# AechPro/rlgym-ppo

Measured on AMD Instinct MI355X. Metric: ppo_update_samples_per_sec, higher is better.
Workload: dtype f32; 1 GPU; configs[1]: 4096 agents x 128 steps = 524,288-sample buffer, obs 107 f32, 90 discrete actions, 256x3 policy + critic; batch 524,288, minibatch 65,536

## Files before the change

### rlgym_ppo_amd/csrc/api.hip

```cpp
#include "build_id.h"
#include <math.h>
#include <stdarg.h>
#include <string.h>

#include "common.hpp"

namespace rlppo {

static thread_local char g_err[512] = "";

void set_error(const char *fmt, ...) {
    va_list ap;
    va_start(ap, fmt);
    vsnprintf(g_err, sizeof(g_err), fmt, ap);
    va_end(ap);
}

static int64_t padded_width(int64_t d) {
    const int64_t p16 = round_up(d, 16), p64 = round_up(d, 64);
    return (p64 - p16) * 10 >= p64 ? p16 : p64;
}
static int64_t padded_out(int64_t d) {
    if (d <= 32) return 32;
    if (d <= 64) return 64;
    if (d <= 96) return 96;
    return round_up(d, 128);
}

int make_layout(const int32_t *dims, int32_t n_layers, NetLayout *out) {
    RLPPO_CHECK_ARG(dims != nullptr && n_layers >= 1 && n_layers <= RLPPO_MAX_LAYERS, "network: n_layers=%d not in [1,%d]",
                    n_layers, RLPPO_MAX_LAYERS);
    for (int i = 0; i <= n_layers; ++i) RLPPO_CHECK_ARG(dims[i] >= 1, "network: dims[%d]=%d", i, dims[i]);
    out->n_layers = n_layers;
    int64_t off = 0, flat = 0;
    int pin = (int)padded_width(dims[0]);
    for (int l = 0; l < n_layers; ++l) {
        LayerLayout &L = out->L[l];
        L.in = dims[l];
        L.out = dims[l + 1];
        L.pin = pin;
        L.pout = (int)padded_out(dims[l + 1]);
        L.off_w = off;
        off += (int64_t)L.pout * L.pin;
        L.off_wt = off;
        off += (int64_t)L.pin * L.pout;
        L.off_b = off;
        off += L.pout;
        L.off_flat_w = flat;
        flat += (int64_t)L.out * L.in;
        L.off_flat_b = flat;
        flat += L.out;
        pin = L.pout;
    }
    out->packed_floats = off;
    out->flat_floats = flat;
    return 0;
}

static int max_pout(const NetLayout &net) {
    int m = 0;
    for (int l = 0; l < net.n_layers; ++l) m = net.L[l].pout > m ? net.L[l].pout : m;
    return m;
}

struct X3Layout {
    int64_t fwd[RLPPO_MAX_LAYERS], dx[RLPPO_MAX_LAYERS], total;
};
static void x3_layout(const NetLayout &net, X3Layout *o) {
    int64_t off = 0;
    const int last = net.n_layers - 1;
    for (int l = 0; l < net.n_layers; ++l) {
        const LayerLayout &L = net.L[l];
        o->fwd[l] = o->dx[l] = -1;
        if (l >= 1 && l < last && nt_split_ok(L.pout, L.pin)) {
            o->fwd[l] = off;
            off += (int64_t)3 * L.pout * L.pin;
        }
        if (l >= 1 && !(l == last && gemv_head_ok(L.out, L.pin)) && nt_split_ok(L.pin, L.pout)) {
            o->dx[l] = off;
            off += (int64_t)3 * L.pin * L.pout;
        }
    }
    o->total = off;
}

static int g_fold_vhead = 1;

struct RowSource {
    const float *x;
    int64_t ld;
    const unsigned *rowtab = nullptr;
    int64_t src_rows = 0;
};

static int forward(hipStream_t st, const NetLayout &net, const float *packed, const RowSource &in, int64_t n, int out_tanh,
                   float *const *acts, int bf16_operands = 0, unsigned long long *const *bits = nullptr, bool *have_bits = nullptr,
                   bool *head_folded = nullptr, const unsigned short *x3 = nullptr, bool head_prezeroed = false) {
    X3Layout xl;
    if (x3) x3_layout(net, &xl);
    if (have_bits)
        for (int l = 0; l < net.n_layers; ++l) have_bits[l] = false;
    const float *x = in.x;
    int64_t ldx = in.ld;
    const int hl = net.n_layers - 1;
    bool fold = head_folded && g_fold_vhead && hl >= 1 && !out_tanh && !bf16_operands && bits && bits[hl - 1] &&
                gemv_head_ok(net.L[hl].out, net.L[hl].pin) && net.L[hl - 1].pout / 128 <= 2;
    if (x3 && hl >= 1 && xl.fwd[hl - 1] >= 0) fold = false;
    if (head_folded) *head_folded = false;
    for (int l = 0; l < net.n_layers; ++l) {
        const LayerLayout &L = net.L[l];
        const bool last = l == net.n_layers - 1;
        const int epi = last ? (out_tanh ? EPI_BIAS_TANH : EPI_BIAS) : EPI_BIAS_RELU;
        int rc;
        if (last && head_folded && *head_folded) break;
        if (last && !out_tanh && gemv_head_ok(L.out, L.pin))
            rc = launch_gemv_fwd(st, x, ldx, packed + L.off_w, packed + L.off_b, acts[l], L.pout, n, L.pin, L.pout);
        else {
            rc = -1;
            if (!last && bits && bits[l] && x3 && xl.fwd[l] >= 0) {
                rc = launch_gemm_nt_split(st, x, ldx, x3 + xl.fwd[l], packed + L.off_b, acts[l], L.pout, n, L.pout, L.pin, 0, bits[l]);
                if (rc == 0) have_bits[l] = true;
            } else if (!last && bits && bits[l] && !bf16_operands) {
                NtDot dots[2];
                const bool fold_here = fold && l == hl - 1;
                if (fold_here) {
                    if (!head_prezeroed) RLPPO_HIP(hipMemsetAsync(acts[hl], 0, (size_t)n * sizeof(float), st));
                    dots[0].w = packed + net.L[hl].off_w;
                    dots[0].b = packed + net.L[hl].off_b;
                    dots[0].out = acts[hl];
                }
                rc = launch_gemm_nt_bits(st, x, ldx, packed + L.off_w, L.pin, packed + L.off_b, acts[l], L.pout, n, L.pout, L.pin,
                                         EPI_BIAS_RELU, bits[l], l == 0 ? in.rowtab : nullptr, in.src_rows, nullptr, fold_here ? dots : nullptr);
                if (rc == 0) have_bits[l] = true;
                if (fold_here) *head_folded = rc == 0;
            }
            if (l == 0 && in.rowtab && rc != 0) {
                if (rc == -1) set_error("forward: the gathered first layer needs the bitmask form");
                return rc == -1 ? RLPPO_ERR_ARG : rc;
            }
            if (rc == -1)
                rc = launch_gemm_nt(st, x, ldx, packed + L.off_w, L.pin, packed + L.off_b, nullptr, 0, acts[l], L.pout, n, L.pout,
                                    L.pin, epi, bf16_operands);
        }
        if (rc) return rc;
        x = acts[l];
        ldx = L.pout;
    }
    return 0;
}

static bool b16_next_wants_f32(const NetLayout &net, int l) {
    const int nx = l + 1, last = net.n_layers - 1;
    const LayerLayout &N = net.L[nx];
    if (nx == last) {
        const bool fwd_b16 = gemv_head_ok(N.out, N.pin) || nt_b16_ok(N.pout, N.pin, false);
        return !(fwd_b16 && thin_head_ok(N.out, N.pin));
    }
    return !(nt_b16_ok(N.pout, N.pin, true) && tn_b16_ok(N.pout, N.pin));
}
static int forward_b16(hipStream_t st, const NetLayout &net, const float *packed_r, const unsigned short *wb16, const float *x,
                       const unsigned short *xb, int64_t ldx, int64_t n, int out_tanh, float *const *acts,
                       unsigned short *const *actsb, unsigned long long *const *bits, bool *have_bits, bool *f32_valid) {
    for (int l = 0; l < net.n_layers; ++l) have_bits[l] = f32_valid[l] = false;
    int64_t off16 = 0;
    bool x_f32 = true;
    for (int l = 0; l < net.n_layers; ++l) {
        const LayerLayout &L = net.L[l];
        const bool last = l == net.n_layers - 1;
        int rc = 0;
        auto need_x_f32 = [&]() -> int {
            if (x_f32) return 0;
            x_f32 = f32_valid[l - 1] = true;
            return launch_expand_rows(st, actsb[l - 1], acts[l - 1], n * (int64_t)net.L[l - 1].pout);
        };
        if (last) {
            const int epi = out_tanh ? EPI_BIAS_TANH : EPI_BIAS;
            if (!out_tanh && gemv_head_ok(L.out, L.pin))
                rc = launch_gemv_fwd_b16(st, xb, ldx, packed_r + L.off_w, packed_r + L.off_b, acts[l], L.pout, n, L.pin, L.pout);
            else if (nt_b16_ok(L.pout, L.pin, false))
                rc = launch_gemm_nt_b16(st, xb, ldx, wb16 + off16, L.pin, packed_r + L.off_b, acts[l], L.pout, nullptr, 0, n, L.pout,
                                        L.pin, epi, 0, nullptr);
            else {
                rc = need_x_f32();
                if (rc == 0)
                    rc = launch_gemm_nt(st, x, ldx, packed_r + L.off_w, L.pin, packed_r + L.off_b, nullptr, 0, acts[l], L.pout, n,
                                        L.pout, L.pin, epi);
            }
            f32_valid[l] = true;
        } else if (nt_b16_ok(L.pout, L.pin, true) && bits[l]) {
            const bool want = b16_next_wants_f32(net, l);
            rc = launch_gemm_nt_b16(st, xb, ldx, wb16 + off16, L.pin, packed_r + L.off_b, want ? acts[l] : nullptr, L.pout, actsb[l],
                                    L.pout, n, L.pout, L.pin, EPI_BIAS_RELU, 1, bits[l]);
            have_bits[l] = rc == 0;
            f32_valid[l] = want;
        } else {
            rc = need_x_f32();
            if (rc) return rc;
            rc = -1;
            if (bits[l]) {
                rc = launch_gemm_nt_bits(st, x, ldx, packed_r + L.off_w, L.pin, packed_r + L.off_b, acts[l], L.pout, n, L.pout, L.pin,
                                         EPI_BIAS_RELU, bits[l]);
                have_bits[l] = rc == 0;
            }
            if (rc == -1)
                rc = launch_gemm_nt(st, x, ldx, packed_r + L.off_w, L.pin, packed_r + L.off_b, nullptr, 0, acts[l], L.pout, n, L.pout,
                                    L.pin, EPI_BIAS_RELU);
            if (rc == 0) rc = launch_round_rows(st, acts[l], actsb[l], n * (int64_t)L.pout);
            f32_valid[l] = true;
        }
        if (rc) return rc;
        off16 += (int64_t)L.pout * L.pin;
        x = acts[l];
        xb = actsb[l];
        x_f32 = f32_valid[l];
        ldx = L.pout;
    }
    return 0;
}

static size_t forward_ws_floats(const NetLayout &net, int64_t n) { return (size_t)2 * (size_t)n * (size_t)max_pout(net); }

static int forward_pingpong(hipStream_t st, const NetLayout &net, const float *packed, const float *obs, int64_t ld_obs,
                            int64_t n, int out_tanh, void *ws, size_t ws_bytes, float *final_out, const float **out,
                            int64_t *ld_out, int bf16_operands) {
    if (ws_bytes < forward_ws_floats(net, n) * sizeof(float)) {
        set_error("forward: workspace %zu < %zu bytes", ws_bytes, forward_ws_floats(net, n) * sizeof(float));
        return RLPPO_ERR_WORKSPACE;
    }
    RLPPO_CHECK_ARG(ld_obs >= net.L[0].pin && ld_obs % 4 == 0, "forward: ld_obs=%ld must be >= %d (zero padded rows)",
                    (long)ld_obs, net.L[0].pin);
    float *b0 = reinterpret_cast<float *>(ws);
    float *b1 = b0 + (size_t)n * max_pout(net);
    float *acts[RLPPO_MAX_LAYERS];
    for (int l = 0; l < net.n_layers; ++l) acts[l] = (l & 1) ? b1 : b0;
    if (final_out) acts[net.n_layers - 1] = final_out;
    int rc = forward(st, net, packed, RowSource{obs, ld_obs}, n, out_tanh, acts, bf16_operands);
    if (rc) return rc;
    *out = acts[net.n_layers - 1];
    *ld_out = net.L[net.n_layers - 1].pout;
    return 0;
}

}

using namespace rlppo;

static int g_fused_act = 1;
static std::atomic<long long> g_cnt_fused_act{0}, g_cnt_act_chain{0}, g_cnt_paired_pass{0}, g_cnt_gather_fused_pass{0}, g_cnt_pass{0}, g_cnt_group_dw{0}, g_cnt_md_nvec{0};
constexpr int64_t FUSED_ACT_MAX_ROWS = 8192;

struct ActCtx {
    int bf16 = 0;
    unsigned *done = nullptr;
    unsigned done_value = 0;
    unsigned *noise_ctl = nullptr;
    const unsigned *mask = nullptr;
    int mask_words = 0;
};
static int act_ctx(const rlppo_act_opts *o, ActCtx *c, bool late_noise = false, const char *mask_for = nullptr) {
    c->bf16 = get_infer_bf16();
    if (!o) return 0;
    RLPPO_CHECK_ARG(o->precision == RLPPO_PRECISION_DEFAULT || o->precision == RLPPO_PRECISION_FP32 || o->precision == RLPPO_PRECISION_BF16,
                    "act options: inference precision %d (0 = process default, 1 = fp32, 2 = bf16 operands)", o->precision);
    if (o->precision != RLPPO_PRECISION_DEFAULT) c->bf16 = o->precision == RLPPO_PRECISION_BF16;
    c->done = o->done_words;
    c->done_value = o->done_value;
    c->noise_ctl = o->noise_ctl;
    c->mask = o->action_mask;
    c->mask_words = o->mask_words;
    RLPPO_CHECK_ARG(!o->action_mask || !mask_for, "act options: action_mask is an option of the discrete head, not of %s", mask_for ? mask_for : "");
    RLPPO_CHECK_ARG(!o->noise_ctl || late_noise, "act options: noise_ctl is an option of rlppo_discrete_step");
    RLPPO_CHECK_ARG(!o->noise_ctl || (o->done_words && !(o->done_value & 0x80000000u)),
                    "act options: noise_ctl needs done_words (a kernel that gives up on the noise reports it there) and done_value < 2^31");
    return 0;
}
static int mask_words_check(const void *mask, int mask_words, int bits, const char *who, bool logits) {
    RLPPO_CHECK_ARG(!mask || mask_words == (bits + 31) / 32,
                    logits ? "%s: mask_words=%d, but %d logits need %d words per row" : "%s: mask_words=%d, but n_actions=%d needs %d words per row",
                    who, mask_words, bits, (bits + 31) / 32);
    return 0;
}
static int act_mask_check(const ActCtx &c, int n_actions) { return mask_words_check(c.mask, c.mask_words, n_actions, "act options", false); }
static int act_done(hipStream_t st, const ActCtx &c, int64_t n) {
    return c.done ? launch_signal_words(st, c.done, (int)rlppo_act_done_words(n), c.done_value) : 0;
}

extern "C" {
// ... 369 lines not shown
static int ensure_slot(SlotBank &b, int s) {
    if (!b.side[s]) {
        RLPPO_HIP(hipStreamCreateWithFlags(&b.side[s], hipStreamNonBlocking));
        RLPPO_HIP(hipStreamCreateWithFlags(&b.main[s], hipStreamNonBlocking));
        RLPPO_HIP(hipEventCreateWithFlags(&b.ev_fork[s], hipEventDisableTiming));
        RLPPO_HIP(hipEventCreateWithFlags(&b.ev_join[s], hipEventDisableTiming));
        RLPPO_HIP(hipEventCreateWithFlags(&b.ev_slot[s], hipEventDisableTiming));
        RLPPO_HIP(hipEventCreateWithFlags(&b.ev_mid[s], hipEventDisableTiming));
    }
    return 0;
}
static int order_after(hipStream_t to, hipStream_t from, hipEvent_t ev) {
    RLPPO_HIP(hipEventRecord(ev, from));
    RLPPO_HIP(hipStreamWaitEvent(to, ev, 0));
    return 0;
}

static size_t tn_layer_floats(const NetLayout &net, int l, int64_t mb, int prec) {
    size_t f = tn_partial_floats(net.L[l].out, net.L[l].in, mb);
    if (net.L[l].out == 1) {
        const size_t g = (size_t)cdiv(mb, 64) * (size_t)(net.L[l].pin + 4);
        if (g > f) f = g;
    }
    if (prec == 1 && l == net.n_layers - 1) {
        const size_t g = thin_dw_ws_floats(net.L[l].out, net.L[l].pin, mb);
        if (g > f) f = g;
    }
    return (f + 3) / 4 * 4;
}
static size_t tn_ws_floats(const NetLayout &net, int64_t mb, int prec) {
    size_t m = 0;
    for (int l = 0; l < net.n_layers; ++l) {
        const size_t f = tn_layer_floats(net, l, mb, prec);
        m = f > m ? f : m;
    }
    return m;
}
static int g_group_dw = 1;
struct DwList {
    TnProduct p[2 * RLPPO_MAX_LAYERS];
    int n = 0;
    void add(const LayerLayout &L, const float *dY, const RowSource &X, float *grad) {
        TnProduct &q = p[n++];
        q.dY = dY; q.ldy = L.pout; q.ny_valid = L.pout; q.X = X.x; q.ldx = X.ld; q.kx_valid = L.pin;
        q.dW = grad + L.off_flat_w; q.db = grad + L.off_flat_b; q.out = L.out; q.in = L.in;
        q.rowtab = X.rowtab; q.src_rows = X.src_rows;
    }
};
static bool dw_is_gemv(const NetLayout &net, int l) { return l == net.n_layers - 1 && l > 0 && gemv_head_ok(net.L[l].out, net.L[l].pin); }
static size_t tn_region_floats(const NetLayout &pol, const NetLayout &val, int64_t mb, int prec) {
    const size_t chains = tn_ws_floats(pol, mb, prec) + tn_ws_floats(val, mb, prec);
    int outs[2 * RLPPO_MAX_LAYERS], ins[2 * RLPPO_MAX_LAYERS], n = 0;
    for (const NetLayout *net : {&pol, &val})
        for (int l = 0; l < net->n_layers; ++l)
            if (!dw_is_gemv(*net, l)) {
                outs[n] = net->L[l].out;
                ins[n++] = net->L[l].in;
            }
    const size_t group = tn_group_floats(outs, ins, n, mb);
    return chains > group ? chains : group;
}

struct NetWs {
    float *act[RLPPO_MAX_LAYERS] = {};
    float *dx[RLPPO_MAX_LAYERS] = {};
    unsigned long long *bits[RLPPO_MAX_LAYERS] = {};
    unsigned short *actb[RLPPO_MAX_LAYERS] = {};
    unsigned short *dxb[RLPPO_MAX_LAYERS] = {};
    float *tn = nullptr;
};
struct WsPlan {
    NetWs pol, val;
    size_t tn_floats = 0;
    float *states = nullptr;
    float *g_old = nullptr, *g_adv = nullptr, *g_tgt = nullptr, *g_act = nullptr;
    unsigned *rowtab = nullptr;
    unsigned short *states_b = nullptr;
};
constexpr size_t BITS_PAD_RESERVE = 2, B16_PAD_RESERVE = 4;
static size_t plan_workspace(const NetLayout &pol, const NetLayout &val, int64_t mb, int prec, void *base, WsPlan *w) {
    const uintptr_t addr = reinterpret_cast<uintptr_t>(base);
    const size_t rows = (size_t)mb;
    size_t off = 0, slack = 0;
    auto take = [&](size_t floats) {
        off += floats;
        return reinterpret_cast<float *>(addr + (off - floats) * sizeof(float));
    };
    auto align = [&](size_t floats, size_t reserve) {
        const size_t pad = (floats - (addr / sizeof(float) + off) % floats) % floats;
        off += pad;
        slack += reserve - pad;
    };
    const NetLayout *nets[2] = {&pol, &val};
    NetWs *ws[2] = {&w->pol, &w->val};
    for (int i = 0; i < 2; ++i)
        for (int l = 0; l < nets[i]->n_layers; ++l) ws[i]->act[l] = take(rows * nets[i]->L[l].pout);
    const size_t m = max_pout(pol) > max_pout(val) ? max_pout(pol) : max_pout(val);
    for (int i = 0; i < 2; ++i)
        for (int l = 0; l + 1 < nets[i]->n_layers; ++l) ws[i]->dx[l] = take(rows * m);
    w->tn_floats = tn_region_floats(pol, val, mb, prec);
    w->pol.tn = take(w->tn_floats);
    w->val.tn = w->pol.tn + tn_ws_floats(pol, mb, prec);
    align(2, BITS_PAD_RESERVE);
    for (int i = 0; i < 2; ++i)
        for (int l = 0; l + 1 < nets[i]->n_layers; ++l) {
            const size_t f = nt_bits_floats(mb, nets[i]->L[l].pout);
            ws[i]->bits[l] = f ? reinterpret_cast<unsigned long long *>(take(f)) : nullptr;
        }
    w->states = take(rows * pol.L[0].pin);
    w->g_old = take(rows);
    w->g_adv = take(rows);
    w->g_tgt = take(rows);
    w->g_act = take(rows * pol.L[pol.n_layers - 1].pout);
    w->rowtab = reinterpret_cast<unsigned *>(take(rows));
    if (prec == 1) {
        align(4, B16_PAD_RESERVE);
        size_t el = pol.L[0].pin;
        for (int i = 0; i < 2; ++i)
            for (int l = 0; l + 1 < nets[i]->n_layers; ++l) el += 2 * (size_t)nets[i]->L[l].pout;
        unsigned short *hb = reinterpret_cast<unsigned short *>(take((el * rows + 1) / 2));
        auto take16 = [&](size_t n) {
            hb += n;
            return hb - n;
        };
        w->states_b = take16(rows * pol.L[0].pin);
        for (int i = 0; i < 2; ++i)
            for (int l = 0; l + 1 < nets[i]->n_layers; ++l) ws[i]->actb[l] = take16(rows * nets[i]->L[l].pout);
        for (int i = 0; i < 2; ++i)
            for (int l = 0; l + 1 < nets[i]->n_layers; ++l) ws[i]->dxb[l] = take16(rows * nets[i]->L[l].pout);
    }
    return off + slack;
}

static int resolve_precision(int32_t precision, int *mode) {
    RLPPO_CHECK_ARG(precision >= 0 && precision <= 3, "update precision %d (0 = process default, 1 = fp32, 2 = bf16 mixed precision, 3 = split-bf16 products)", precision);
    *mode = precision == RLPPO_PRECISION_DEFAULT ? g_update_bf16 : precision - 1;
    return 0;
}
size_t rlppo_minibatch_workspace_bytes_for(const int32_t *pol_dims, int32_t pol_layers, const int32_t *val_dims, int32_t val_layers,
                                           int64_t mb, int32_t precision) {
    NetLayout pol, val;
    int prec = 0;
    if (make_layout(pol_dims, pol_layers, &pol) || make_layout(val_dims, val_layers, &val) || resolve_precision(precision, &prec)) return 0;
    WsPlan unused;
    return plan_workspace(pol, val, mb > 0 ? mb : 0, prec, nullptr, &unused) * sizeof(float) + 256;
}
size_t rlppo_minibatch_workspace_bytes(const int32_t *pol_dims, int32_t pol_layers, const int32_t *val_dims,
                                       int32_t val_layers, int64_t mb) {
    return rlppo_minibatch_workspace_bytes_for(pol_dims, pol_layers, val_dims, val_layers, mb, RLPPO_PRECISION_DEFAULT);
}

static int backward(hipStream_t st, const NetLayout &net, const float *packed, const RowSource &in, int64_t mb, float *const *acts,
                    float *const *dx, float *grad, float *tn_ws, unsigned long long *const *bits, const bool *have_bits,
                    bool head_folded = false, const unsigned short *x3 = nullptr, DwList *defer = nullptr) {
    const int last = net.n_layers - 1;
    int rc = 0;
    X3Layout xl;
    if (x3) x3_layout(net, &xl);
    for (int l = last; l >= 0; --l) {
        const LayerLayout &L = net.L[l];
        const float *dY = l == last ? acts[last] : dx[l];
        const int64_t ld_hy = head_folded ? 1 : L.pout;
        const RowSource X = l > 0 ? RowSource{acts[l - 1], net.L[l - 1].pout} : in;
        const bool gemv = l == last && l > 0 && gemv_head_ok(L.out, L.pin);
        const size_t floats = tn_layer_floats(net, l, mb, 0);
        if (gemv)
            rc = launch_gemv_dw(st, dY, ld_hy, X.x, X.ld, grad + L.off_flat_w, grad + L.off_flat_b, L.in, L.pin, mb, tn_ws, floats);
        else if (defer)
            defer->add(L, dY, X, grad);
        else
            rc = launch_gemm_tn(st, dY, L.pout, L.pout, X.x, X.ld, L.pin, grad + L.off_flat_w, grad + L.off_flat_b, L.out, L.in, mb,
                                tn_ws, floats, X.rowtab, X.src_rows);
        if (rc) return rc;
        if (l == 0) break;
        rc = -1;
        if (gemv) {
            if (have_bits[l - 1]) rc = launch_gemv_dx_bits(st, dY, ld_hy, packed + L.off_w, bits[l - 1], dx[l - 1], L.pin, L.pin, mb);
            if (rc == -1) rc = launch_gemv_dx(st, dY, ld_hy, packed + L.off_w, acts[l - 1], L.pin, dx[l - 1], L.pin, L.pin, mb);
        } else {
            if (have_bits[l - 1] && x3 && xl.dx[l] >= 0)
                rc = launch_gemm_nt_split(st, dY, L.pout, x3 + xl.dx[l], nullptr, dx[l - 1], L.pin, mb, L.pin, L.pout, 1, bits[l - 1]);
            else if (have_bits[l - 1])
                rc = launch_gemm_nt_bits(st, dY, L.pout, packed + L.off_wt, L.pout, nullptr, dx[l - 1], L.pin, mb, L.pin, L.pout,
                                         EPI_MASK, bits[l - 1]);
            if (rc == -1)
                rc = launch_gemm_nt(st, dY, L.pout, packed + L.off_wt, L.pout, nullptr, acts[l - 1], L.pin, dx[l - 1], L.pin, mb,
                                    L.pin, L.pout, EPI_MASK);
        }
        if (rc) return rc;
    }
    return rc;
}

static int backward_b16(hipStream_t st, const NetLayout &net, const float *packed_r, const unsigned short *wb16, const float *states,
                        const unsigned short *states_b, int64_t ld_states, int64_t mb, float *const *acts,
                        unsigned short *const *actsb, float *const *dx, unsigned short *const *dxb, float *grad, float *tn_ws,
                        size_t tn_floats, unsigned long long *const *bits, const bool *have_bits, bool *f32_valid) {
    const int last = net.n_layers - 1;
    int64_t first[RLPPO_MAX_LAYERS], total = 0;
    for (int l = 0; l < net.n_layers; ++l) {
        first[l] = total;
        total += (int64_t)net.L[l].pout * net.L[l].pin;
    }
    bool dx_f32[RLPPO_MAX_LAYERS] = {};
    int rc = 0;
    auto act_f32 = [&](int l) -> int {
        if (l < 0 || f32_valid[l]) return 0;
        f32_valid[l] = true;
        return launch_expand_rows(st, actsb[l], acts[l], mb * (int64_t)net.L[l].pout);
    };
    auto grad_f32 = [&](int l) -> int {
        if (dx_f32[l]) return 0;
        dx_f32[l] = true;
        return launch_expand_rows(st, dxb[l], dx[l], mb * (int64_t)net.L[l].pout);
    };
    for (int l = last; l >= 0; --l) {
        const LayerLayout &L = net.L[l];
        const float *X = l > 0 ? acts[l - 1] : states;
        const unsigned short *Xb = l > 0 ? actsb[l - 1] : states_b;
        const int64_t ldx = l > 0 ? net.L[l - 1].pout : ld_states;
        const bool gemv = l == last && l > 0 && gemv_head_ok(L.out, L.pin);
        if (l == last) {
            rc = l > 0 ? launch_thin_dw_b16(st, acts[last], L.pout, Xb, ldx, grad + L.off_flat_w, grad + L.off_flat_b, L.out, L.in,
                                            L.pin, mb, tn_ws, tn_floats)
                       : -1;
            if (rc == -1) {
                rc = act_f32(l - 1);
                if (rc) return rc;
                if (gemv)
                    rc = launch_gemv_dw(st, acts[last], L.pout, X, ldx, grad + L.off_flat_w, grad + L.off_flat_b, L.in, L.pin, mb,
                                        tn_ws, tn_floats);
                else
                    rc = launch_gemm_tn(st, acts[last], L.pout, L.pout, X, ldx, L.pin, grad + L.off_flat_w, grad + L.off_flat_b,
                                        L.out, L.in, mb, tn_ws, tn_floats);
            }
        } else if (tn_b16_ok(L.pout, L.pin) && ldx % 8 == 0) {
            rc = launch_gemm_tn_b16(st, dxb[l], L.pout, Xb, ldx, grad + L.off_flat_w, grad + L.off_flat_b, L.pout, L.pin, L.out, L.in,
                                    mb, tn_ws, tn_floats);
        } else {
            rc = grad_f32(l);
            if (rc == 0) rc = act_f32(l - 1);
            if (rc) return rc;
            rc = launch_gemm_tn(st, dx[l], L.pout, L.pout, X, ldx, L.pin, grad + L.off_flat_w, grad + L.off_flat_b, L.out, L.in, mb,
                                tn_ws, tn_floats);
        }
        if (rc) return rc;
        if (l == 0) break;
        if (l < last && have_bits[l - 1] && nt_b16_ok(L.pin, L.pout, true)) {
            rc = launch_gemm_nt_b16(st, dxb[l], L.pout, wb16 + total + first[l], L.pout, nullptr, nullptr, 0, dxb[l - 1], L.pin, mb,
                                    L.pin, L.pout, EPI_MASK, 2, bits[l - 1]);
            if (rc) return rc;
            continue;
        }
        if (l == last && have_bits[l - 1]) {
            rc = launch_thin_dx_b16(st, acts[last], L.pout, L.out, packed_r + L.off_w, L.pin, bits[l - 1], dxb[l - 1], L.pin, L.pin, mb);
            if (rc == 0) continue;
            if (rc != -1) return rc;
        }
        const float *dY = acts[last];
        if (l < last) {
            rc = grad_f32(l);
            if (rc) return rc;
            dY = dx[l];
        }
        rc = -1;
        if (gemv) {
            if (have_bits[l - 1]) rc = launch_gemv_dx_bits(st, dY, L.pout, packed_r + L.off_w, bits[l - 1], dx[l - 1], L.pin, L.pin, mb);
            if (rc == -1) {
                rc = act_f32(l - 1);
                if (rc) return rc;
                rc = launch_gemv_dx(st, dY, L.pout, packed_r + L.off_w, acts[l - 1], L.pin, dx[l - 1], L.pin, L.pin, mb);
            }
        } else {
            if (have_bits[l - 1])
                rc = launch_gemm_nt_bits(st, dY, L.pout, packed_r + L.off_wt, L.pout, nullptr, dx[l - 1], L.pin, mb, L.pin, L.pout,
                                         EPI_MASK, bits[l - 1]);
            if (rc == -1) {
                rc = act_f32(l - 1);
                if (rc) return rc;
                rc = launch_gemm_nt(st, dY, L.pout, packed_r + L.off_wt, L.pout, nullptr, acts[l - 1], L.pin, dx[l - 1], L.pin, mb,
                                    L.pin, L.pout, EPI_MASK);
            }
        }
        if (rc) return rc;
        rc = launch_round_rows(st, dx[l - 1], dxb[l - 1], mb * (int64_t)L.pin);
        if (rc) return rc;
        dx_f32[l - 1] = true;
    }
    return rc;
}

static int g_head_order = 1;
static int g_paired = 1;
constexpr int64_t PAIRED_MIN_ROWS = 262144;
static bool twin_ok(const NetLayout &p, const NetLayout &v, int64_t mb) {
    if (p.n_layers != v.n_layers || p.n_layers < 2) return false;
    for (int l = 0; l + 1 < p.n_layers; ++l) {
        const LayerLayout &a = p.L[l], &b = v.L[l];
        if (a.in != b.in || a.out != b.out || a.pin != b.pin || a.pout != b.pout) return false;
        if (a.pout % 128 != 0 || a.pin % 16 != 0 || nt_bits_floats(mb, a.pout) == 0) return false;
    }
    return true;
}

static int head_forward(hipStream_t st, const NetLayout &net, const float *packed, const float *x, int64_t ldx, int64_t n, int out_tanh,
                        float *out) {
    const LayerLayout &L = net.L[net.n_layers - 1];
    if (!out_tanh && gemv_head_ok(L.out, L.pin)) return launch_gemv_fwd(st, x, ldx, packed + L.off_w, packed + L.off_b, out, L.pout, n, L.pin, L.pout);
    return launch_gemm_nt(st, x, ldx, packed + L.off_w, L.pin, packed + L.off_b, nullptr, 0, out, L.pout, n, L.pout, L.pin,
                          out_tanh ? EPI_BIAS_TANH : EPI_BIAS);
}
static int head_backward(hipStream_t st, const NetLayout &net, const float *packed, const float *dY, const float *X, int64_t mb,
                         float *dx_prev, float *grad, float *tn_ws, const unsigned long long *bits_prev, int64_t ld_dy = 0,
                         DwList *defer = nullptr) {
    const int last = net.n_layers - 1;
    const LayerLayout &L = net.L[last];
    const int64_t ldx = net.L[last - 1].pout;
    const bool gemv = gemv_head_ok(L.out, L.pin);
    const size_t floats = tn_layer_floats(net, last, mb, 0);
    if (!ld_dy) ld_dy = L.pout;
    int rc = 0;
    if (gemv) rc = launch_gemv_dw(st, dY, ld_dy, X, ldx, grad + L.off_flat_w, grad + L.off_flat_b, L.in, L.pin, mb, tn_ws, floats);
    else if (defer) defer->add(L, dY, RowSource{X, ldx}, grad);
    else rc = launch_gemm_tn(st, dY, L.pout, L.pout, X, ldx, L.pin, grad + L.off_flat_w, grad + L.off_flat_b, L.out, L.in, mb, tn_ws, floats);
    if (rc) return rc;
    if (gemv) return launch_gemv_dx_bits(st, dY, ld_dy, packed + L.off_w, bits_prev, dx_prev, L.pin, L.pin, mb);
    rc = launch_gemm_nt_bits(st, dY, L.pout, packed + L.off_wt, L.pout, nullptr, dx_prev, L.pin, mb, L.pin, L.pout, EPI_MASK,
                             const_cast<unsigned long long *>(bits_prev));
    if (rc == -1) {
        set_error("paired pass: the output layer's dX needs the bitmask form");
        return RLPPO_ERR_ARG;
    }
    return rc;
}

constexpr int64_t FUSED_GATHER_MIN_ROWS = 262144;
static RowSource first_layer_rows(const rlppo_minibatch_args &a, const NetLayout &pol, const NetLayout &val, int prec, const WsPlan &w) {
    const int64_t src_rows = a.ring_cap > 0 ? a.ring_cap : a.n_rows;
    auto gather_form = [&](const NetLayout &n) {
        return n.n_layers > 1 && nt_gather_ok(a.ld_states, src_rows, n.L[0].pout, n.L[0].pin) && tn_gather_ok(a.ld_states, src_rows) &&
               !(n.L[0].out > 64 && n.L[0].out <= 96 && !(n.L[0].in > 96 && n.L[0].in <= 112));
    };
    if (prec != 1 && (g_fused_gather == 2 || (g_fused_gather == 1 && a.mb >= FUSED_GATHER_MIN_ROWS)) && src_rows > 0 &&
        gather_form(pol) && gather_form(val))
        return RowSource{a.states, a.ld_states, w.rowtab, src_rows};
    return RowSource{w.states, pol.L[0].pin};
}

struct Pass {
    const rlppo_minibatch_args *a;
    NetLayout pol, val;
    int64_t mb;
    int prec;
    int64_t ring_base, ring_cap;
    WsPlan w;
    RowSource rows;
    LossCfg cfg;
    MdSpec md;
    bool md_general = false;
    const float *pol_w, *val_w;
    hipStream_t st, side;
    DwList *defer;
};

static LossCfg loss_cfg(const rlppo_minibatch_args &a) {
    LossCfg c;
    c.clip = a.clip_range;
    c.clip_lo = (float)(1.0 - (double)a.clip_range);
    c.clip_hi = (float)(1.0 + (double)a.clip_range);
    c.ent_coef = a.ent_coef;
    c.mb_ratio = a.mb_ratio;
    c.inv_mb = 1.0f / (float)a.mb;
    c.var_m = a.var_m;
    c.var_b = a.var_b;
    c.adv_norm = a.adv_norm;
    c.vclip = a.value_clip;
    c.kl_slots = a.kl_slots;
    c.stop_word = a.stop_word;
    return c;
}

static int policy_loss(hipStream_t st, const Pass &p) {
    const rlppo_minibatch_args &a = *p.a;
    const int last = p.pol.n_layers - 1;
    const LayerLayout &L = p.pol.L[last];
    const WsPlan &w = p.w;
    MaskRows mr;
    mr.mask = a.action_mask;
    mr.W = a.mask_words;
    mr.idx = a.idx;
    mr.ring_base = p.ring_base;
    mr.ring_cap = p.ring_cap;
    if (a.head == RLPPO_HEAD_DISCRETE) {
        return launch_discrete_loss(st, w.pol.act[last], L.pout, L.out, w.g_act, w.g_old, w.g_adv, p.mb, p.cfg, a.stats, a.action_mask ? &mr : nullptr);
    }
    if (a.head == RLPPO_HEAD_GAUSSIAN)
        return launch_gaussian_loss(st, w.pol.act[last], L.pout, L.out / 2, w.g_act, w.g_old, w.g_adv, p.mb, p.cfg, a.stats);
    if (p.md_general) {
        ++g_cnt_md_nvec;
        return launch_multidiscrete_nvec_loss(st, w.pol.act[last], L.pout, w.g_act, w.g_old, w.g_adv, p.mb, p.cfg, a.stats, p.md,
                                              a.action_mask ? &mr : nullptr);
    }
    return launch_multidiscrete_loss(st, w.pol.act[last], L.pout, w.g_act, w.g_old, w.g_adv, p.mb, p.cfg, a.stats);
}

static int gather(const Pass &p) {
    const rlppo_minibatch_args &a = *p.a;
    const WsPlan &w = p.w;
    const int width = p.pol.L[0].pin;
    float *const vout = w.val.act[p.val.n_layers - 1];
    if (p.prec == 1) {
        auto lean0 = [](const NetLayout &n) {
            return n.n_layers > 1 && nt_b16_ok(n.L[0].pout, n.L[0].pin, true) && tn_b16_ok(n.L[0].pout, n.L[0].pin);
        };
        const int rc = launch_gather_rows_round(p.st, a.states, a.ld_states, a.idx, lean0(p.pol) && lean0(p.val) ? nullptr : w.states,
                                                w.states_b, width, p.mb, p.ring_base, p.ring_cap);
        if (rc) return rc;
    } else if (!p.rows.rowtab) {
        GatherMeta gm;
        gm.actions = a.actions; gm.old_logp = a.old_logp; gm.adv = a.advantages; gm.targets = a.targets;
        gm.g_old = w.g_old; gm.g_adv = w.g_adv; gm.g_tgt = w.g_tgt; gm.g_act = w.g_act;
        gm.zero_n = vout;
        gm.act_dim = a.act_dim;
        return launch_gather_rows(p.st, a.states, a.ld_states, a.idx, w.states, width, p.mb, p.ring_base, p.ring_cap, &gm);
    }
    return launch_gather_meta(p.st, a.idx, a.actions, a.act_dim, a.old_logp, a.advantages, a.targets, w.g_act, w.g_old, w.g_adv, w.g_tgt,
                              p.mb, p.ring_base, p.ring_cap, p.rows.rowtab ? w.rowtab : nullptr, vout);
}

static int paired_pass(const Pass &p, SlotBank &bk, int slot) {
    const rlppo_minibatch_args &a = *p.a;
    const NetLayout &pol = p.pol, &val = p.val;
    const WsPlan &w = p.w;
    const int64_t mb = p.mb;
    const hipStream_t st = p.st, hs = p.side;
    const int H = pol.n_layers - 1;
    int rc;
    const LayerLayout &Lvh = val.L[H];
    const bool fold_v = g_fold_vhead && gemv_head_ok(Lvh.out, Lvh.pin) && val.L[H - 1].pout / 128 <= 2;
    float *vout = w.val.act[H], *pout = w.pol.act[H];
    const int64_t ldv = fold_v ? 1 : Lvh.pout;
    const float *xp = p.rows.x, *xv = xp;
    int64_t ldx = p.rows.ld;
    for (int l = 0; l < H; ++l) {
        const LayerLayout &Lp = pol.L[l], &Lv = val.L[l];
        NtAlt alt;
        alt.A = xv;
        alt.B = p.val_w + Lv.off_w;
        alt.bias = p.val_w + Lv.off_b;
        alt.C = w.val.act[l];
        alt.bits = w.val.bits[l];
        NtDot dots[2];
        const bool fold_here = fold_v && l == H - 1;
        if (fold_here) {
            dots[1].w = p.val_w + Lvh.off_w;
            dots[1].out = vout;
            dots[1].b = p.val_w + Lvh.off_b;
        }
        rc = launch_gemm_nt_bits(st, xp, ldx, p.pol_w + Lp.off_w, Lp.pin, p.pol_w + Lp.off_b, w.pol.act[l], Lp.pout, mb, Lp.pout, Lp.pin,
                                 EPI_BIAS_RELU, w.pol.bits[l], l == 0 ? p.rows.rowtab : nullptr, p.rows.src_rows, &alt,
                                 fold_here ? dots : nullptr);
        if (rc) {
            if (rc == -1) set_error("paired pass: a hidden layer does not have the bitmask form");
            return rc == -1 ? RLPPO_ERR_ARG : rc;
        }
        xp = w.pol.act[l];
        xv = w.val.act[l];
        ldx = Lp.pout;
    }
    if (hs != st) {
        rc = order_after(hs, st, bk.ev_fork[slot]);
        if (rc) return rc;
    }
    if (!fold_v) {
        rc = head_forward(hs, val, p.val_w, xv, ldx, mb, 0, vout);
        if (rc) return rc;
    }
    rc = launch_value_loss(hs, vout, ldv, w.g_tgt, w.g_adv, mb, p.cfg, a.stats);
    if (rc) return rc;
    const bool ordered = g_head_order && hs != st;
    if (!ordered) {
        rc = head_backward(hs, val, p.val_w, vout, xv, mb, w.val.dx[H - 1], a.val_grad, w.val.tn, w.val.bits[H - 1], ldv, p.defer);
        if (rc) return rc;
    }
    rc = head_forward(st, pol, p.pol_w, xp, ldx, mb, a.head == RLPPO_HEAD_GAUSSIAN, pout);
    if (rc) return rc;
    rc = policy_loss(st, p);
    if (rc) return rc;
    if (ordered) {
        rc = order_after(hs, st, bk.ev_mid[slot]);
        if (rc) return rc;
        rc = head_backward(hs, val, p.val_w, vout, xv, mb, w.val.dx[H - 1], a.val_grad, w.val.tn, w.val.bits[H - 1], ldv, p.defer);
        if (rc) return rc;
    }
    rc = head_backward(st, pol, p.pol_w, pout, xp, mb, w.pol.dx[H - 1], a.pol_grad, w.pol.tn, w.pol.bits[H - 1], 0, p.defer);
    if (rc) return rc;
    if (hs != st) {
        rc = order_after(st, hs, bk.ev_join[slot]);
        if (rc) return rc;
    }
    for (int l = H - 1; l >= 0; --l) {
        const LayerLayout &Lp = pol.L[l], &Lv = val.L[l];
        const RowSource Xp = l > 0 ? RowSource{w.pol.act[l - 1], pol.L[l - 1].pout} : p.rows;
        const RowSource Xv = l > 0 ? RowSource{w.val.act[l - 1], val.L[l - 1].pout} : p.rows;
        if (p.defer) {
            p.defer->add(Lp, w.pol.dx[l], Xp, a.pol_grad);
            p.defer->add(Lv, w.val.dx[l], Xv, a.val_grad);
        } else {
            TnPair pr;
            pr.dY = w.val.dx[l];
            pr.X = Xv.x;
            pr.dW = a.val_grad + Lv.off_flat_w;
            pr.db = a.val_grad + Lv.off_flat_b;
            pr.ws = w.val.tn;
            rc = launch_gemm_tn(st, w.pol.dx[l], Lp.pout, Lp.pout, Xp.x, Xp.ld, Lp.pin, a.pol_grad + Lp.off_flat_w, a.pol_grad + Lp.off_flat_b,
                                Lp.out, Lp.in, mb, w.pol.tn, tn_layer_floats(pol, l, mb, 0), Xp.rowtab, Xp.src_rows, &pr);
            if (rc) return rc;
        }
        if (l == 0) break;
        NtAlt alt;
        alt.A = w.val.dx[l];
        alt.B = p.val_w + Lv.off_wt;
        alt.C = w.val.dx[l - 1];
        alt.bits = w.val.bits[l - 1];
        rc = launch_gemm_nt_bits(st, w.pol.dx[l], Lp.pout, p.pol_w + Lp.off_wt, Lp.pout, nullptr, w.pol.dx[l - 1], Lp.pin, mb, Lp.pin,
                                 Lp.pout, EPI_MASK, w.pol.bits[l - 1], nullptr, 0, &alt);
        if (rc) return rc == -1 ? RLPPO_ERR_ARG : rc;
    }
    return 0;
}

static int two_chain_pass(const Pass &p) {
    const rlppo_minibatch_args &a = *p.a;
    const NetLayout &pol = p.pol, &val = p.val;
    const WsPlan &w = p.w;
    const int64_t mb = p.mb;
    const bool b16 = p.prec == 1;
    const unsigned short *pol_wb16 = reinterpret_cast<const unsigned short *>(a.pol_wb16);
    const unsigned short *val_wb16 = reinterpret_cast<const unsigned short *>(a.val_wb16);
    const unsigned short *pol_x3 = p.prec == 2 ? pol_wb16 : nullptr, *val_x3 = p.prec == 2 ? val_wb16 : nullptr;
    bool phave[RLPPO_MAX_LAYERS] = {}, vhave[RLPPO_MAX_LAYERS] = {};
    bool pf32[RLPPO_MAX_LAYERS] = {}, vf32[RLPPO_MAX_LAYERS] = {};
    bool v_folded = false;
    int rc;
    if (b16) {
        rc = forward_b16(p.side, val, p.val_w, val_wb16, p.rows.x, w.states_b, p.rows.ld, mb, 0, w.val.act, w.val.actb, w.val.bits, vhave,
                         vf32);
        if (rc) return rc;
        rc = forward_b16(p.st, pol, p.pol_w, pol_wb16, p.rows.x, w.states_b, p.rows.ld, mb, a.head == RLPPO_HEAD_GAUSSIAN, w.pol.act,
                         w.pol.actb, w.pol.bits, phave, pf32);
    } else {
        rc = forward(p.side, val, p.val_w, p.rows, mb, 0, w.val.act, 0, w.val.bits, vhave, &v_folded, val_x3, true);
        if (rc) return rc;
        rc = forward(p.st, pol, p.pol_w, p.rows, mb, a.head == RLPPO_HEAD_GAUSSIAN, w.pol.act, 0, w.pol.bits, phave, nullptr, pol_x3);
    }
    if (rc) return rc;
    const int64_t ldv = v_folded ? 1 : val.L[val.n_layers - 1].pout;
    rc = launch_value_loss(p.side, w.val.act[val.n_layers - 1], ldv, w.g_tgt, w.g_adv, mb, p.cfg, a.stats);
    if (rc) return rc;
    rc = policy_loss(p.st, p);
    if (rc) return rc;
    if (b16) {
        rc = backward_b16(p.side, val, p.val_w, val_wb16, p.rows.x, w.states_b, p.rows.ld, mb, w.val.act, w.val.actb, w.val.dx, w.val.dxb,
                          a.val_grad, w.val.tn, tn_ws_floats(val, mb, p.prec), w.val.bits, vhave, vf32);
        if (rc) return rc;
        return backward_b16(p.st, pol, p.pol_w, pol_wb16, p.rows.x, w.states_b, p.rows.ld, mb, w.pol.act, w.pol.actb, w.pol.dx, w.pol.dxb,
                            a.pol_grad, w.pol.tn, tn_ws_floats(pol, mb, p.prec), w.pol.bits, phave, pf32);
    }
    rc = backward(p.side, val, p.val_w, p.rows, mb, w.val.act, w.val.dx, a.val_grad, w.val.tn, w.val.bits, vhave, v_folded, val_x3, p.defer);
    if (rc) return rc;
    return backward(p.st, pol, p.pol_w, p.rows, mb, w.pol.act, w.pol.dx, a.pol_grad, w.pol.tn, w.pol.bits, phave, false, pol_x3, p.defer);
}

static int ppo_minibatch(void *stream, const rlppo_minibatch_args *a, const int32_t *md_nvec, int32_t md_heads) {
    RLPPO_CHECK_ARG(a != nullptr, "ppo_minibatch: null args");
    Pass p;
    p.a = a;
    int rc = make_layout(a->pol_dims, a->pol_layers, &p.pol);
    if (rc) return rc;
    rc = make_layout(a->val_dims, a->val_layers, &p.val);
    if (rc) return rc;
    const NetLayout &pol = p.pol, &val = p.val;
    const int64_t mb = p.mb = a->mb;
    if (mb == 0) return 0;
    rc = resolve_precision(a->precision, &p.prec);
    if (rc) return rc;
    RLPPO_CHECK_ARG(mb > 0 && a->pol_packed && a->val_packed && a->pol_grad && a->val_grad && a->states && a->actions &&
                        a->old_logp && a->targets && a->advantages && a->idx && a->stats && a->workspace,
                    "ppo_minibatch: null pointer");
    RLPPO_CHECK_ARG(val.L[val.n_layers - 1].out == 1, "ppo_minibatch: critic must have one output");
    RLPPO_CHECK_ARG(a->value_clip >= 0.f && a->value_clip < INFINITY, "ppo_minibatch: value_clip=%g", (double)a->value_clip);
    RLPPO_CHECK_ARG(pol.L[0].in == val.L[0].in, "ppo_minibatch: policy and critic observe different sizes");
    RLPPO_CHECK_ARG(a->ld_states >= pol.L[0].pin && a->ld_states % 4 == 0, "ppo_minibatch: ld_states=%ld < %d",
                    (long)a->ld_states, pol.L[0].pin);
    const size_t ws_bytes = plan_workspace(pol, val, mb, p.prec, a->workspace, &p.w) * sizeof(float);
    if (a->ws_bytes < ws_bytes) {
        set_error("ppo_minibatch: workspace %zu < %zu bytes", a->ws_bytes, ws_bytes);
        return RLPPO_ERR_WORKSPACE;
    }
    const int n_out = pol.L[pol.n_layers - 1].out;
    RLPPO_CHECK_ARG(a->head == RLPPO_HEAD_DISCRETE || a->head == RLPPO_HEAD_GAUSSIAN || a->head == RLPPO_HEAD_MULTIDISCRETE,
                    "ppo_minibatch: unknown head %d", a->head);
    RLPPO_CHECK_ARG(!a->action_mask || a->head == RLPPO_HEAD_DISCRETE || (a->head == RLPPO_HEAD_MULTIDISCRETE && md_nvec),
                    "ppo_minibatch: action_mask is an option of the discrete head, not of the %s head",
                    a->head == RLPPO_HEAD_GAUSSIAN ? "Gaussian" : "multi-discrete (without md_nvec: the fixed-bin kernels take no mask)");
    if (int rc_mask = mask_words_check(a->action_mask, a->mask_words, n_out, "ppo_minibatch", false)) return rc_mask;
    if (a->head == RLPPO_HEAD_DISCRETE) {
        RLPPO_CHECK_ARG(a->act_dim == 1, "discrete head: act_dim must be 1");
        RLPPO_CHECK_ARG(pol.L[pol.n_layers - 1].pout <= DISCRETE_LOSS_MAX_LD, "discrete head: padded width %ld too large",
                        (long)pol.L[pol.n_layers - 1].pout);
    }
    if (a->head == RLPPO_HEAD_GAUSSIAN)
        RLPPO_CHECK_ARG(n_out % 2 == 0 && a->act_dim == n_out / 2, "gaussian head: act_dim=%d, outputs=%d", a->act_dim, n_out);
    RLPPO_CHECK_ARG(!md_nvec || a->head == RLPPO_HEAD_MULTIDISCRETE, "ppo_minibatch: md_nvec is an option of the multi-discrete head, not of the %s head",
                    a->head == RLPPO_HEAD_GAUSSIAN ? "Gaussian" : "discrete");
    if (a->head == RLPPO_HEAD_MULTIDISCRETE && md_nvec) {
        rc = md_spec_make(md_nvec, md_heads, "multi-discrete head: md_nvec / md_heads", &p.md);
        if (rc) return rc;
        p.md_general = true;
        RLPPO_CHECK_ARG(p.md.S == n_out, "multi-discrete head: md_nvec sums to %d, but the policy has %d outputs", p.md.S, n_out);
        RLPPO_CHECK_ARG(a->act_dim == p.md.H, "multi-discrete head: act_dim=%d, but md_heads=%d", a->act_dim, p.md.H);
    } else if (a->head == RLPPO_HEAD_MULTIDISCRETE)
        RLPPO_CHECK_ARG(n_out == 21 && a->act_dim == 8, "multi-discrete head: needs 21 outputs and act_dim 8");
    RLPPO_CHECK_ARG(p.prec != 1 || (a->pol_packed_r && a->val_packed_r && a->pol_wb16 && a->val_wb16),
                    "ppo_minibatch: the bf16 update precision needs the rlppo_net_pack_bf16 images of both networks (pol_packed_r / val_packed_r / pol_wb16 / val_wb16)");
    RLPPO_CHECK_ARG(p.prec != 2 || (a->pol_wb16 && a->val_wb16),
                    "ppo_minibatch: the split-bf16 update precision needs the rlppo_net_pack_x3 images of both networks (pol_wb16 / val_wb16)");
    p.ring_cap = a->ring_cap > 0 ? a->ring_cap : INT64_MAX;
    p.ring_base = a->ring_cap > 0 ? a->ring_base : 0;
    RLPPO_CHECK_ARG(p.ring_base >= 0 && p.ring_base < p.ring_cap, "ppo_minibatch: ring_base=%ld not in [0, ring_cap=%ld)",
                    (long)a->ring_base, (long)a->ring_cap);
    const int slot = a->slot;
    RLPPO_CHECK_ARG(slot >= 0 && slot < RLPPO_MAX_SLOTS, "ppo_minibatch: slot %d not in [0, %d)", slot, RLPPO_MAX_SLOTS);

    p.rows = first_layer_rows(*a, pol, val, p.prec, p.w);
    const bool twin = p.prec == 0 && (g_paired == 2 || (g_paired == 1 && mb >= PAIRED_MIN_ROWS)) && twin_ok(pol, val, mb);
    p.cfg = loss_cfg(*a);
    p.pol_w = p.prec == 1 ? a->pol_packed_r : a->pol_packed;
    p.val_w = p.prec == 1 ? a->val_packed_r : a->val_packed;
    DwList dws;
    p.defer = (g_group_dw && p.prec != 1) ? &dws : nullptr;

    SlotBank *bank = nullptr;
    rc = slot_bank(&bank);
    if (rc) return rc;
    SlotBank &bk = *bank;
    rc = ensure_slot(bk, slot);
    if (rc) return rc;
    const hipStream_t caller = (hipStream_t)stream;
    p.st = caller;
    if (slot > 0) {
        p.st = bk.main[slot];
        rc = order_after(p.st, caller, bk.ev_slot[slot]);
        if (rc) return rc;
        bk.pending[slot] = true;
    }
    rc = gather(p);
    if (rc) return rc;
    p.side = p.st;
    if (g_two_streams) {
        p.side = bk.side[slot];
        rc = order_after(p.side, p.st, bk.ev_fork[slot]);
        if (rc) return rc;
    }
    ++g_cnt_pass;
    if (twin) ++g_cnt_paired_pass;
    if (p.rows.rowtab) ++g_cnt_gather_fused_pass;
    rc = twin ? paired_pass(p, bk, slot) : two_chain_pass(p);
    if (rc) return rc;
    if (!twin && p.side != p.st) {
        rc = order_after(p.st, p.side, bk.ev_join[slot]);
        if (rc) return rc;
    }
    if (p.defer && dws.n) {
        ++g_cnt_group_dw;
        rc = launch_gemm_tn_group(p.st, dws.p, dws.n, mb, p.w.pol.tn, p.w.tn_floats);
    }
    return rc;
}

int rlppo_ppo_minibatch(void *stream, const rlppo_minibatch_args *a) { return ppo_minibatch(stream, a, nullptr, 0); }
int rlppo_ppo_minibatch_nvec(void *stream, const rlppo_minibatch_args *a, const int32_t *md_nvec, int32_t md_heads) {
    return ppo_minibatch(stream, a, md_nvec, md_heads);
}

int rlppo_ppo_join(void *stream) {
    SlotBank *bank = nullptr;
    int rc = slot_bank(&bank);
    if (rc) return rc;
    SlotBank &bk = *bank;
    for (int s = 1; s < RLPPO_MAX_SLOTS; ++s)
        if (bk.pending[s]) {
            rc = order_after((hipStream_t)stream, bk.main[s], bk.ev_slot[s]);
            if (rc) return rc;
            bk.pending[s] = false;
        }
    return 0;
}

int rlppo_clip_adam(void *stream, float *params, float *grads, float *exp_avg, float *exp_avg_sq, int64_t n,
                    double max_norm, double lr, double beta1, double beta2, double eps, int64_t step, double *gnorm2) {
    if (n == 0) return 0;
    RLPPO_CHECK_ARG(n > 0 && params && grads && exp_avg && exp_avg_sq && gnorm2 && step >= 1, "clip_adam: bad argument");
    const double bc1 = 1.0 - pow(beta1, (double)step);
    const double bc2 = 1.0 - pow(beta2, (double)step);
    const float step_size = (float)(lr / bc1);
    const float bc2_sqrt = (float)sqrt(bc2);
    return launch_clip_adam((hipStream_t)stream, params, grads, exp_avg, exp_avg_sq, n, (float)max_norm, step_size, bc2_sqrt,
                            (float)(1.0 - beta1), (float)beta2, (float)(1.0 - beta2), (float)eps, gnorm2);
}

int rlppo_clip_adam_pack2(void *stream, const rlppo_opt_net *a, const rlppo_opt_net *b, void *sync_ws) {
    RLPPO_CHECK_ARG(a && b, "clip_adam_pack2: null descriptor");
    const rlppo_opt_net *d[2] = {a, b};
    NetLayout nets[2];
    float *p[2], *g[2], *m[2], *v[2], *packed[2];
    double *gn[2];
    int64_t n[2];
    float max_norm[2], step_size[2], bc2_sqrt[2], omb1[2], beta2[2], omb2[2], eps[2];
    const unsigned *skip[2];
    for (int k = 0; k < 2; ++k) {
        skip[k] = d[k]->skip_word;
        int rc = make_layout(d[k]->dims, d[k]->n_layers, &nets[k]);
        if (rc) return rc;
        RLPPO_CHECK_ARG(d[k]->params && d[k]->grads && d[k]->exp_avg && d[k]->exp_avg_sq && d[k]->packed && d[k]->gnorm2 &&
                            d[k]->step >= 1, "clip_adam_pack2: bad argument (net %d)", k);
        const double bc1 = 1.0 - pow(d[k]->beta1, (double)d[k]->step);
        const double bc2 = 1.0 - pow(d[k]->beta2, (double)d[k]->step);
        p[k] = d[k]->params; g[k] = d[k]->grads; m[k] = d[k]->exp_avg; v[k] = d[k]->exp_avg_sq; packed[k] = d[k]->packed;
        gn[k] = d[k]->gnorm2;
        const LayerLayout &last = nets[k].L[nets[k].n_layers - 1];
        n[k] = last.off_flat_b + last.out;
        max_norm[k] = (float)d[k]->max_norm; step_size[k] = (float)(d[k]->lr / bc1); bc2_sqrt[k] = (float)sqrt(bc2);
        omb1[k] = (float)(1.0 - d[k]->beta1); beta2[k] = (float)d[k]->beta2; omb2[k] = (float)(1.0 - d[k]->beta2);
        eps[k] = (float)d[k]->eps;
    }
    return launch_clip_adam_pack2((hipStream_t)stream, nets, p, g, m, v, packed, gn, n, max_norm, step_size, bc2_sqrt, omb1, beta2,
                                  omb2, eps, sync_ws, skip);
}

int64_t rlppo_kl_slots_doubles(int64_t mb) { return kl_slots_doubles(mb); }

int rlppo_adv_stats(void *stream, const int64_t *idx, int64_t n, const float *advantages, int64_t ring_base, int64_t ring_cap,
                    float *out, void *ws) {
    RLPPO_CHECK_ARG(n >= 1 && idx && advantages && out && ws, "adv_stats: bad argument");
    const int64_t cap = ring_cap > 0 ? ring_cap : INT64_MAX, base = ring_cap > 0 ? ring_base : 0;
    RLPPO_CHECK_ARG(base >= 0 && base < cap, "adv_stats: ring_base=%ld not in [0, ring_cap=%ld)", (long)ring_base, (long)ring_cap);
    return launch_adv_stats((hipStream_t)stream, idx, n, advantages, base, cap, out, ws);
}

int rlppo_kl_gate(void *stream, const rlppo_kl_gate_args *a) {
    RLPPO_CHECK_ARG(a && a->kl_slots && a->n_passes >= 0 && a->slot_stride >= 3 && a->phase >= 0 && a->phase <= 2 && a->stop_word,
                    "kl_gate: bad argument");
    RLPPO_CHECK_ARG(a->phase == 0 || a->exchange, "kl_gate: phases 1 and 2 need the exchange words");
    RLPPO_CHECK_ARG(a->phase == 1 || a->host_words, "kl_gate: host_words missing");
    return launch_kl_gate((hipStream_t)stream, *a);
}

int rlppo_learn_report(void *stream, const rlppo_report_args *a) {
    RLPPO_CHECK_ARG(a != nullptr, "learn_report: null args");
    RLPPO_CHECK_ARG(a->n_pol >= 0 && a->n_val >= 0 && (a->n_pol == 0 || (a->pol_before && a->pol_now)) && (a->n_val == 0 || (a->val_before && a->val_now)),
                    "learn_report: parameter vectors missing");
    RLPPO_CHECK_ARG(a->stats && a->out && a->done_word && a->ws, "learn_report: null pointer (stats / out / done_word / ws)");
    RLPPO_CHECK_ARG((reinterpret_cast<uintptr_t>(a->ws) & 15) == 0, "learn_report: ws must be 16-byte aligned");
    return launch_learn_report((hipStream_t)stream, *a);
}

}

extern "C" {
int rlppo_gather_rows(void *stream, const float *src, int64_t ld_src, const int64_t *idx, float *dst, int32_t width, int64_t n) {
    if (n == 0) return 0;
    RLPPO_CHECK_ARG(n > 0 && src && idx && dst, "gather_rows: null pointer");
    return launch_gather_rows((hipStream_t)stream, src, ld_src, idx, dst, width, n);
}
int rlppo_welford_increment(void *stream, const float *samples, int64_t ld, int64_t n, int32_t d, void *mean, void *m2,
                            int64_t count, int32_t state_is_f64) {
    if (n == 0) return 0;
    RLPPO_CHECK_ARG(n > 0 && d > 0 && ld >= d && count >= 0 && samples && mean && m2, "welford_increment: bad argument");
    return launch_welford((hipStream_t)stream, samples, ld, n, d, mean, m2, (long long)count, state_is_f64 != 0);
}
int rlppo_welford_merge(void *stream, int32_t d, void *mean, void *m2, int64_t count, const float *other_mean,
                        const float *other_m2, int64_t other_count, int32_t state_is_f64) {
    if (other_count == 0) return 0;
    RLPPO_CHECK_ARG(d > 0 && count >= 0 && other_count > 0 && mean && m2 && other_mean && other_m2, "welford_merge: bad argument");
    return launch_welford_merge((hipStream_t)stream, d, mean, m2, (long long)count, other_mean, other_m2, (long long)other_count,
                                state_is_f64 != 0);
}
int64_t rlppo_wb16_elems(const int32_t *dims, int32_t n_layers) {
    NetLayout net;
    if (make_layout(dims, n_layers, &net)) return -1;
    int64_t n = 0;
    for (int l = 0; l < net.n_layers; ++l) n += (int64_t)net.L[l].pout * net.L[l].pin;
    return 2 * n;
}
int rlppo_net_pack_bf16(void *stream, const int32_t *dims, int32_t n_layers, const float *flat, float *packed_r, void *wb16) {
    NetLayout net;
    int rc = make_layout(dims, n_layers, &net);
    if (rc) return rc;
    RLPPO_CHECK_ARG(flat && packed_r && wb16, "net_pack_bf16: null pointer");
    return launch_pack_bf16((hipStream_t)stream, net, flat, packed_r, reinterpret_cast<unsigned short *>(wb16));
}
int64_t rlppo_x3_elems(const int32_t *dims, int32_t n_layers) {
    NetLayout net;
    if (make_layout(dims, n_layers, &net)) return -1;
    X3Layout xl;
    x3_layout(net, &xl);
    return xl.total;
}
int rlppo_net_pack_x3(void *stream, const int32_t *dims, int32_t n_layers, const float *packed, void *planes) {
    NetLayout net;
    int rc = make_layout(dims, n_layers, &net);
    if (rc) return rc;
    X3Layout xl;
    x3_layout(net, &xl);
    if (xl.total == 0) return 0;
    RLPPO_CHECK_ARG(packed && planes, "net_pack_x3: null pointer");
    unsigned short *pl = reinterpret_cast<unsigned short *>(planes);
    for (int l = 0; l < net.n_layers; ++l) {
        const LayerLayout &L = net.L[l];
        if (xl.fwd[l] >= 0) {
            rc = launch_pack_split((hipStream_t)stream, packed + L.off_w, L.pin, L.pout, L.pin, pl + xl.fwd[l]);
            if (rc) return rc;
        }
        if (xl.dx[l] >= 0) {
            rc = launch_pack_split((hipStream_t)stream, packed + L.off_wt, L.pout, L.pin, L.pout, pl + xl.dx[l]);
            if (rc) return rc;
        }
    }
    return 0;
}
int rlppo_dbg_pack_x3(void *stream, const float *S, int64_t ld, int32_t R, int32_t C, void *planes) {
    return launch_pack_split((hipStream_t)stream, S, ld, R, C, reinterpret_cast<unsigned short *>(planes));
}
int rlppo_dbg_gemm_nt_x3(void *stream, const float *A, int64_t lda, const void *planes, const float *bias, float *C, int64_t ldc, int64_t M,
                         int32_t N, int32_t K, int32_t mode, void *bits) {
    return launch_gemm_nt_split((hipStream_t)stream, A, lda, reinterpret_cast<const unsigned short *>(planes), bias, C, ldc, M, N, K, mode,
                                reinterpret_cast<unsigned long long *>(bits));
}
static int64_t g_selection_epoch = 0;
int rlppo_set_update_precision(int32_t mode) {
    RLPPO_CHECK_ARG(mode >= 0 && mode <= 2, "set_update_precision: mode %d (0 = fp32, 1 = bf16 mixed precision, 2 = split-bf16 products)", mode);
    g_update_bf16 = mode;
    ++g_selection_epoch;
    return 0;
}
int rlppo_get_update_precision(void) { return g_update_bf16; }
int rlppo_set_inference_precision(int32_t mode) {
    RLPPO_CHECK_ARG(mode == 0 || mode == 1, "set_inference_precision: mode %d (0 = fp32, 1 = bf16 operands)", mode);
    set_infer_bf16(mode);
    ++g_selection_epoch;
    return 0;
}
int rlppo_dbg_set(int32_t key, int32_t value) {
    ++g_selection_epoch;
    switch (key) {
        case 1: set_gae_algo(value); return 0;
        case 4: g_two_streams = value; return 0;
        case 21: set_gae_spin_limit(value); return 0;
        case 22: set_gae_oversubscribe(value); return 0;
        case 34: set_fused_spin_limit(value); return 0;
        case 35: set_fused_test_hold(value); return 0;
        case 36: set_split_persistent(value); return 0;
        case 23: set_b16_wide_tiles(value); return 0;
        case 24: set_exp_fast_transform(value); return 0;
        case 26: g_fused_gather = value; return 0;
        case 27: g_fused_act = value; return 0;
        case 29: g_paired = value; return 0;
        case 31: g_head_order = value; return 0;
        case 32: g_fold_vhead = value; return 0;
        case 33: set_pair_interleave(value); return 0;
        case 37: g_group_dw = value; return 0;
        case 38: set_tn_group_budget(value); return 0;
        case 40: set_nt_skinny(value); return 0;
        case 41: g_window_mode = value; return 0;
        default: break;
    }
    set_error("dbg_set: unknown key %d", key);
    return RLPPO_ERR_ARG;
}
int64_t rlppo_selection_epoch(void) { return g_selection_epoch; }
const int64_t *rlppo_selection_epoch_ptr(void) { return &g_selection_epoch; }
int rlppo_dbg_count(int32_t key, int64_t delta) {
    RLPPO_CHECK_ARG(key == 6, "dbg_count: key %d (only counter 6 is kept by hosts that replay)", key);
    g_cnt_md_nvec += delta;
    return 0;
}
int64_t rlppo_dbg_counter(int32_t key) {
    switch (key) {
        case 0: return g_cnt_fused_act;
        case 1: return g_cnt_act_chain;
        case 2: return g_cnt_pass;
        case 3: return g_cnt_paired_pass;
        case 4: return g_cnt_gather_fused_pass;
        case 5: return g_cnt_group_dw;
        case 6: return g_cnt_md_nvec;
        default: return -1;
    }
}
size_t rlppo_dbg_gemm_nt_bits_bytes(int64_t M, int32_t N) { return nt_bits_floats(M, N) * sizeof(float); }
int rlppo_dbg_gemm_nt_bits(void *stream, const float *A, int64_t lda, const float *B, int64_t ldb, const float *bias, float *C,
                           int64_t ldc, int64_t M, int32_t N, int32_t K, int32_t epilogue, void *bits) {
    const int rc = launch_gemm_nt_bits((hipStream_t)stream, A, lda, B, ldb, bias, C, ldc, M, N, K, epilogue,
                                       reinterpret_cast<unsigned long long *>(bits));
    if (rc == -1) {
        set_error("dbg_gemm_nt_bits: the bitmask form does not apply to this call");
        return RLPPO_ERR_ARG;
    }
    return rc;
}
int rlppo_dbg_gemm_nt(void *stream, const float *A, int64_t lda, const float *B, int64_t ldb, const float *bias,
                      const float *mask_src, int64_t ld_mask, float *C, int64_t ldc, int64_t M, int32_t N, int32_t K,
                      int32_t epilogue) {
    return launch_gemm_nt((hipStream_t)stream, A, lda, B, ldb, bias, mask_src, ld_mask, C, ldc, M, N, K, epilogue);
}
int rlppo_dbg_gemm_nt_b16(void *stream, const void *A, int64_t lda, const void *W, int64_t ldw, const float *bias, float *C,
                          int64_t ldc, void *Cb, int64_t ldcb, int64_t M, int32_t N, int32_t K, int32_t epilogue, int32_t hidden,
                          void *bits) {
    return launch_gemm_nt_b16((hipStream_t)stream, reinterpret_cast<const unsigned short *>(A), lda,
                              reinterpret_cast<const unsigned short *>(W), ldw, bias, C, ldc, reinterpret_cast<unsigned short *>(Cb),
                              ldcb, M, N, K, epilogue, hidden, reinterpret_cast<unsigned long long *>(bits));
}
int rlppo_dbg_gemm_tn_b16(void *stream, const void *dY, int64_t ldy, const void *X, int64_t ldx, float *dW, float *db, int32_t pout,
                          int32_t pin, int32_t out, int32_t in, int64_t M, void *ws, size_t ws_bytes) {
    return launch_gemm_tn_b16((hipStream_t)stream, reinterpret_cast<const unsigned short *>(dY), ldy,
                              reinterpret_cast<const unsigned short *>(X), ldx, dW, db, pout, pin, out, in, M, (float *)ws,
                              ws_bytes / sizeof(float));
}
size_t rlppo_dbg_thin_head_workspace_bytes(int32_t out, int32_t kp, int64_t M) { return thin_dw_ws_floats(out, kp, M) * sizeof(float); }
int rlppo_dbg_thin_head_b16(void *stream, const float *dY, int64_t ldy, int32_t out, const float *W, int64_t ldw, const void *bits,
                            const void *hb, int64_t ldh, void *dxb, float *dW, float *db, int32_t in, int32_t kp, int64_t M, void *ws,
                            size_t ws_bytes) {
    int rc = launch_thin_dx_b16((hipStream_t)stream, dY, ldy, out, W, ldw, reinterpret_cast<const unsigned long long *>(bits),
                                reinterpret_cast<unsigned short *>(dxb), kp, kp, M);
    if (rc) return rc == -1 ? RLPPO_ERR_ARG : rc;
    rc = launch_thin_dw_b16((hipStream_t)stream, dY, ldy, reinterpret_cast<const unsigned short *>(hb), ldh, dW, db, out, in, kp, M,
                            (float *)ws, ws_bytes / sizeof(float));
    return rc == -1 ? RLPPO_ERR_ARG : rc;
}
static int tn_products(const rlppo_tn_product *p, int32_t n, TnProduct *q) {
    RLPPO_CHECK_ARG(p && n > 0 && n <= 2 * RLPPO_MAX_LAYERS, "gemm_tn_group: %d products (1..%d)", n, 2 * RLPPO_MAX_LAYERS);
    for (int i = 0; i < n; ++i) {
        q[i].dY = p[i].dY; q[i].ldy = p[i].ldy; q[i].ny_valid = p[i].ny_valid; q[i].X = p[i].X; q[i].ldx = p[i].ldx;
        q[i].kx_valid = p[i].kx_valid; q[i].dW = p[i].dW; q[i].db = p[i].db; q[i].out = p[i].out; q[i].in = p[i].in;
        q[i].rowtab = p[i].rowtab; q[i].src_rows = p[i].src_rows;
    }
    return 0;
}
size_t rlppo_dbg_gemm_tn_group_workspace_bytes(const rlppo_tn_product *p, int32_t n, int64_t M) {
    if (!p || n <= 0 || n > 2 * RLPPO_MAX_LAYERS) return 0;
    int outs[2 * RLPPO_MAX_LAYERS], ins[2 * RLPPO_MAX_LAYERS];
    for (int i = 0; i < n; ++i) {
        outs[i] = p[i].out;
        ins[i] = p[i].in;
    }
    return tn_group_floats(outs, ins, n, M) * sizeof(float);
}
int rlppo_dbg_gemm_tn_group(void *stream, const rlppo_tn_product *p, int32_t n, int64_t M, void *ws, size_t ws_bytes) {
    TnProduct q[2 * RLPPO_MAX_LAYERS];
    const int rc = tn_products(p, n, q);
    if (rc) return rc;
    return launch_gemm_tn_group((hipStream_t)stream, q, n, M, (float *)ws, ws_bytes / sizeof(float));
}
size_t rlppo_dbg_gemm_tn_workspace_bytes(int32_t out, int32_t in, int64_t M) { return tn_partial_floats(out, in, M) * sizeof(float); }
int rlppo_dbg_gemm_tn(void *stream, const float *dY, int64_t ldy, int32_t ny_valid, const float *X, int64_t ldx,
                      int32_t kx_valid, float *dW, float *db, int32_t out, int32_t in, int64_t M, void *ws, size_t ws_bytes) {
    return launch_gemm_tn((hipStream_t)stream, dY, ldy, ny_valid, X, ldx, kx_valid, dW, db, out, in, M, (float *)ws,
                          ws_bytes / sizeof(float));
}
}
```

### rlgym_ppo_amd/csrc/common.hpp

```cpp
#pragma once
#include <hip/hip_runtime.h>
#include <stdint.h>
#include <stdio.h>

#include <atomic>

#include "../../include/rlppo.h"

namespace rlppo {

void set_error(const char *fmt, ...);

#define RLPPO_CHECK_ARG(cond, ...)                \
    do {                                          \
        if (!(cond)) {                            \
            rlppo::set_error(__VA_ARGS__);        \
            return RLPPO_ERR_ARG;                 \
        }                                         \
    } while (0)

#define RLPPO_HIP(expr)                                                                         \
    do {                                                                                        \
        hipError_t e_ = (expr);                                                                 \
        if (e_ != hipSuccess) {                                                                 \
            rlppo::set_error("%s failed: %s (%s:%d)", #expr, hipGetErrorString(e_), __FILE__, __LINE__); \
            return (int)e_;                                                                     \
        }                                                                                       \
    } while (0)

#define RLPPO_LAUNCH_CHECK() RLPPO_HIP(hipGetLastError())

struct PerDeviceOnce {
    std::atomic<unsigned long long> done{0};
};
inline int set_dynamic_lds_once(const void *fn, int bytes, PerDeviceOnce &once) {
    int dev = 0;
    RLPPO_HIP(hipGetDevice(&dev));
    const unsigned long long bit = 1ull << (dev & 63);
    if (!(once.done.load(std::memory_order_acquire) & bit)) {
        RLPPO_HIP(hipFuncSetAttribute(fn, hipFuncAttributeMaxDynamicSharedMemorySize, bytes));
        once.done.fetch_or(bit, std::memory_order_release);
    }
    return 0;
}
inline int device_cu_count(int *cus) {
    static std::atomic<int> by_dev[64];
    int dev = 0;
    RLPPO_HIP(hipGetDevice(&dev));
    int n = by_dev[dev & 63].load(std::memory_order_relaxed);
    if (n == 0) {
        RLPPO_HIP(hipDeviceGetAttribute(&n, hipDeviceAttributeMultiprocessorCount, dev));
        by_dev[dev & 63].store(n, std::memory_order_relaxed);
    }
    *cus = n;
    return 0;
}
#undef hipLaunchKernelGGL
#define hipLaunchKernelGGL(kernel, grid, block, shmem, stream, ...)        \
    do {                                                                   \
        (void)hipGetLastError();                                           \
        kernel<<<(grid), (block), (shmem), (stream)>>>(__VA_ARGS__);       \
    } while (0)

static inline int64_t round_up(int64_t x, int64_t m) { return (x + m - 1) / m * m; }
static inline int64_t cdiv(int64_t a, int64_t b) { return (a + b - 1) / b; }

struct LayerLayout {
    int in, out;
    int pin, pout;
    int64_t off_w, off_wt, off_b;
    int64_t off_flat_w, off_flat_b;
};

struct NetLayout {
    int n_layers;
    LayerLayout L[RLPPO_MAX_LAYERS];
    int64_t packed_floats;
    int64_t flat_floats;
};

int make_layout(const int32_t *dims, int32_t n_layers, NetLayout *out);

enum Epilogue { EPI_BIAS = 0, EPI_BIAS_RELU = 1, EPI_BIAS_TANH = 2, EPI_MASK = 3 };

int launch_gemm_nt(hipStream_t st, const float *A, int64_t lda, const float *B, int64_t ldb, const float *bias,
                   const float *mask_src, int64_t ld_mask, float *C, int64_t ldc, int64_t M, int N, int K, int epi,
                   int bf16_operands = 0);
size_t nt_bits_floats(int64_t M, int N);
struct NtAlt {
    const float *A = nullptr, *B = nullptr, *bias = nullptr;
    float *C = nullptr;
    unsigned long long *bits = nullptr;
    int interleave = 0;
};
struct NtDot {
    const float *w = nullptr, *b = nullptr;
    float *out = nullptr;
};
struct TnPair {
    const float *dY = nullptr, *X = nullptr;
    float *dW = nullptr, *db = nullptr, *ws = nullptr;
};
int launch_gemm_nt_bits(hipStream_t st, const float *A, int64_t lda, const float *B, int64_t ldb, const float *bias, float *C,
                        int64_t ldc, int64_t M, int N, int K, int epi, unsigned long long *bits, const unsigned *rowtab = nullptr,
                        int64_t src_rows = 0, const NtAlt *alt = nullptr, const NtDot *dot = nullptr );
bool nt_gather_ok(int64_t lda, int64_t src_rows, int N, int K);
int launch_gemm_nt_bf16(hipStream_t st, const float *A, int64_t lda, const float *B, int64_t ldb, const float *bias, float *C,
                        int64_t ldc, int64_t M, int N, int nb, int K, int epi);
void set_infer_bf16(int v);
void set_pair_interleave(int v);
void set_nt_skinny(int on);
int get_infer_bf16();
size_t tn_partial_floats(int out, int in, int64_t M);
int launch_gemm_tn(hipStream_t st, const float *dY, int64_t ldy, int ny_valid, const float *X, int64_t ldx, int kx_valid,
                   float *dW, float *db, int out, int in, int64_t M, float *ws, size_t ws_floats, const unsigned *rowtab = nullptr,
                   int64_t src_rows = 0, const TnPair *pair = nullptr);
bool tn_gather_ok(int64_t ldx, int64_t src_rows);
struct TnProduct {
    const float *dY = nullptr;
    int64_t ldy = 0;
    int ny_valid = 0;
    const float *X = nullptr;
    int64_t ldx = 0;
    int kx_valid = 0;
    float *dW = nullptr, *db = nullptr;
    int out = 0, in = 0;
    const unsigned *rowtab = nullptr;
    int64_t src_rows = 0;
};
constexpr int TN_GROUP_MAX = 2 * RLPPO_MAX_LAYERS;
size_t tn_group_floats(const int *outs, const int *ins, int n, int64_t M);
int launch_gemm_tn_group(hipStream_t st, const TnProduct *prods, int n, int64_t M, float *ws, size_t ws_floats);
void set_tn_group_budget(int workgroups);

bool nt_b16_ok(int N, int K, bool hidden);
bool nt_split_ok(int N, int K);
void set_split_persistent(int v);
int launch_pack_split(hipStream_t st, const float *S, int64_t ld, int R, int Cc, unsigned short *planes);
int launch_gemm_nt_split(hipStream_t st, const float *A, int64_t lda, const unsigned short *planes, const float *bias, float *C, int64_t ldc,
                         int64_t M, int N, int K, int mode, unsigned long long *bits);
int launch_gemm_nt_b16(hipStream_t st, const unsigned short *A, int64_t lda, const unsigned short *B, int64_t ldb, const float *bias,
                       float *C, int64_t ldc, unsigned short *Cb, int64_t ldcb, int64_t M, int N, int K, int epi, int mode,
                       unsigned long long *bits);
void set_b16_wide_tiles(int on);
bool tn_b16_ok(int pout, int pin);
int launch_gemm_tn_b16(hipStream_t st, const unsigned short *dY, int64_t ldy, const unsigned short *X, int64_t ldx, float *dW,
                       float *db, int pout, int pin, int out, int in, int64_t M, float *ws, size_t ws_floats);

void set_exp_fast_transform(int on);

bool gemv_head_ok(int out, int kp);
int launch_gemv_fwd(hipStream_t st, const float *x, int64_t ldx, const float *w, const float *b, float *y, int64_t ldy, int64_t n, int kp, int pout);
int launch_gemv_fwd_b16(hipStream_t st, const unsigned short *x, int64_t ldx, const float *w, const float *b, float *y, int64_t ldy,
                        int64_t n, int kp, int pout);
bool thin_head_ok(int out, int kp);
size_t thin_dw_ws_floats(int out, int kp, int64_t n);
int launch_thin_dx_b16(hipStream_t st, const float *dy, int64_t ldy, int out, const float *w, int64_t ldw,
                       const unsigned long long *bits, unsigned short *dxb, int64_t ldc, int kp, int64_t n);
int launch_thin_dw_b16(hipStream_t st, const float *dy, int64_t ldy, const unsigned short *xb, int64_t ldx, float *dw, float *db,
                       int out, int in, int kp, int64_t n, float *ws, size_t ws_floats);
int launch_gemv_dx(hipStream_t st, const float *dy, int64_t ldy, const float *w, const float *mask, int64_t ldm, float *dx, int64_t ldc, int kp, int64_t n);
int launch_gemv_dx_bits(hipStream_t st, const float *dy, int64_t ldy, const float *w, const unsigned long long *bits, float *dx,
                        int64_t ldc, int kp, int64_t n);
int launch_gemv_dw(hipStream_t st, const float *dy, int64_t ldy, const float *x, int64_t ldx, float *dw, float *db, int in, int kp, int64_t n,
                   float *ws = nullptr, size_t ws_floats = 0);

struct LossCfg {
    float clip, clip_lo, clip_hi, ent_coef, mb_ratio, inv_mb;
    float var_m, var_b;
    const float *adv_norm = nullptr;
    float vclip = 0.f;
    double *kl_slots = nullptr;
    const unsigned *stop_word = nullptr;
};
__host__ __device__ __forceinline__ int64_t ring_row(int64_t i, int64_t base, int64_t cap) {
    const int64_t r = i + base;
    return r >= cap ? r - cap : r;
}
int launch_discrete_sample_logits(hipStream_t, const float *, int64_t, int64_t, int, const float *, int64_t *, float *, float *,
                                  const unsigned *mask = nullptr, int mask_words = 0);
int launch_discrete_probs(hipStream_t st, const float *logits, int64_t ld, int64_t n, int A, int clamp, float *probs,
                          int64_t ld_p, int64_t *flat_argmax, const unsigned *mask = nullptr, int mask_words = 0);
struct MaskRows {
    const unsigned *mask = nullptr;
    int W = 0;
    const int64_t *idx = nullptr;
    int64_t ring_base = 0, ring_cap = INT64_MAX;
};
int launch_categorical_select(hipStream_t, const float *, int64_t, int64_t, int, const float *, int64_t *, float *);
int launch_gaussian_sample(hipStream_t, const float *, int64_t, int64_t, int, const float *, float, float, float *, float *,
                           unsigned *done_words = nullptr, unsigned done_value = 0);
int launch_multidiscrete_sample(hipStream_t, const float *, int64_t, int64_t, const float *, int64_t *, float *,
                                unsigned *done_words = nullptr, unsigned done_value = 0);
int launch_value_loss(hipStream_t st, float *vout, int64_t ldv, const float *targets, const float *adv, int64_t mb, const LossCfg &cfg,
                      double *stats);
int64_t kl_slots_doubles(int64_t mb);
constexpr int64_t DISCRETE_LOSS_MAX_LD = 64 * 32;
int launch_discrete_loss(hipStream_t, float *, int64_t, int, const float *, const float *, const float *, int64_t, const LossCfg &, double *,
                         const MaskRows *mask_rows = nullptr);
int launch_gaussian_loss(hipStream_t, float *, int64_t, int, const float *, const float *, const float *, int64_t, const LossCfg &, double *);
int launch_multidiscrete_loss(hipStream_t, float *, int64_t, const float *, const float *, const float *, int64_t, const LossCfg &, double *);
struct MdSpec {
    int H, B, S;
    unsigned char b[RLPPO_MD_MAX_HEADS];
};
int md_spec_make(const int32_t *nvec, int n_heads, const char *who, MdSpec *spec);
int launch_multidiscrete_nvec_sample(hipStream_t, const float *, int64_t, int64_t, const float *, int64_t *, float *, const MdSpec &,
                                     unsigned *done_words = nullptr, unsigned done_value = 0, const unsigned *mask = nullptr,
                                     int mask_words = 0);
int launch_multidiscrete_nvec_loss(hipStream_t, float *, int64_t, const float *, const float *, const float *, int64_t, const LossCfg &, double *,
                                   const MdSpec &, const MaskRows *mask_rows = nullptr);

struct FusedActIO {
    const float *rows = nullptr;
    int64_t ld_rows = 0;
    const void *raw = nullptr;
    int raw_is_f64 = 0, standardize = 0;
    int64_t ld_raw = 0;
    float mean0 = 0.f, std0 = 1.f;
    const float *mean_v = nullptr, *std_v = nullptr;
    float *rows_out = nullptr;
    int64_t ld_rows_out = 0;
    const float *noise = nullptr;
    int64_t *actions = nullptr;
    float *actions_f32 = nullptr;
    float *logp = nullptr, *probs_out = nullptr;
    unsigned *done_words = nullptr;
    unsigned done_value = 0;
    unsigned *noise_ctl = nullptr;
    const unsigned *mask = nullptr;
    int mask_words = 0;
};
bool fused_act_ok(const NetLayout &net);
}
void host_window_register(void *base, size_t bytes, unsigned *hdp_flush);
void host_window_unregister(void *base);
namespace rlppo {
int launch_discrete_act_fused(hipStream_t st, const NetLayout &net, const float *packed, const FusedActIO &io, int64_t n);

size_t gae_workspace_bytes(int64_t n);
void set_gae_algo(int algo);
void set_gae_spin_limit(int v);
void set_gae_oversubscribe(int v);
void set_fused_spin_limit(int v);
void set_fused_test_hold(int v);
int launch_gae(hipStream_t, const float *, const float *, const float *, const float *, const float *, int64_t, double, double, float,
               float *, float *, float *, void *, size_t);

int launch_pack(hipStream_t, const NetLayout &, const float *, float *);
int launch_pack_bf16(hipStream_t st, const NetLayout &net, const float *flat, float *packed_r, unsigned short *wb16);
int launch_round_rows(hipStream_t st, float *x, unsigned short *xb, int64_t n_elems);
int launch_expand_rows(hipStream_t st, const unsigned short *xb, float *x, int64_t n_elems);
int launch_gather_rows_round(hipStream_t st, const float *src, int64_t ld_src, const int64_t *idx, float *dst, unsigned short *dstb,
                             int width, int64_t n, int64_t ring_base, int64_t ring_cap);
int launch_clip_adam(hipStream_t, float *p, float *g, float *m, float *v, int64_t n, float max_norm, float step_size,
                     float bc2_sqrt, float one_minus_beta1, float beta2, float one_minus_beta2, float eps, double *gnorm2);
int launch_clip_adam_pack2(hipStream_t st, const NetLayout *nets, float *const *p, float *const *g, float *const *m, float *const *v,
                           float *const *packed, double *const *gnorm2, const int64_t *n, const float *max_norm,
                           const float *step_size, const float *bc2_sqrt, const float *omb1, const float *beta2, const float *omb2,
                           const float *eps, void *sync_ws = nullptr, const unsigned *const *skip = nullptr);
int launch_adv_stats(hipStream_t st, const int64_t *idx, int64_t n, const float *adv, int64_t ring_base, int64_t ring_cap, float *out,
                     void *ws);
int launch_kl_gate(hipStream_t st, const rlppo_kl_gate_args &a);
int launch_welford(hipStream_t st, const float *x, int64_t ld, int64_t n, int d, void *mean, void *m2, long long count0, int state_f64);
int launch_welford_merge(hipStream_t st, int d, void *mean, void *m2, long long count, const float *omean, const float *om2,
                         long long ocount, int state_f64);
struct GatherMeta {
    const float *actions = nullptr, *old_logp = nullptr, *adv = nullptr, *targets = nullptr;
    float *g_act = nullptr, *g_old = nullptr, *g_adv = nullptr, *g_tgt = nullptr, *zero_n = nullptr;
    int act_dim = 0;
};
int launch_gather_rows(hipStream_t st, const float *src, int64_t ld_src, const int64_t *idx, float *dst, int width, int64_t n,
                       int64_t ring_base = 0, int64_t ring_cap = INT64_MAX, const GatherMeta *meta = nullptr);
int launch_gather_meta(hipStream_t st, const int64_t *idx, const float *actions, int act_dim, const float *old_logp,
                       const float *adv, const float *targets, float *g_act, float *g_old, float *g_adv, float *g_tgt, int64_t n,
                       int64_t ring_base, int64_t ring_cap, unsigned *rowtab = nullptr, float *zero_n = nullptr);
int launch_i64_to_f32(hipStream_t st, const int64_t *src, float *dst, int64_t n);
int launch_learn_report(hipStream_t st, const rlppo_report_args &r);
int launch_signal_words(hipStream_t st, unsigned *words, int count, unsigned value);
int launch_pad_rows(hipStream_t, const void *, int, int64_t, int64_t, int64_t, float *, int64_t, int, float, float);
int launch_pad_rows_vec(hipStream_t, const void *, int, int64_t, int64_t, int64_t, float *, int64_t, const float *, const float *);

}
```

### rlgym_ppo_amd/csrc/gemm.hip

```cpp
#include "gemm_detail.hpp"

namespace rlppo {

template <int NB, int EPI, int BKT, bool BITS = false, bool GATHER = false>
__global__ __launch_bounds__(256, BKT == 16 ? 4 : 2) void gemm_nt_dma_kernel(const float *__restrict__ A, unsigned lda_b,
                                                                              const float *__restrict__ B, unsigned ldb_b,
                                                                              const float *__restrict__ bias,
                                                                              const float *__restrict__ mask_src,
                                                                              unsigned ldm_b, float *__restrict__ C,
                                                                              unsigned ldc_b, int64_t M, int K,
                                                                              unsigned long long *__restrict__ bits = nullptr,
                                                                              const unsigned *__restrict__ rowtab = nullptr,
                                                                              unsigned src_rows = 0, NtAlt alt = NtAlt{},
                                                                              NtDot dot = NtDot{}, NtDot dot_alt = NtDot{}) {
    constexpr int BN = NB * 16;
    constexpr int CPR = BKT / 4;
    constexpr int RPW = 64 / CPR;
    constexpr int RPP = 4 * RPW;
    constexpr int A_IT = SBM / RPP, B_IT = BN / RPP;
    constexpr int B_REM = BN % RPP;
    static_assert(B_REM % RPW == 0, "the ragged staging pass must be whole wave instructions");
    __shared__ __attribute__((aligned(16))) float lds[2 * SBM * BKT + 2 * BN * BKT];
    float *As = lds;
    float *Bs = lds + 2 * SBM * BKT;

    const int tid = threadIdx.x;
    const int lane = tid & 63, wave = tid >> 6;
    const int wave_u = __builtin_amdgcn_readfirstlane(wave);
    const int r16 = lane & 15, q = lane >> 4;
    int row_tile, col_tile;
    xcd_tile(row_tile, col_tile);
    int nct = gridDim.y;
    bool second = blockIdx.z != 0;
    if (alt.interleave) {
        nct >>= 1;
        second = col_tile >= nct;
        if (second) col_tile -= nct;
    }
    if (second) {
        A = alt.A;
        B = alt.B;
        bias = alt.bias;
        C = alt.C;
        bits = alt.bits;
        dot = dot_alt;
    }
    const int64_t m0 = (int64_t)row_tile * SBM;
    const int n0 = col_tile * BN;
    const int rows_here = (int)((M - m0) < SBM ? (M - m0) : SBM);
    unsigned long long *const bit_word = BITS ? bits + ((size_t)row_tile * nct + col_tile) * 256 + tid : nullptr;
    unsigned long long mask_word = 0;
    if (BITS && EPI == EPI_MASK) mask_word = *bit_word;

    const __amdgpu_buffer_rsrc_t a_rs = GATHER ? __builtin_amdgcn_make_buffer_rsrc(const_cast<float *>(A), (short)lda_b, src_rows, 0x00020000)
                                               : make_rsrc(reinterpret_cast<const char *>(A) + m0 * lda_b,
                                                           (unsigned)(rows_here - 1) * lda_b + (unsigned)K * 4);
    const __amdgpu_buffer_rsrc_t b_rs = make_rsrc(reinterpret_cast<const char *>(B) + (int64_t)n0 * ldb_b,
                                                  (unsigned)(BN - 1) * ldb_b + (unsigned)K * 4);
    const int row_p = wave * RPW + lane / CPR, pch = lane % CPR;
    const int lch = BKT == 32 ? (pch ^ (row_p & 7)) : (pch ^ ((0 - (row_p >> 2)) & 3));
    const unsigned a_off = GATHER ? (unsigned)lch * 16 : (unsigned)row_p * lda_b + lch * 16;
    const unsigned b_off = (unsigned)row_p * ldb_b + lch * 16;
    const unsigned a_step = (unsigned)RPP * lda_b, b_step = (unsigned)RPP * ldb_b;
    unsigned a_row[4];
    static_assert(A_IT <= 4, "a_row");
    if (GATHER) {
        const __amdgpu_buffer_rsrc_t t_rs = make_rsrc(rowtab + m0, (unsigned)rows_here * 4);
#pragma unroll
        for (int i = 0; i < A_IT; ++i) a_row[i] = __builtin_amdgcn_raw_buffer_load_b32(t_rs, (unsigned)(row_p + i * RPP) * 4, 0, 0);
    }

    f32x4 acc[2][NB];
    if (EPI == EPI_MASK) {
#pragma unroll
        for (int i = 0; i < 2; ++i)
#pragma unroll
            for (int j = 0; j < NB; ++j) acc[i][j] = f32x4{0.f, 0.f, 0.f, 0.f};
    } else {
        const __amdgpu_buffer_rsrc_t bias_rs = make_rsrc(bias + n0, BN * 4);
#pragma unroll
        for (int j = 0; j < NB; ++j) {
            acc[0][j] = ldb(bias_rs, (unsigned)(q * 16), j * 64);
            acc[1][j] = acc[0][j];
        }
    }

    auto issue_tile = [&](int buf, unsigned kb) {
        float *Ad = As + buf * SBM * BKT + wave_u * RPW * BKT;
        float *Bd = Bs + buf * BN * BKT + wave_u * RPW * BKT;
#pragma unroll
        for (int i = 0; i < A_IT; ++i) {
            if (GATHER)
                __builtin_amdgcn_struct_ptr_buffer_load_lds(a_rs, Ad + i * RPP * BKT, 16, a_row[i], a_off, kb, 0, 0);
            else
                __builtin_amdgcn_raw_ptr_buffer_load_lds(a_rs, Ad + i * RPP * BKT, 16, a_off, kb + i * a_step, 0, 0);
        }
#pragma unroll
        for (int i = 0; i < B_IT; ++i)
            __builtin_amdgcn_raw_ptr_buffer_load_lds(b_rs, Bd + i * RPP * BKT, 16, b_off, kb + i * b_step, 0, 0);
        if (B_REM != 0 && wave_u * RPW < B_REM)
            __builtin_amdgcn_raw_ptr_buffer_load_lds(b_rs, Bd + B_IT * RPP * BKT, 16, b_off, kb + B_IT * b_step, 0, 0);
    };

    const int nk = K / BKT;
    if (GATHER) asm volatile("s_waitcnt vmcnt(0)" ::: "memory");
    issue_tile(0, 0);
    asm volatile("s_waitcnt vmcnt(0)" ::: "memory");
    __syncthreads();
    for (int kt = 0; kt < nk; ++kt) {
        const int cur = kt & 1;
        if ((kt + 1) < nk) issue_tile(cur ^ 1, (unsigned)(kt + 1) * (BKT * 4));
        const float *Ac = As + cur * SBM * BKT + (wave * 32) * BKT;
        const float *Bc = Bs + cur * BN * BKT;
#pragma unroll
        for (int kc = 0; kc < BKT / 16; ++kc) {
            f32x4 fa[2], fb[NB];
#pragma unroll
            for (int i = 0; i < 2; ++i) fa[i] = *reinterpret_cast<const f32x4 *>(&Ac[dswz<BKT>(i * 16 + r16, kc * 4 + q)]);
#pragma unroll
            for (int j = 0; j < NB; ++j) fb[j] = *reinterpret_cast<const f32x4 *>(&Bc[dswz<BKT>(j * 16 + r16, kc * 4 + q)]);
#pragma unroll
            for (int s = 0; s < 4; ++s)
#pragma unroll
                for (int i = 0; i < 2; ++i)
#pragma unroll
                    for (int j = 0; j < NB; ++j) acc[i][j] = MFMA16(fb[j][s], fa[i][s], acc[i][j]);
        }
        __builtin_amdgcn_sched_barrier(0);
        asm volatile("s_waitcnt vmcnt(0)" ::: "memory");
        __syncthreads();
    }
    char *const park = reinterpret_cast<char *>(lds) + wave_u * 8192;
    if (BITS && EPI == EPI_MASK) {
        apply_bits<NB>(acc, mask_word);
        nt_epilogue<NB, EPI_NONE>(acc, nullptr, 0, C, ldc_b, m0, n0, rows_here, wave, r16, q, park);
    } else if (BITS && EPI == EPI_BIAS_RELU) {
#pragma unroll
        for (int i = 0; i < 2; ++i)
#pragma unroll
            for (int j = 0; j < NB; ++j)
#pragma unroll
                for (int e = 0; e < 4; ++e) acc[i][j][e] = relu1(acc[i][j][e]);
        *bit_word = relu_bits<NB>(acc);
        if (dot.w) {
            const __amdgpu_buffer_rsrc_t w_rs = make_rsrc(dot.w + n0, BN * 4);
            float s0 = 0.f, s1 = 0.f;
#pragma unroll
            for (int j = 0; j < NB; ++j) {
                const f32x4 wv = ldb(w_rs, (unsigned)(q * 16), j * 64);
#pragma unroll
                for (int e = 0; e < 4; ++e) {
                    s0 += acc[0][j][e] * wv[e];
                    s1 += acc[1][j][e] * wv[e];
                }
            }
            s0 += __shfl_xor(s0, 16);
            s1 += __shfl_xor(s1, 16);
            s0 += __shfl_xor(s0, 32);
            s1 += __shfl_xor(s1, 32);
            if (q == 0) {
                const float b0 = col_tile == 0 ? dot.b[0] : 0.f;
                const int r0 = wave * 32 + r16;
                if (r0 < rows_here) atomicAdd(dot.out + m0 + r0, s0 + b0);
                if (r0 + 16 < rows_here) atomicAdd(dot.out + m0 + r0 + 16, s1 + b0);
            }
        }
        nt_epilogue<NB, EPI_NONE>(acc, nullptr, 0, C, ldc_b, m0, n0, rows_here, wave, r16, q, park);
    } else {
        nt_epilogue<NB, EPI>(acc, mask_src, ldm_b, C, ldc_b, m0, n0, rows_here, wave, r16, q, park);
    }
}

__device__ __forceinline__ bf16x8 to_bf16x8(const float *lo, const float *hi) {
    const f32x4 a = *reinterpret_cast<const f32x4 *>(lo), b = *reinterpret_cast<const f32x4 *>(hi);
    bf16x8 r;
#pragma unroll
    for (int e = 0; e < 4; ++e) {
        r[e] = (__bf16)a[e];
        r[4 + e] = (__bf16)b[e];
    }
    return r;
}

template <int NB, int EPI>
__global__ __launch_bounds__(256, 2) void gemm_nt_bf16_kernel(const float *__restrict__ A, unsigned lda_b,
                                                                              const float *__restrict__ B, unsigned ldb_b,
                                                                              const float *__restrict__ bias,
                                                                              const float *__restrict__ mask_src,
                                                                              unsigned ldm_b, float *__restrict__ C,
                                                                              unsigned ldc_b, int64_t M, int K) {
    constexpr int BN = NB * 16;
    constexpr int BKT = 32;
    constexpr int CPR = BKT / 4;
    constexpr int RPW = 64 / CPR;
    constexpr int RPP = 4 * RPW;
    constexpr int A_IT = SBM / RPP, B_IT = BN / RPP;
    static_assert(BN % RPP == 0, "column tile must be a whole number of staging passes");
    __shared__ __attribute__((aligned(16))) float lds[2 * SBM * BKT + 2 * BN * BKT];
    float *As = lds;
    float *Bs = lds + 2 * SBM * BKT;

    const int tid = threadIdx.x;
    const int lane = tid & 63, wave = tid >> 6;
    const int wave_u = __builtin_amdgcn_readfirstlane(wave);
    const int r16 = lane & 15, q = lane >> 4;
    int row_tile, col_tile;
    xcd_tile(row_tile, col_tile);
    const int64_t m0 = (int64_t)row_tile * SBM;
    const int n0 = col_tile * BN;
    const int rows_here = (int)((M - m0) < SBM ? (M - m0) : SBM);

    const __amdgpu_buffer_rsrc_t a_rs = make_rsrc(reinterpret_cast<const char *>(A) + m0 * lda_b,
                                                  (unsigned)(rows_here - 1) * lda_b + (unsigned)K * 4);
    const __amdgpu_buffer_rsrc_t b_rs = make_rsrc(reinterpret_cast<const char *>(B) + (int64_t)n0 * ldb_b,
                                                  (unsigned)(BN - 1) * ldb_b + (unsigned)K * 4);
    const int row_p = wave * RPW + lane / CPR, pch = lane % CPR;
    const int lch = BKT == 32 ? (pch ^ (row_p & 7)) : (pch ^ ((0 - (row_p >> 2)) & 3));
    const unsigned a_off = (unsigned)row_p * lda_b + lch * 16;
    const unsigned b_off = (unsigned)row_p * ldb_b + lch * 16;
    const unsigned a_step = (unsigned)RPP * lda_b, b_step = (unsigned)RPP * ldb_b;

    f32x4 acc[2][NB];
    if (EPI == EPI_MASK) {
#pragma unroll
        for (int i = 0; i < 2; ++i)
#pragma unroll
            for (int j = 0; j < NB; ++j) acc[i][j] = f32x4{0.f, 0.f, 0.f, 0.f};
    } else {
        const __amdgpu_buffer_rsrc_t bias_rs = make_rsrc(bias + n0, BN * 4);
#pragma unroll
        for (int j = 0; j < NB; ++j) {
            acc[0][j] = ldb(bias_rs, (unsigned)(q * 16), j * 64);
            acc[1][j] = acc[0][j];
        }
    }

    auto issue_tile = [&](int buf, unsigned kb) {
        float *Ad = As + buf * SBM * BKT + wave_u * RPW * BKT;
        float *Bd = Bs + buf * BN * BKT + wave_u * RPW * BKT;
#pragma unroll
        for (int i = 0; i < A_IT; ++i)
            __builtin_amdgcn_raw_ptr_buffer_load_lds(a_rs, Ad + i * RPP * BKT, 16, a_off, kb + i * a_step, 0, 0);
#pragma unroll
        for (int i = 0; i < B_IT; ++i)
            __builtin_amdgcn_raw_ptr_buffer_load_lds(b_rs, Bd + i * RPP * BKT, 16, b_off, kb + i * b_step, 0, 0);
    };

    const int nk = K / BKT;
    issue_tile(0, 0);
    asm volatile("s_waitcnt vmcnt(0)" ::: "memory");
    __syncthreads();
    for (int kt = 0; kt < nk; ++kt) {
        const int cur = kt & 1;
        if ((kt + 1) < nk) issue_tile(cur ^ 1, (unsigned)(kt + 1) * (BKT * 4));
        const float *Ac = As + cur * SBM * BKT + (wave * 32) * BKT;
        const float *Bc = Bs + cur * BN * BKT;
        bf16x8 fa[2], fb[NB];
#pragma unroll
        for (int i = 0; i < 2; ++i) fa[i] = to_bf16x8(&Ac[dswz<32>(i * 16 + r16, 2 * q)], &Ac[dswz<32>(i * 16 + r16, 2 * q + 1)]);
#pragma unroll
        for (int j = 0; j < NB; ++j) fb[j] = to_bf16x8(&Bc[dswz<32>(j * 16 + r16, 2 * q)], &Bc[dswz<32>(j * 16 + r16, 2 * q + 1)]);
#pragma unroll
        for (int i = 0; i < 2; ++i)
#pragma unroll
            for (int j = 0; j < NB; ++j) acc[i][j] = __builtin_amdgcn_mfma_f32_16x16x32_bf16(fb[j], fa[i], acc[i][j], 0, 0, 0);
        __builtin_amdgcn_sched_barrier(0);
        asm volatile("s_waitcnt vmcnt(0)" ::: "memory");
        __syncthreads();
    }
    nt_epilogue<NB, EPI>(acc, mask_src, ldm_b, C, ldc_b, m0, n0, rows_here, wave, r16, q);
}

template <int NB>
static int launch_nt_1(hipStream_t st, dim3 grid, int epi, const float *A, unsigned lda_b, const float *B, unsigned ldb_b,
                       const float *bias, const float *mask_src, unsigned ldm_b, float *C, unsigned ldc_b, int64_t M,
                       int K) {
    constexpr int BKT = (NB * 16) % 32 == 0 && NB * 16 >= 64 ? 16 : 32;
    if (BKT == 32 && K % 32 != 0) {
        if (epi == EPI_BIAS_RELU || epi == EPI_BIAS || epi == EPI_BIAS_TANH || epi == EPI_MASK) {
#define NT16(E)                                                                                                         \
    case E:                                                                                                            \
        hipLaunchKernelGGL((gemm_nt_dma_kernel<NB, E, 16>), grid, dim3(256), 0, st, A, lda_b, B, ldb_b, bias, mask_src,  \
                           ldm_b, C, ldc_b, M, K);                                                                     \
        break;
            switch (epi) { NT16(EPI_BIAS) NT16(EPI_BIAS_RELU) NT16(EPI_BIAS_TANH) NT16(EPI_MASK) }
#undef NT16
            RLPPO_LAUNCH_CHECK();
            return 0;
        }
    }
#define NT(E)                                                                                                          \
    case E:                                                                                                            \
        hipLaunchKernelGGL((gemm_nt_dma_kernel<NB, E, BKT>), grid, dim3(256), 0, st, A, lda_b, B, ldb_b, bias, mask_src, \
                           ldm_b, C, ldc_b, M, K);                                                                     \
        break;
    switch (epi) {
        NT(EPI_BIAS) NT(EPI_BIAS_RELU) NT(EPI_BIAS_TANH) NT(EPI_MASK)
        default:
            set_error("gemm_nt: bad epilogue %d", epi);
            return RLPPO_ERR_ARG;
    }
#undef NT
    RLPPO_LAUNCH_CHECK();
    return 0;
}

namespace {
constexpr int SK_AHEAD = 8;
constexpr int64_t SK_MAX_ROWS = 1024;
int g_nt_skinny = 1;
}
void set_nt_skinny(int on) { g_nt_skinny = on; }

template <int EPI>
__global__ __launch_bounds__(256) void gemm_nt_skinny_kernel(const float *__restrict__ A, int64_t lda, const float *__restrict__ B, int64_t ldb,
                                                             const float *__restrict__ bias, float *__restrict__ C, int64_t ldc, int64_t M, int N,
                                                             int K) {
    const int lane = threadIdx.x & 63, wave = threadIdx.x >> 6;
    const int r16 = lane & 15, q = lane >> 4;
    const int n0 = ((int)blockIdx.x * 4 + wave) * 16;
    if (n0 >= N) return;
    const int64_t m0 = (int64_t)blockIdx.y * 16;
    const int64_t arow = m0 + r16 < M ? m0 + r16 : M - 1;
    const float *ap = A + arow * lda + q * 4;
    const float *bp = B + (int64_t)(n0 + r16) * ldb + q * 4;
    f32x4 acc = *reinterpret_cast<const f32x4 *>(bias + n0 + q * 4);
    const int nk = K / 16;
    f32x4 fa[2][SK_AHEAD], fb[2][SK_AHEAD];
    auto fetch = [&](int buf, int kt0) {
#pragma unroll
        for (int i = 0; i < SK_AHEAD; ++i) {
            const int kt = kt0 + i < nk ? kt0 + i : nk - 1;
            fa[buf][i] = *reinterpret_cast<const f32x4 *>(ap + kt * 16);
            fb[buf][i] = *reinterpret_cast<const f32x4 *>(bp + kt * 16);
        }
    };
    fetch(0, 0);
    for (int kt0 = 0; kt0 < nk; kt0 += 2 * SK_AHEAD) {
        fetch(1, kt0 + SK_AHEAD);
#pragma unroll
        for (int i = 0; i < SK_AHEAD; ++i)
            if (kt0 + i < nk) {
#pragma unroll
                for (int s = 0; s < 4; ++s) acc = MFMA16(fb[0][i][s], fa[0][i][s], acc);
            }
        fetch(0, kt0 + 2 * SK_AHEAD);
#pragma unroll
        for (int i = 0; i < SK_AHEAD; ++i)
            if (kt0 + SK_AHEAD + i < nk) {
#pragma unroll
                for (int s = 0; s < 4; ++s) acc = MFMA16(fb[1][i][s], fa[1][i][s], acc);
            }
    }
#pragma unroll
    for (int e = 0; e < 4; ++e) {
        if (EPI == EPI_BIAS_RELU) acc[e] = relu1(acc[e]);
        if (EPI == EPI_BIAS_TANH) acc[e] = tanhf(acc[e]);
    }
    if (m0 + r16 < M) *reinterpret_cast<f32x4 *>(C + (m0 + r16) * ldc + n0 + q * 4) = acc;
}

static int launch_gemm_nt_skinny(hipStream_t st, const float *A, int64_t lda, const float *B, int64_t ldb, const float *bias, float *C,
                                 int64_t ldc, int64_t M, int N, int K, int epi) {
    dim3 grid((unsigned)cdiv(N, 64), (unsigned)cdiv(M, 16));
#define SK(E)                                                                                                              \
    case E:                                                                                                                \
        hipLaunchKernelGGL((gemm_nt_skinny_kernel<E>), grid, dim3(256), 0, st, A, lda, B, ldb, bias, C, ldc, M, N, K);      \
        break;
    switch (epi) {
        SK(EPI_BIAS) SK(EPI_BIAS_RELU) SK(EPI_BIAS_TANH)
        default:
            set_error("gemm_nt (few rows): bad epilogue %d", epi);
            return RLPPO_ERR_ARG;
    }
#undef SK
    RLPPO_LAUNCH_CHECK();
    return 0;
}

static int g_infer_bf16 = 0;
void set_infer_bf16(int v) { g_infer_bf16 = v; }
int get_infer_bf16() { return g_infer_bf16; }

template <int NB>
static int launch_bf16_1(hipStream_t st, dim3 grid, int epi, const float *A, unsigned lda_b, const float *B, unsigned ldb_b,
                         const float *bias, float *C, unsigned ldc_b, int64_t M, int K) {
#define BF(E)                                                                                                          \
    case E:                                                                                                            \
        hipLaunchKernelGGL((gemm_nt_bf16_kernel<NB, E>), grid, dim3(256), 0, st, A, lda_b, B, ldb_b, bias, nullptr, 0u, C, \
                           ldc_b, M, K);                                                                               \
        break;
    switch (epi) {
        BF(EPI_BIAS) BF(EPI_BIAS_RELU) BF(EPI_BIAS_TANH)
        default:
            set_error("gemm_nt (bf16 operands): epilogue %d is not a forward epilogue", epi);
            return RLPPO_ERR_ARG;
    }
#undef BF
    RLPPO_LAUNCH_CHECK();
    return 0;
}

int launch_gemm_nt_bf16(hipStream_t st, const float *A, int64_t lda, const float *B, int64_t ldb, const float *bias, float *C,
                        int64_t ldc, int64_t M, int N, int nb, int K, int epi) {
    dim3 grid((unsigned)cdiv(M, SBM), (unsigned)(N / (nb * 16)));
    const unsigned la = (unsigned)(lda * 4), lb = (unsigned)(ldb * 4), lc = (unsigned)(ldc * 4);
    switch (nb) {
        case 8: return launch_bf16_1<8>(st, grid, epi, A, la, B, lb, bias, C, lc, M, K);
        case 6: return launch_bf16_1<6>(st, grid, epi, A, la, B, lb, bias, C, lc, M, K);
        case 4: return launch_bf16_1<4>(st, grid, epi, A, la, B, lb, bias, C, lc, M, K);
        default: return launch_bf16_1<2>(st, grid, epi, A, la, B, lb, bias, C, lc, M, K);
    }
}

size_t nt_bits_floats(int64_t M, int N) {
    if (N % 128 != 0 || M <= 0) return 0;
    return (size_t)cdiv(M, SBM) * (size_t)(N / 128) * 256 * 2;
}
static int g_pair_interleave = 1;
void set_pair_interleave(int v) { g_pair_interleave = v; }
bool nt_gather_ok(int64_t lda, int64_t src_rows, int N, int K) {
    return N % 128 == 0 && K % 16 == 0 && lda * 4 < 16384 && lda % 4 == 0 && src_rows > 0 && src_rows < ((int64_t)1 << 32);
}
int launch_gemm_nt_bits(hipStream_t st, const float *A, int64_t lda, const float *B, int64_t ldb, const float *bias, float *C,
                        int64_t ldc, int64_t M, int N, int K, int epi, unsigned long long *bits, const unsigned *rowtab,
                        int64_t src_rows, const NtAlt *alt, const NtDot *dot) {
    if (!bits || N % 128 != 0 || K % 16 != 0 || M <= 0) return -1;
    if (epi != EPI_BIAS_RELU && epi != EPI_MASK) return -1;
    const int64_t lim = (int64_t)1 << 31;
    if ((!rowtab && 129 * lda * 4 >= lim) || 129 * ldb * 4 >= lim || 129 * ldc * 4 >= lim) return -1;
    RLPPO_CHECK_ARG(!alt || (alt->A && alt->B && alt->C && alt->bits), "gemm_nt: incomplete second operand set");
    dim3 grid((unsigned)cdiv(M, SBM), (unsigned)(N / 128), alt ? 2u : 1u);
    NtAlt second = alt ? *alt : NtAlt{};
    if (alt && g_pair_interleave) {
        grid.y *= 2;
        grid.z = 1;
        second.interleave = 1;
    }
    const NtDot d0 = dot ? dot[0] : NtDot{}, d1 = dot && alt ? dot[1] : NtDot{};
    RLPPO_CHECK_ARG(!dot || (epi == EPI_BIAS_RELU && N / 128 <= 2 && (!d0.w || (d0.out && d0.b)) && (!d1.w || (d1.out && d1.b))),
                    "gemm_nt: the folded one-output head needs the ReLU forward form and at most two column tiles");
    const unsigned la = (unsigned)(lda * 4), lb = (unsigned)(ldb * 4), lc = (unsigned)(ldc * 4);
    if (rowtab) {
        RLPPO_CHECK_ARG(epi == EPI_BIAS_RELU && nt_gather_ok(lda, src_rows, N, K), "gemm_nt (gathered rows): unsupported shape");
        hipLaunchKernelGGL((gemm_nt_dma_kernel<8, EPI_BIAS_RELU, 16, true, true>), grid, dim3(256), 0, st, A, la, B, lb, bias, nullptr,
                           0u, C, lc, M, K, bits, rowtab, (unsigned)src_rows, second, d0, d1);
    } else if (epi == EPI_BIAS_RELU)
        hipLaunchKernelGGL((gemm_nt_dma_kernel<8, EPI_BIAS_RELU, 16, true>), grid, dim3(256), 0, st, A, la, B, lb, bias, nullptr,
                           0u, C, lc, M, K, bits, nullptr, 0u, second, d0, d1);
    else
        hipLaunchKernelGGL((gemm_nt_dma_kernel<8, EPI_MASK, 16, true>), grid, dim3(256), 0, st, A, la, B, lb, nullptr, nullptr, 0u,
                           C, lc, M, K, bits, nullptr, 0u, second);
    RLPPO_LAUNCH_CHECK();
    return 0;
}

int launch_gemm_nt(hipStream_t st, const float *A, int64_t lda, const float *B, int64_t ldb, const float *bias,
                   const float *mask_src, int64_t ld_mask, float *C, int64_t ldc, int64_t M, int N, int K, int epi,
                   int bf16_operands) {
    if (M <= 0) return 0;
    RLPPO_CHECK_ARG(K > 0 && K % 16 == 0, "gemm_nt: K=%d must be a positive multiple of 16", K);
    RLPPO_CHECK_ARG(lda % 4 == 0 && ldb % 4 == 0 && ldc % 4 == 0 && lda >= K && ldb >= K && ldc >= N,
                    "gemm_nt: leading dimensions lda=%ld ldb=%ld ldc=%ld incompatible with K=%d N=%d", (long)lda,
                    (long)ldb, (long)ldc, K, N);
    RLPPO_CHECK_ARG(epi != EPI_MASK || (mask_src && ld_mask >= N && ld_mask % 4 == 0), "gemm_nt: mask operand missing");
    RLPPO_CHECK_ARG(epi == EPI_MASK || bias, "gemm_nt: bias operand missing");
    int nb;
    if (N % 128 == 0) nb = 8;
    else if (N == 96) nb = 6;
    else if (N == 64) nb = 4;
    else if (N == 32) nb = 2;
    else {
        set_error("gemm_nt: N=%d is not a padded output width", N);
        return RLPPO_ERR_ARG;
    }
    const int64_t lim = (int64_t)1 << 31;
    RLPPO_CHECK_ARG(129 * lda * 4 < lim && 129 * ldb * 4 < lim && 129 * ldc * 4 < lim && 129 * ld_mask * 4 < lim,
                    "gemm_nt: a leading dimension is too wide for 32-bit tile offsets");
    if (bf16_operands && epi != EPI_MASK && K % 32 == 0) return launch_gemm_nt_bf16(st, A, lda, B, ldb, bias, C, ldc, M, N, nb, K, epi);
    if (g_nt_skinny && M <= SK_MAX_ROWS && epi != EPI_MASK && !bf16_operands) return launch_gemm_nt_skinny(st, A, lda, B, ldb, bias, C, ldc, M, N, K, epi);
    dim3 grid((unsigned)cdiv(M, SBM), (unsigned)(N / (nb * 16)));
    const unsigned la = (unsigned)(lda * 4), lb = (unsigned)(ldb * 4), lc = (unsigned)(ldc * 4), lm = (unsigned)(ld_mask * 4);
    switch (nb) {
        case 8: return launch_nt_1<8>(st, grid, epi, A, la, B, lb, bias, mask_src, lm, C, lc, M, K);
        case 6: return launch_nt_1<6>(st, grid, epi, A, la, B, lb, bias, mask_src, lm, C, lc, M, K);
        case 4: return launch_nt_1<4>(st, grid, epi, A, la, B, lb, bias, mask_src, lm, C, lc, M, K);
        default: return launch_nt_1<2>(st, grid, epi, A, la, B, lb, bias, mask_src, lm, C, lc, M, K);
    }
}

namespace {
constexpr int TM = 32;
constexpr unsigned OOR = 0x80000000u;
}

struct TnGeom {
    int ni, nj, wn;
    __host__ __device__ int bnt() const { return wn * ni * 16; }
    __host__ __device__ int bkx() const { return (4 / wn) * nj * 16; }
    __host__ __device__ int tile_floats() const { return ni * nj * 1024; }
};
static TnGeom tn_geometry(int out, int in) {
    if (in > 96 && in <= 112) return TnGeom{2, 7, 4};
    if (out > 64 && out <= 96) return TnGeom{3, 4, 2};
    return TnGeom{4, 4, 2};
}

constexpr int TN_LDS_FLOATS = 2 * 2 * 32 * 128;
template <int TMT, int NI, int NJ, int WN, bool GATHER>
__device__ __forceinline__ void tn_tile(float *lds, const float *__restrict__ dY, unsigned ldy_b, int ny_valid,
                                        const float *__restrict__ X, unsigned ldx_b, int kx_valid, bool with_db, int out, int64_t M,
                                        int rows_per_wg, float *__restrict__ partial, const unsigned *__restrict__ rowtab,
                                        unsigned src_rows, int bx, int by, int bz, int tiles_x, int tiles_y, int splits_z) {
    constexpr int WK = 4 / WN;
    constexpr int BNT = WN * NI * 16, BKX = WK * NJ * 16, TILE_F = NI * NJ * 1024;
    constexpr int PPW = TMT / 8;
    static_assert(2 * 2 * TMT * 128 <= TN_LDS_FLOATS && 8 * 128 <= TN_LDS_FLOATS, "stage buffers");
    float *Ys = lds;
    float *Xs = lds + 2 * TMT * 128;

    const int tid = threadIdx.x;
    const int lane = tid & 63, wave = tid >> 6;
    const int wave_u = __builtin_amdgcn_readfirstlane(wave);
    const int r16 = lane & 15, q = lane >> 4;
    const int wn = wave / WK, wk = wave % WK;
    const int n0 = bx * BNT, k0 = by * BKX;
    const int64_t mbeg = (int64_t)bz * rows_per_wg;
    const int rows = (int)((M - mbeg) < rows_per_wg ? (M - mbeg) : rows_per_wg);
    const int steps = (rows + TMT - 1) / TMT;
    const int rem = rows - (steps - 1) * TMT;
    const int ny_here = (ny_valid - n0) < BNT ? (ny_valid - n0) : BNT;
    const int kx_here = (kx_valid - k0) < BKX ? (kx_valid - k0) : BKX;

    const __amdgpu_buffer_rsrc_t y_rs = make_rsrc(reinterpret_cast<const char *>(dY) + mbeg * ldy_b + (int64_t)n0 * 4,
                                                  (unsigned)(rows - 1) * ldy_b + (unsigned)ny_here * 4);
    const __amdgpu_buffer_rsrc_t x_rs =
        GATHER ? __builtin_amdgcn_make_buffer_rsrc(const_cast<float *>(X), (short)ldx_b, src_rows, 0x00020000)
               : make_rsrc(reinterpret_cast<const char *>(X) + mbeg * ldx_b + (int64_t)k0 * 4,
                           (unsigned)(rows - 1) * ldx_b + (unsigned)kx_here * 4);
    const int row_l = 2 * wave + (lane >> 5);
    const int lch = (lane & 31) ^ ((row_l & 3) << 2);
    const bool x_col = lch * 4 < kx_here;
    const unsigned y_off = (lch * 4 < ny_here) ? (unsigned)row_l * ldy_b + lch * 16 : OOR;
    const unsigned x_off = GATHER ? (unsigned)(k0 * 4 + lch * 16) : (x_col ? (unsigned)row_l * ldx_b + lch * 16 : OOR);
    const unsigned y_row8 = 8u * ldy_b, x_row8 = 8u * ldx_b, y_stage = TMT * ldy_b, x_stage = TMT * ldx_b;
    unsigned x_row[4];
    static_assert(PPW <= 4, "x_row");
    const __amdgpu_buffer_rsrc_t t_rs = make_rsrc(GATHER ? rowtab + mbeg : nullptr, GATHER ? (unsigned)rows * 4 : 0u);
    auto load_rows = [&](int stage) {
        if (GATHER) {
#pragma unroll
            for (int i = 0; i < PPW; ++i)
                x_row[i] = __builtin_amdgcn_raw_buffer_load_b32(t_rs, (unsigned)row_l * 4, (unsigned)(stage * TMT + 8 * i) * 4, 0);
        }
    };

    auto issue_stage = [&](int buf, int stage) {
        float *Yd = Ys + (buf * TMT + 2 * wave_u) * 128, *Xd = Xs + (buf * TMT + 2 * wave_u) * 128;
#pragma unroll
        for (int i = 0; i < PPW; ++i) {
            __builtin_amdgcn_raw_ptr_buffer_load_lds(y_rs, Yd + 8 * i * 128, 16, y_off, (unsigned)stage * y_stage + i * y_row8, 0, 0);
            if (GATHER) {
                if (x_col) __builtin_amdgcn_struct_ptr_buffer_load_lds(x_rs, Xd + 8 * i * 128, 16, x_row[i], x_off, 0, 0, 0);
            } else {
                __builtin_amdgcn_raw_ptr_buffer_load_lds(x_rs, Xd + 8 * i * 128, 16, x_off, (unsigned)stage * x_stage + i * x_row8, 0, 0);
            }
        }
    };
    const int zr = tid >> 5, zc = (tid & 31) * 4;
    auto clear_tail = [&](int buf) {
        const f32x4 z = f32x4{0.f, 0.f, 0.f, 0.f};
        for (int r = rem + zr; r < TMT; r += 8) {
            *reinterpret_cast<f32x4 *>(&Ys[(buf * TMT + r) * 128 + zc]) = z;
            *reinterpret_cast<f32x4 *>(&Xs[(buf * TMT + r) * 128 + zc]) = z;
        }
    };

    f32x4 acc[NI][NJ], acc2[NI][NJ];
#pragma unroll
    for (int i = 0; i < NI; ++i)
#pragma unroll
        for (int j = 0; j < NJ; ++j) acc[i][j] = acc2[i][j] = f32x4{0.f, 0.f, 0.f, 0.f};
    f32x4 bs4 = f32x4{0.f, 0.f, 0.f, 0.f};
    const bool want_db = with_db && by == 0;

    load_rows(0);
    if (GATHER) asm volatile("s_waitcnt vmcnt(0)" ::: "memory");
    issue_stage(0, 0);
    if (steps > 1) load_rows(1);
    asm volatile("s_waitcnt vmcnt(0)" ::: "memory");
    if (steps == 1 && rem < TMT) clear_tail(0);
    __syncthreads();
    int fy[NI], fx[NJ];
#pragma unroll
    for (int i = 0; i < NI; ++i) {
        const int g = wn * NI + i;
        fy[i] = q * 128 + (((g & ~3) | ((g & 3) ^ q)) << 4) + r16;
    }
#pragma unroll
    for (int j = 0; j < NJ; ++j) {
        const int g = wk * NJ + j;
        fx[j] = q * 128 + (((g & ~3) | ((g & 3) ^ q)) << 4) + r16;
// ... 490 lines not shown
```

### rlgym_ppo_amd/csrc/heads.hip

```cpp
#include <type_traits>

#include "common.hpp"

namespace rlppo {

constexpr float PROB_MIN = 1e-11f;

__device__ __forceinline__ float wave_max(float v) {
#pragma unroll
    for (int o = 32; o > 0; o >>= 1) v = fmaxf(v, __shfl_xor(v, o));
    return v;
}
__device__ __forceinline__ float wave_sum(float v) {
#pragma unroll
    for (int o = 32; o > 0; o >>= 1) v += __shfl_xor(v, o);
    return v;
}

template <int CTRL>
__device__ __forceinline__ float dpp_mov(float v) {
    return __builtin_bit_cast(float, __builtin_amdgcn_update_dpp(0, __builtin_bit_cast(int, v), CTRL, 0xF, 0xF, true));
}
__device__ __forceinline__ float row16_sum(float v) {
    v += dpp_mov<0xB1>(v);
// ... 184 lines not shown
static int launch_discrete_sample(hipStream_t st, const float *src, int64_t ld, int64_t n, int A, const float *noise,
                                  int64_t *actions, float *logp, float *probs_out, const unsigned *mask = nullptr, int W = 0) {
    if (n <= 0) return 0;
    if (FROM_PROBS) mask = nullptr;
    RLPPO_CHECK_ARG(!mask || W == (A + 31) / 32, "discrete head: mask_words=%d, n_actions=%d needs %d", W, A, (A + 31) / 32);
    return dispatch_discrete(A, mask != nullptr, [&](auto epl, auto masked) {
        hipLaunchKernelGGL((discrete_sample_kernel<decltype(epl)::value, FROM_PROBS, !FROM_PROBS && decltype(masked)::value>), dim3((unsigned)cdiv(n, 4)), dim3(256), 0, st, src,
                           ld, n, A, noise, actions, logp, probs_out, mask, W);
    });
}

int launch_discrete_sample_logits(hipStream_t st, const float *logits, int64_t ld, int64_t n, int A, const float *noise,
                                  int64_t *actions, float *logp, float *probs_out, const unsigned *mask, int mask_words) {
    return launch_discrete_sample<false>(st, logits, ld, n, A, noise, actions, logp, probs_out, mask, mask_words);
}
int launch_categorical_select(hipStream_t st, const float *probs, int64_t ld, int64_t n, int A, const float *noise,
                              int64_t *actions, float *logp) {
    return launch_discrete_sample<true>(st, probs, ld, n, A, noise, actions, logp, nullptr);
}

template <int EPL, bool MASKED>
__global__ __launch_bounds__(256) void discrete_probs_kernel(const float *__restrict__ logits, int64_t ld, int64_t n, int A,
                                                              int clamp, float *__restrict__ probs, int64_t ld_p,
                                                              unsigned long long *__restrict__ key,
                                                              const unsigned *__restrict__ mask, int W) {
    typedef WaveRow<EPL> L;
    const L lay;
    const int64_t row = (int64_t)blockIdx.x * L::ROWS + lay.group;
    if (row >= n) return;
    float p[EPL], pc[EPL];
    unsigned valid = 0;
    if (MASKED) valid = lay.valid_bits(mask + row * W, A);
    const auto in = [&](int e) { return MASKED ? ((valid >> e) & 1u) != 0 : lay.col(e) < A; };
    lay.load(logits + row * ld, ld, p, in);
    softmax_clamp<L>(p, pc, in);
    float best = -1.f;
    int besti = 0x7fffffff;
#pragma unroll
    for (int e = 0; e < EPL; ++e) {
        const int c = lay.col(e);
        if (probs && c < A) probs[row * ld_p + c] = in(e) ? (clamp ? pc[e] : p[e]) : 0.f;
        if (in(e) && pc[e] > best) {
            best = pc[e];
            besti = c;
        }
    }
    if (!key) return;
#pragma unroll
    for (int o = 32; o > 0; o >>= 1) {
        const float ov = __shfl_xor(best, o);
        const int oi = __shfl_xor(besti, o);
        if (ov > best || (ov == best && oi < besti)) {
            best = ov;
            besti = oi;
        }
    }
    if (lay.writer()) {
        const unsigned long long flat = (unsigned long long)(row * A + besti);
        atomicMax(key, ((unsigned long long)__float_as_uint(best) << 32) | (0xffffffffull - flat));
    }
}
__global__ void decode_flat_argmax_kernel(unsigned long long *key) {
    *(long long *)key = (long long)(0xffffffffull - (*key & 0xffffffffull));
}

int launch_discrete_probs(hipStream_t st, const float *logits, int64_t ld, int64_t n, int A, int clamp, float *probs,
                          int64_t ld_p, int64_t *flat_argmax, const unsigned *mask, int W) {
    if (n <= 0) return 0;
    RLPPO_CHECK_ARG(!mask || W == (A + 31) / 32, "discrete head: mask_words=%d, n_actions=%d needs %d", W, A, (A + 31) / 32);
    if (flat_argmax && (unsigned long long)n * (unsigned long long)A > 0xffffffffull) {
        set_error("discrete_probs: n * n_actions exceeds the 32-bit flat index of the arg-max key");
        return RLPPO_ERR_ARG;
    }
    unsigned long long *key = (unsigned long long *)flat_argmax;
    if (key) RLPPO_HIP(hipMemsetAsync(key, 0, sizeof(*key), st));
    const int rc = dispatch_discrete(A, mask != nullptr, [&](auto epl, auto masked) {
        hipLaunchKernelGGL((discrete_probs_kernel<decltype(epl)::value, decltype(masked)::value>), dim3((unsigned)cdiv(n, 4)), dim3(256), 0, st, logits, ld, n, A, clamp, probs,
                           ld_p, key, mask, W);
    });
    if (rc) return rc;
    if (key) {
        hipLaunchKernelGGL(decode_flat_argmax_kernel, dim3(1), dim3(1), 0, st, key);
        RLPPO_LAUNCH_CHECK();
    }
    return 0;
}

__device__ __forceinline__ float surrogate_weight(float ratio, float adv, const LossCfg &c, float &s_min) {
    const float s1 = ratio * adv;
    const float cl = fminf(fmaxf(ratio, c.clip_lo), c.clip_hi);
    const float s2 = cl * adv;
    const float inr = (ratio >= c.clip_lo && ratio <= c.clip_hi) ? 1.f : 0.f;
    s_min = fminf(s1, s2);
    return s1 < s2 ? 1.f : (s1 > s2 ? inr : 0.5f + 0.5f * inr);
}

__device__ __forceinline__ float surrogate_adv(float adv, const LossCfg &c) { return c.adv_norm ? (adv - c.adv_norm[0]) * c.adv_norm[1] : adv; }

struct Surrogate {
    float lr, ratio, smin, g_logp;
};
__device__ __forceinline__ Surrogate surrogate_row(float lp, float old_logp, float stored_adv, const LossCfg &c) {
    const float adv = surrogate_adv(stored_adv, c);
    Surrogate t;
    t.lr = lp - old_logp;
    t.ratio = expf(t.lr);
    const float w = surrogate_weight(t.ratio, adv, c, t.smin);
    t.g_logp = c.mb_ratio * (-(adv * w * t.ratio) * c.inv_mb);
    return t;
}
__device__ __forceinline__ void surrogate_stats_add(float (&st)[5], float entropy, const Surrogate &t, const LossCfg &c) {
    st[RLPPO_STAT_ENTROPY] += entropy;
    st[RLPPO_STAT_KL] += ((t.ratio - 1.f) - t.lr) * c.inv_mb;
    st[RLPPO_STAT_CLIPFRAC] += (fabsf(t.ratio - 1.f) > c.clip ? 1.f : 0.f) * c.inv_mb;
    st[RLPPO_STAT_PLOSS] += -t.smin * c.inv_mb;
}

__device__ __forceinline__ void block_stats_add(double *stats, const float (&v)[5], bool active, const LossCfg &c,
                                                double *kl_slots = nullptr) {
    __shared__ float red[5][4];
    const int lane = threadIdx.x & 63, wave = threadIdx.x >> 6;
#pragma unroll
    for (int k = 0; k < 5; ++k) {
        float x = wave_sum(active ? v[k] : 0.f);
        if (lane == 0) red[k][wave] = x;
    }
    __syncthreads();
    if (threadIdx.x < 5) {
        const int k = threadIdx.x;
        const double s = (double)red[k][0] + (double)red[k][1] + (double)red[k][2] + (double)red[k][3];
        if (k == RLPPO_STAT_KL && kl_slots) {
            kl_slots[2 + blockIdx.x] = s;
            if (blockIdx.x == 0) {
                kl_slots[0] = (double)gridDim.x;
                kl_slots[1] = (double)c.mb_ratio;
            }
        }
        if (!(c.stop_word && *c.stop_word)) atomicAdd(stats + k, s);
    }
}

constexpr int64_t DISCRETE_LOSS_MAX_BLOCKS = 2048;
static unsigned discrete_loss_grid(int64_t mb, int rows_per_block) {
    const int64_t g = cdiv(mb, rows_per_block);
    return (unsigned)(g < DISCRETE_LOSS_MAX_BLOCKS ? g : DISCRETE_LOSS_MAX_BLOCKS);
}
static unsigned thread_per_row_grid(int64_t mb) { return (unsigned)cdiv(mb, 256); }
int64_t kl_slots_doubles(int64_t mb) {
    const int64_t g = thread_per_row_grid(mb > 0 ? mb : 1);
    return 2 + (g > DISCRETE_LOSS_MAX_BLOCKS ? g : DISCRETE_LOSS_MAX_BLOCKS);
}

__device__ __forceinline__ float value_row(float *vout_row, float target, float adv, const LossCfg &c) {
    const float v = vout_row[0];
    if (c.vclip > 0.f) {
        const float v_old = target - adv;
        const float dv = v - v_old;
        const float d = (v_old + fminf(fmaxf(dv, -c.vclip), c.vclip)) - target;
        vout_row[0] = fabsf(dv) <= c.vclip ? c.mb_ratio * (2.f * d * c.inv_mb) : 0.f;
        return d * d;
    }
    const float d = v - target;
    vout_row[0] = c.mb_ratio * (2.f * d * c.inv_mb);
    return d * d;
}

template <class L, bool MASKED>
__global__ __launch_bounds__(256) void discrete_loss_kernel(float *__restrict__ logits, int64_t ld, int A,
                                                             const float *__restrict__ actions,
                                                             const float *__restrict__ old_logp,
                                                             const float *__restrict__ advantages, int64_t mb,
                                                             LossCfg cfg, double *__restrict__ stats, MaskRows mr) {
    constexpr int EPL = L::EPL;
    const L lay;
    float st[5] = {0.f, 0.f, 0.f, 0.f, 0.f};
    for (int64_t base = (int64_t)blockIdx.x * L::ROWS; base < mb; base += (int64_t)gridDim.x * L::ROWS) {
        const bool live = base + lay.group < mb;
        if (!L::SHADOW && !live) break;
        const int64_t row = live ? base + lay.group : mb - 1;
        float *z = logits + row * ld;
        unsigned valid = 0;
        if (MASKED) valid = lay.valid_bits(mr.mask + ring_row(mr.idx[row], mr.ring_base, mr.ring_cap) * mr.W, A);
        const auto in = [&](int e) { return MASKED ? ((valid >> e) & 1u) != 0 : lay.col(e) < A; };
        float p[EPL], pc[EPL], lp[EPL];
        lay.load(z, ld, p, in);
        softmax_clamp<L>(p, pc, in);
        const int a = (int)actions[row];
        float ent = 0.f, lpa = 0.f, pca = 0.f;
#pragma unroll
        for (int e = 0; e < EPL; ++e) {
            lp[e] = in(e) ? logf(pc[e]) : 0.f;
            if (in(e)) ent -= lp[e] * pc[e];
            if (lay.col(e) == a) {
                lpa = MASKED && !in(e) ? logf(pc[e]) : lp[e];
                pca = pc[e];
            }
        }
        ent = L::sum(ent);
        lpa = L::sum(lpa);
        pca = L::sum(pca);
        const Surrogate t = surrogate_row(lpa, old_logp[row], advantages[row], cfg);
        const float g_ent = cfg.mb_ratio * (cfg.ent_coef * cfg.inv_mb);
        float g[EPL];
        float dot = 0.f;
#pragma unroll
        for (int e = 0; e < EPL; ++e) {
            g[e] = 0.f;
            if (in(e)) {
                g[e] = g_ent * (lp[e] + 1.f);
                if (lay.col(e) == a) g[e] += t.g_logp / pca;
                if (!(p[e] >= PROB_MIN)) g[e] = 0.f;
            }
            dot += g[e] * p[e];
        }
        dot = L::sum(dot);
#pragma unroll
        for (int e = 0; e < EPL; ++e) g[e] = in(e) ? p[e] * (g[e] - dot) : 0.f;
        if (live) lay.store(z, ld, g);
        if (live && lay.writer()) surrogate_stats_add(st, ent * cfg.inv_mb, t, cfg);
    }
    block_stats_add(stats, st, true, cfg, cfg.kl_slots);
}

__global__ __launch_bounds__(256) void value_loss_kernel(float *__restrict__ vout, int64_t ldv, const float *__restrict__ targets,
                                                         const float *__restrict__ advantages, int64_t mb, LossCfg cfg,
                                                         double *__restrict__ stats) {
    float st[5] = {0.f, 0.f, 0.f, 0.f, 0.f};
    for (int64_t row = (int64_t)blockIdx.x * 256 + threadIdx.x; row < mb; row += (int64_t)gridDim.x * 256)
        st[RLPPO_STAT_VLOSS] += value_row(vout + row * ldv, targets[row], cfg.vclip > 0.f ? advantages[row] : 0.f, cfg) * cfg.inv_mb;
    block_stats_add(stats, st, true, cfg);
}

int launch_value_loss(hipStream_t st, float *vout, int64_t ldv, const float *targets, const float *adv, int64_t mb, const LossCfg &cfg,
                      double *stats) {
    if (mb <= 0) return 0;
    RLPPO_CHECK_ARG(!(cfg.vclip > 0.f) || adv, "value loss: clipping needs the advantages");
    dim3 grid((unsigned)(cdiv(mb, 256) < 1024 ? cdiv(mb, 256) : 1024));
    hipLaunchKernelGGL(value_loss_kernel, grid, dim3(256), 0, st, vout, ldv, targets, adv, mb, cfg, stats);
    RLPPO_LAUNCH_CHECK();
    return 0;
}

int launch_discrete_loss(hipStream_t st, float *logits, int64_t ld, int A, const float *actions, const float *old_logp, const float *adv,
                         int64_t mb, const LossCfg &cfg, double *stats, const MaskRows *mr) {
    if (mb <= 0) return 0;
    RLPPO_CHECK_ARG(ld <= DISCRETE_LOSS_MAX_LD, "discrete head: padded width %ld too large", (long)ld);
    const bool masked = mr && mr->mask;
    RLPPO_CHECK_ARG(!masked || (mr->W == (A + 31) / 32 && mr->idx), "discrete head: mask_words=%d, n_actions=%d needs %d", mr->W, A, (A + 31) / 32);
    return dispatch_discrete((int)ld, masked, [&](auto epl, auto is_masked) {
        typedef std::conditional_t<decltype(epl)::value == 2, Lanes16, WaveRow<decltype(epl)::value>> L;
        hipLaunchKernelGGL((discrete_loss_kernel<L, decltype(is_masked)::value>), dim3(discrete_loss_grid(mb, L::ROWS)), dim3(256), 0, st, logits, ld, A, actions,
                           old_logp, adv, mb, cfg, stats, masked ? *mr : MaskRows{});
    });
}

constexpr int FLOAT_SUM_K = 32;

__device__ __forceinline__ float gauss_logpdf(float x, float mean, float sd) {
    const float msq = mean * mean, ssq = sd * sd, xsq = x * x;
    const float t1 = -(msq / (2.f * ssq));
    const float t2 = (mean * x) / ssq;
    const float t3 = -(xsq / (2.f * ssq));
    const float t4 = logf(1.f / sqrtf((float)(2.0 * 3.14159265358979323846) * ssq));
    return t1 + t2 + t3 + t4;
}

__device__ __forceinline__ void block_done_words(unsigned *done_words, unsigned done_value, int64_t n) {
    if (!done_words) return;
    __builtin_amdgcn_fence(__ATOMIC_RELEASE, "");
    __syncthreads();
    const int64_t w = (int64_t)blockIdx.x * 16 + threadIdx.x;
    if (threadIdx.x < 16 && w < (n + 15) / 16) __hip_atomic_store(done_words + w, done_value, __ATOMIC_RELEASE, __HIP_MEMORY_SCOPE_SYSTEM);
}

__global__ __launch_bounds__(256) void gaussian_sample_kernel(const float *__restrict__ y, int64_t ld, int64_t n, int k,
                                                               const float *__restrict__ eps, float var_m, float var_b,
                                                               float *__restrict__ actions, float *__restrict__ logp,
                                                               unsigned *done_words, unsigned done_value) {
    const int64_t row = (int64_t)blockIdx.x * blockDim.x + threadIdx.x;
    if (row < n) {
        const float *yr = y + row * ld;
        float lp = 0.f;
        double lpd = 0.0;
        for (int j = 0; j < k; ++j) {
            const float mean = yr[j];
            const float sd = yr[k + j] * var_m + var_b;
            float a = eps[row * k + j] * sd + mean;
            a = fminf(fmaxf(a, -1.f), 1.f);
            actions[row * k + j] = a;
            if (k <= FLOAT_SUM_K)
                lp += gauss_logpdf(a, mean, sd);
            else
                lpd += (double)gauss_logpdf(a, mean, sd);
        }
        logp[row] = k <= FLOAT_SUM_K ? lp : (float)lpd;
    }
    block_done_words(done_words, done_value, n);
}

int launch_gaussian_sample(hipStream_t st, const float *y, int64_t ld, int64_t n, int k, const float *eps, float var_m,
                           float var_b, float *actions, float *logp, unsigned *done_words, unsigned done_value) {
    if (n <= 0) return 0;
    hipLaunchKernelGGL(gaussian_sample_kernel, dim3((unsigned)cdiv(n, 256)), dim3(256), 0, st, y, ld, n, k, eps, var_m,
                       var_b, actions, logp, done_words, done_value);
    RLPPO_LAUNCH_CHECK();
    return 0;
}

__global__ __launch_bounds__(256) void gaussian_loss_kernel(float *__restrict__ y, int64_t ld, int k,
                                                             const float *__restrict__ actions,
                                                             const float *__restrict__ old_logp,
                                                             const float *__restrict__ advantages, int64_t mb,
                                                             LossCfg cfg, double *__restrict__ stats) {
    const int64_t row = (int64_t)blockIdx.x * blockDim.x + threadIdx.x;
    const bool active = row < mb;
    float st[5] = {0.f, 0.f, 0.f, 0.f, 0.f};
    if (active) {
// ... 347 lines not shown
```

### rlgym_ppo_amd/csrc/optim.hip

```cpp
#include <atomic>

#include "common.hpp"

namespace rlppo {

struct PackJob {
    int in, out, pin, pout;
    int64_t off_w, off_wt, off_b, off_flat_w, off_flat_b;
    int64_t first;
};
struct PackJobs {
    int n;
    PackJob j[RLPPO_MAX_LAYERS];
    int64_t total;
};

__global__ __launch_bounds__(256) void pack_kernel(const float *__restrict__ flat, float *__restrict__ packed, PackJobs jobs) {
    for (int64_t g = (int64_t)blockIdx.x * blockDim.x + threadIdx.x; g < jobs.total; g += (int64_t)gridDim.x * blockDim.x) {
        int l = 0;
        while (l + 1 < jobs.n && g >= jobs.j[l + 1].first) ++l;
        const PackJob &J = jobs.j[l];
        const int64_t e = g - J.first;
        const int o = (int)(e / J.pin), i = (int)(e % J.pin);
        const float w = (o < J.out && i < J.in) ? flat[J.off_flat_w + (int64_t)o * J.in + i] : 0.f;
// ... 20 lines not shown
}

__device__ __forceinline__ unsigned short bf16_bits(float x) { return __builtin_bit_cast(unsigned short, (__bf16)x); }
__global__ __launch_bounds__(256) void pack_bf16_kernel(const float *__restrict__ flat, float *__restrict__ packed_r,
                                                        unsigned short *__restrict__ wb16, PackJobs jobs) {
    for (int64_t g = (int64_t)blockIdx.x * blockDim.x + threadIdx.x; g < jobs.total; g += (int64_t)gridDim.x * blockDim.x) {
        int l = 0;
        while (l + 1 < jobs.n && g >= jobs.j[l + 1].first) ++l;
        const PackJob &J = jobs.j[l];
        const int64_t e = g - J.first;
        const int o = (int)(e / J.pin), i = (int)(e % J.pin);
        const float w = (o < J.out && i < J.in) ? flat[J.off_flat_w + (int64_t)o * J.in + i] : 0.f;
        const unsigned short h = bf16_bits(w);
        const float wr = __uint_as_float((unsigned)h << 16);
        packed_r[J.off_w + (int64_t)o * J.pin + i] = wr;
        packed_r[J.off_wt + (int64_t)i * J.pout + o] = wr;
        wb16[J.first + e] = h;
        wb16[jobs.total + J.first + (int64_t)i * J.pout + o] = h;
        if (i == 0) packed_r[J.off_b + o] = o < J.out ? flat[J.off_flat_b + o] : 0.f;
    }
}

int launch_pack_bf16(hipStream_t st, const NetLayout &net, const float *flat, float *packed_r, unsigned short *wb16) {
    PackJobs jobs;
    jobs.n = net.n_layers;
    int64_t tot = 0;
    for (int l = 0; l < net.n_layers; ++l) {
        const LayerLayout &L = net.L[l];
        jobs.j[l] = PackJob{L.in, L.out, L.pin, L.pout, L.off_w, L.off_wt, L.off_b, L.off_flat_w, L.off_flat_b, tot};
        tot += (int64_t)L.pin * L.pout;
    }
    jobs.total = tot;
    const int blocks = (int)(cdiv(tot, 256) < 2048 ? cdiv(tot, 256) : 2048);
    hipLaunchKernelGGL(pack_bf16_kernel, dim3(blocks), dim3(256), 0, st, flat, packed_r, wb16, jobs);
    RLPPO_LAUNCH_CHECK();
    return 0;
}

__global__ __launch_bounds__(256) void round_rows_kernel(float *__restrict__ x, unsigned short *__restrict__ xb, int64_t n4) {
    typedef float f32x4 __attribute__((ext_vector_type(4)));
    typedef unsigned short u16x4 __attribute__((ext_vector_type(4)));
    for (int64_t g = (int64_t)blockIdx.x * blockDim.x + threadIdx.x; g < n4; g += (int64_t)gridDim.x * blockDim.x) {
        f32x4 v = reinterpret_cast<f32x4 *>(x)[g];
        u16x4 h;
#pragma unroll
        for (int e = 0; e < 4; ++e) {
            const float f = v[e];
            h[e] = bf16_bits(f);
            v[e] = __uint_as_float((unsigned)h[e] << 16);
        }
        reinterpret_cast<f32x4 *>(x)[g] = v;
        reinterpret_cast<u16x4 *>(xb)[g] = h;
    }
}

int launch_round_rows(hipStream_t st, float *x, unsigned short *xb, int64_t n_elems) {
    if (n_elems <= 0) return 0;
    RLPPO_CHECK_ARG(n_elems % 4 == 0, "round_rows: element count %ld is not a multiple of 4", (long)n_elems);
    const int64_t n4 = n_elems / 4;
    const int blocks = (int)(cdiv(n4, 256) < 8192 ? cdiv(n4, 256) : 8192);
    hipLaunchKernelGGL(round_rows_kernel, dim3(blocks), dim3(256), 0, st, x, xb, n4);
    RLPPO_LAUNCH_CHECK();
    return 0;
}

__global__ __launch_bounds__(256) void expand_rows_kernel(const unsigned short *__restrict__ xb, float *__restrict__ x, int64_t n4) {
    typedef float f32x4 __attribute__((ext_vector_type(4)));
    typedef unsigned short u16x4 __attribute__((ext_vector_type(4)));
    for (int64_t g = (int64_t)blockIdx.x * blockDim.x + threadIdx.x; g < n4; g += (int64_t)gridDim.x * blockDim.x) {
        const u16x4 h = reinterpret_cast<const u16x4 *>(xb)[g];
        f32x4 v;
#pragma unroll
        for (int e = 0; e < 4; ++e) v[e] = __uint_as_float((unsigned)h[e] << 16);
        reinterpret_cast<f32x4 *>(x)[g] = v;
    }
}

int launch_expand_rows(hipStream_t st, const unsigned short *xb, float *x, int64_t n_elems) {
    if (n_elems <= 0) return 0;
    RLPPO_CHECK_ARG(n_elems % 4 == 0, "expand_rows: element count %ld is not a multiple of 4", (long)n_elems);
    const int64_t n4 = n_elems / 4;
    const int blocks = (int)(cdiv(n4, 256) < 8192 ? cdiv(n4, 256) : 8192);
    hipLaunchKernelGGL(expand_rows_kernel, dim3(blocks), dim3(256), 0, st, xb, x, n4);
    RLPPO_LAUNCH_CHECK();
    return 0;
}

__global__ __launch_bounds__(256) void i64_to_f32_kernel(const int64_t *__restrict__ src, float *__restrict__ dst, int64_t n) {
    const int64_t i = (int64_t)blockIdx.x * 256 + threadIdx.x;
    if (i < n) dst[i] = (float)src[i];
}
__global__ void signal_words_kernel(unsigned *__restrict__ words, int count, unsigned value) {
    __builtin_amdgcn_fence(__ATOMIC_RELEASE, "");
    for (int i = threadIdx.x; i < count; i += blockDim.x) __hip_atomic_store(words + i, value, __ATOMIC_RELEASE, __HIP_MEMORY_SCOPE_SYSTEM);
}
int launch_signal_words(hipStream_t st, unsigned *words, int count, unsigned value) {
    if (count <= 0) return 0;
    hipLaunchKernelGGL(signal_words_kernel, dim3(1), dim3(64), 0, st, words, count, value);
    RLPPO_LAUNCH_CHECK();
    return 0;
}
int launch_i64_to_f32(hipStream_t st, const int64_t *src, float *dst, int64_t n) {
    if (n <= 0) return 0;
    hipLaunchKernelGGL(i64_to_f32_kernel, dim3((unsigned)cdiv(n, 256)), dim3(256), 0, st, src, dst, n);
    RLPPO_LAUNCH_CHECK();
    return 0;
}

template <typename T>
__global__ __launch_bounds__(256) void pad_rows_kernel(const T *__restrict__ src, int64_t n, int64_t d, int64_t ld_src,
                                                        float *__restrict__ dst, int64_t ld_dst, int standardize,
                                                        float mean0, float std0) {
    const int64_t total = n * ld_dst;
    for (int64_t g = (int64_t)blockIdx.x * blockDim.x + threadIdx.x; g < total; g += (int64_t)gridDim.x * blockDim.x) {
        const int64_t r = g / ld_dst, c = g % ld_dst;
        float v = 0.f;
        if (c < d) {
            v = (float)src[r * ld_src + c];
            if (standardize) v = fminf(fmaxf((v - mean0) / std0, -5.f), 5.f);
        }
        dst[g] = v;
    }
}

template <typename T>
__global__ __launch_bounds__(256) void pad_rows_vec_kernel(const T *__restrict__ src, int64_t n, int64_t d, int64_t ld_src,
                                                            float *__restrict__ dst, int64_t ld_dst,
                                                            const float *__restrict__ mean, const float *__restrict__ stdv) {
    const int64_t total = n * ld_dst;
    for (int64_t g = (int64_t)blockIdx.x * blockDim.x + threadIdx.x; g < total; g += (int64_t)gridDim.x * blockDim.x) {
        const int64_t r = g / ld_dst, c = g % ld_dst;
        float v = 0.f;
        if (c < d) v = fminf(fmaxf(((float)src[r * ld_src + c] - mean[c]) / stdv[c], -5.f), 5.f);
        dst[g] = v;
    }
}

__global__ __launch_bounds__(256) void gather_rows_kernel(const float *__restrict__ src, int64_t ld_src,
                                                          const int64_t *__restrict__ idx, float *__restrict__ dst,
                                                          int chunks_per_row, int64_t n, int64_t ring_base, int64_t ring_cap, GatherMeta meta) {
    typedef float f32x4 __attribute__((ext_vector_type(4)));
    const int64_t t = (int64_t)blockIdx.x * 256 + threadIdx.x;
    const int64_t row = t / chunks_per_row;
    const int c = (int)(t - row * chunks_per_row);
    if (row >= n) return;
    const int64_t srow = ring_row(idx[row], ring_base, ring_cap);
    const f32x4 v = __builtin_nontemporal_load(reinterpret_cast<const f32x4 *>(src + srow * ld_src) + c);
    reinterpret_cast<f32x4 *>(dst)[t] = v;
    if (c == 0 && meta.g_old) {
        meta.g_old[row] = meta.old_logp[srow];
        meta.g_adv[row] = meta.adv[srow];
        meta.g_tgt[row] = meta.targets[srow];
        for (int k = 0; k < meta.act_dim; ++k) meta.g_act[row * meta.act_dim + k] = meta.actions[srow * meta.act_dim + k];
        if (meta.zero_n) meta.zero_n[row] = 0.f;
    }
}

__global__ __launch_bounds__(256) void gather_rows_round_kernel(const float *__restrict__ src, int64_t ld_src,
                                                                const int64_t *__restrict__ idx, float *__restrict__ dst,
                                                                unsigned short *__restrict__ dstb, int chunks_per_row, int64_t n,
                                                                int64_t ring_base, int64_t ring_cap) {
    typedef float f32x4 __attribute__((ext_vector_type(4)));
    typedef unsigned short u16x4 __attribute__((ext_vector_type(4)));
    const int64_t t = (int64_t)blockIdx.x * 256 + threadIdx.x;
    const int64_t row = t / chunks_per_row;
    const int c = (int)(t - row * chunks_per_row);
    if (row >= n) return;
    f32x4 v = __builtin_nontemporal_load(reinterpret_cast<const f32x4 *>(src + ring_row(idx[row], ring_base, ring_cap) * ld_src) + c);
    u16x4 h;
#pragma unroll
    for (int e = 0; e < 4; ++e) {
        const float f = v[e];
        h[e] = bf16_bits(f);
        v[e] = __uint_as_float((unsigned)h[e] << 16);
    }
    if (dst) reinterpret_cast<f32x4 *>(dst)[t] = v;
    reinterpret_cast<u16x4 *>(dstb)[t] = h;
}

int launch_gather_rows_round(hipStream_t st, const float *src, int64_t ld_src, const int64_t *idx, float *dst, unsigned short *dstb,
                             int width, int64_t n, int64_t ring_base, int64_t ring_cap) {
    if (n <= 0) return 0;
    RLPPO_CHECK_ARG(width > 0 && width % 4 == 0 && ld_src >= width && ld_src % 4 == 0, "gather_rows: width=%d ld=%ld", width,
                    (long)ld_src);
    const int cpr = width / 4;
    hipLaunchKernelGGL(gather_rows_round_kernel, dim3((unsigned)cdiv(n * cpr, 256)), dim3(256), 0, st, src, ld_src, idx, dst, dstb,
                       cpr, n, ring_base, ring_cap);
    RLPPO_LAUNCH_CHECK();
    return 0;
}

__global__ __launch_bounds__(256) void gather_meta_kernel(const int64_t *__restrict__ idx, const float *__restrict__ actions,
                                                          int act_dim, const float *__restrict__ old_logp,
                                                          const float *__restrict__ adv, const float *__restrict__ targets,
                                                          float *__restrict__ g_act, float *__restrict__ g_old,
                                                          float *__restrict__ g_adv, float *__restrict__ g_tgt, int64_t n,
                                                          int64_t ring_base, int64_t ring_cap, unsigned *__restrict__ rowtab,
                                                          float *__restrict__ zero_n) {
    const int64_t r = (int64_t)blockIdx.x * 256 + threadIdx.x;
    if (r >= n) return;
    const int64_t src = ring_row(idx[r], ring_base, ring_cap);
    if (rowtab) rowtab[r] = (unsigned)src;
    if (zero_n) zero_n[r] = 0.f;
    g_old[r] = old_logp[src];
    g_adv[r] = adv[src];
    g_tgt[r] = targets[src];
    for (int k = 0; k < act_dim; ++k) g_act[r * act_dim + k] = actions[src * act_dim + k];
}

int launch_gather_meta(hipStream_t st, const int64_t *idx, const float *actions, int act_dim, const float *old_logp,
                       const float *adv, const float *targets, float *g_act, float *g_old, float *g_adv, float *g_tgt, int64_t n,
                       int64_t ring_base, int64_t ring_cap, unsigned *rowtab, float *zero_n) {
    if (n <= 0) return 0;
    hipLaunchKernelGGL(gather_meta_kernel, dim3((unsigned)cdiv(n, 256)), dim3(256), 0, st, idx, actions, act_dim, old_logp, adv,
                       targets, g_act, g_old, g_adv, g_tgt, n, ring_base, ring_cap, rowtab, zero_n);
    RLPPO_LAUNCH_CHECK();
    return 0;
}

int launch_gather_rows(hipStream_t st, const float *src, int64_t ld_src, const int64_t *idx, float *dst, int width,
                       int64_t n, int64_t ring_base, int64_t ring_cap, const GatherMeta *meta) {
    if (n <= 0) return 0;
    RLPPO_CHECK_ARG(width > 0 && width % 4 == 0 && ld_src >= width && ld_src % 4 == 0, "gather_rows: width=%d ld=%ld", width,
                    (long)ld_src);
    const int cpr = width / 4;
    hipLaunchKernelGGL(gather_rows_kernel, dim3((unsigned)cdiv(n * cpr, 256)), dim3(256), 0, st, src, ld_src, idx, dst, cpr, n, ring_base,
                       ring_cap, meta ? *meta : GatherMeta{});
    RLPPO_LAUNCH_CHECK();
    return 0;
}

template <typename T>
__global__ __launch_bounds__(128) void welford_kernel(const float *__restrict__ x, int64_t ld, int64_t n, int d,
                                                      T *__restrict__ mean, T *__restrict__ m2, long long count0) {
    const int f = blockIdx.x * 128 + threadIdx.x;
    if (f >= d) return;
    T mu = mean[f], v = m2[f];
    constexpr int PF = 16;
    int64_t i = 0;
    for (; i + PF <= n; i += PF) {
        float xs[PF];
#pragma unroll
        for (int u = 0; u < PF; ++u) xs[u] = x[(i + u) * ld + f];
#pragma unroll
        for (int u = 0; u < PF; ++u) {
            const long long prev = count0 + i + u;
            const T cnt = (T)(prev + 1);
            const T delta = (T)xs[u] - mu;
            const T dn = delta / cnt;
            mu += dn;
            v += (delta * dn) * (T)prev;
        }
    }
    for (; i < n; ++i) {
        const long long prev = count0 + i;
        const T cnt = (T)(prev + 1);
        const T delta = (T)x[i * ld + f] - mu;
        const T dn = delta / cnt;
        mu += dn;
        v += (delta * dn) * (T)prev;
    }
    mean[f] = mu;
    m2[f] = v;
}

int launch_welford(hipStream_t st, const float *x, int64_t ld, int64_t n, int d, void *mean, void *m2, long long count0,
                   int state_f64) {
    if (n <= 0 || d <= 0) return 0;
    if (state_f64)
        hipLaunchKernelGGL(welford_kernel<double>, dim3((unsigned)cdiv(d, 128)), dim3(128), 0, st, x, ld, n, d, (double *)mean,
                           (double *)m2, count0);
    else
        hipLaunchKernelGGL(welford_kernel<float>, dim3((unsigned)cdiv(d, 128)), dim3(128), 0, st, x, ld, n, d, (float *)mean,
                           (float *)m2, count0);
    RLPPO_LAUNCH_CHECK();
    return 0;
}

template <typename T>
__global__ __launch_bounds__(128) void welford_merge_kernel(int d, T *__restrict__ mean, T *__restrict__ m2, long long count,
                                                            const float *__restrict__ omean, const float *__restrict__ om2,
                                                            long long ocount) {
    const int f = blockIdx.x * 128 + threadIdx.x;
    if (f >= d) return;
    const T c = (T)count, oc = (T)ocount, tot = (T)(count + ocount);
    const T mu = mean[f], om = (T)omean[f];
    const T delta = om - mu;
    const T dsq = delta * delta;
    const T oterm = (T)((float)ocount * omean[f]);
    mean[f] = (c * mu + oterm) / tot;
    m2[f] = (m2[f] + (T)om2[f]) + ((dsq * c) * oc) / tot;
}

int launch_welford_merge(hipStream_t st, int d, void *mean, void *m2, long long count, const float *omean, const float *om2,
                         long long ocount, int state_f64) {
    if (d <= 0 || ocount == 0) return 0;
    if (state_f64)
        hipLaunchKernelGGL(welford_merge_kernel<double>, dim3((unsigned)cdiv(d, 128)), dim3(128), 0, st, d, (double *)mean,
                           (double *)m2, count, omean, om2, ocount);
    else
        hipLaunchKernelGGL(welford_merge_kernel<float>, dim3((unsigned)cdiv(d, 128)), dim3(128), 0, st, d, (float *)mean,
                           (float *)m2, count, omean, om2, ocount);
    RLPPO_LAUNCH_CHECK();
    return 0;
}

int launch_pad_rows(hipStream_t st, const void *src, int is_f64, int64_t n, int64_t d, int64_t ld_src, float *dst,
                    int64_t ld_dst, int standardize, float mean0, float std0) {
    if (n <= 0) return 0;
    const int64_t total = n * ld_dst;
    const int blocks = (int)(cdiv(total, 256) < 4096 ? cdiv(total, 256) : 4096);
    if (is_f64)
        hipLaunchKernelGGL(pad_rows_kernel<double>, dim3(blocks), dim3(256), 0, st, (const double *)src, n, d, ld_src, dst,
                           ld_dst, standardize, mean0, std0);
    else
        hipLaunchKernelGGL(pad_rows_kernel<float>, dim3(blocks), dim3(256), 0, st, (const float *)src, n, d, ld_src, dst,
                           ld_dst, standardize, mean0, std0);
    RLPPO_LAUNCH_CHECK();
    return 0;
}

int launch_pad_rows_vec(hipStream_t st, const void *src, int is_f64, int64_t n, int64_t d, int64_t ld_src, float *dst,
                        int64_t ld_dst, const float *mean, const float *stdv) {
    if (n <= 0) return 0;
    const int64_t total = n * ld_dst;
    const int blocks = (int)(cdiv(total, 256) < 4096 ? cdiv(total, 256) : 4096);
    if (is_f64)
        hipLaunchKernelGGL(pad_rows_vec_kernel<double>, dim3(blocks), dim3(256), 0, st, (const double *)src, n, d, ld_src, dst,
                           ld_dst, mean, stdv);
    else
        hipLaunchKernelGGL(pad_rows_vec_kernel<float>, dim3(blocks), dim3(256), 0, st, (const float *)src, n, d, ld_src, dst,
                           ld_dst, mean, stdv);
    RLPPO_LAUNCH_CHECK();
    return 0;
}

__global__ __launch_bounds__(256) void sqnorm_kernel(const float *__restrict__ g, int64_t n, double *__restrict__ out) {
    double acc = 0.0;
    for (int64_t i = (int64_t)blockIdx.x * blockDim.x + threadIdx.x; i < n; i += (int64_t)gridDim.x * blockDim.x) {
        const double v = (double)g[i];
        acc += v * v;
    }
#pragma unroll
    for (int o = 32; o > 0; o >>= 1) acc += __shfl_xor(acc, o);
    __shared__ double red[4];
    if ((threadIdx.x & 63) == 0) red[threadIdx.x >> 6] = acc;
    __syncthreads();
    if (threadIdx.x == 0) atomicAdd(out, red[0] + red[1] + red[2] + red[3]);
}

__global__ __launch_bounds__(256) void adam_kernel(float *__restrict__ p, float *__restrict__ g, float *__restrict__ m,
                                                    float *__restrict__ v, int64_t n, const double *__restrict__ gnorm2,
                                                    float max_norm, float step_size, float bc2_sqrt, float omb1,
                                                    float beta2, float omb2, float eps) {
    const float total = (float)sqrt(*gnorm2);
    float coef = max_norm / (total + 1e-6f);
    coef = coef > 1.f ? 1.f : coef;
    for (int64_t i = (int64_t)blockIdx.x * blockDim.x + threadIdx.x; i < n; i += (int64_t)gridDim.x * blockDim.x) {
        const float gi = g[i] * coef;
        g[i] = gi;
        float mi = m[i], vi = v[i];
        mi = mi + omb1 * (gi - mi);
        vi = vi * beta2 + (omb2 * gi) * gi;
        const float denom = sqrtf(vi) / bc2_sqrt + eps;
        p[i] = p[i] + (-step_size * mi) / denom;
        m[i] = mi;
        v[i] = vi;
    }
// ... 478 lines not shown
```

### rlgym_ppo_amd/ppo/_mlp.py

```python
import ctypes
import math
import os

import numpy as np
import torch
import torch.nn as nn

from .. import _native as N
from ..engine import NetArena, linears_of, ptr, require_gpu, selection_epoch, stream_ptr
from ..util import action_mask as AM


def build_body(input_shape, layer_sizes, n_out, final_activation=None):
    assert len(layer_sizes) != 0, "AT LEAST ONE LAYER MUST BE SPECIFIED TO BUILD THE NEURAL NETWORK!"
    layers = [nn.Linear(int(input_shape), int(layer_sizes[0])), nn.ReLU()]
    prev = int(layer_sizes[0])
    for size in layer_sizes[1:]:
        layers.append(nn.Linear(prev, int(size)))
        layers.append(nn.ReLU())
        prev = int(size)
    layers.append(nn.Linear(prev, int(n_out)))
    if final_activation is not None:
        layers.append(final_activation)
    return nn.Sequential(*layers)


class _WindowRows:

    def __init__(self, address, n, ld):
        self.shape, self._address = (n, ld), address

    def data_ptr(self):
        return self._address


class ActGraph:

    def __init__(self, pol, cap, masked=False):
        a = pol.arena
        dev, d = a.device, a.d_in
        self.cap = cap
        self.masked = bool(masked)
        raw = getattr(pol, "_act_launch_raw", None)
        if masked and raw is None and not getattr(pol, "_masked_chain", False):
            raise ValueError("ActGraph: a masked graph needs the one-launch step of the discrete head or the masked general kernel of "
                             "the multi-discrete head (%s has neither)" % type(pol).__name__)
        self.mask_words = AM.Layout.of(pol).words if masked else 0
        self.mask_pin = None
        self.mask_rows = None
        self.dev = dev
        self.obs_pin = torch.zeros(cap, d).pin_memory()
        self.q_pin = torch.ones(pol._noise_shape(cap)).pin_memory()
        self.rows = torch.zeros(cap, a.ld_in, device=dev)
        self.act_pin = pol._action_buffer(cap).zero_().pin_memory()
        self.logp_pin = torch.zeros(cap, dtype=torch.float32).pin_memory()
        L = N.lib()
        ws_bytes = max(int(L.rlppo_forward_workspace_bytes(a.dims_c, a.n_layers, cap)), raw(None, cap) if raw is not None else 0)
        self.ws = torch.empty(ws_bytes, dtype=torch.uint8, device=dev)

        self.n_done = int(L.rlppo_act_done_words(cap))
        self.done_pin = torch.zeros(max(self.n_done, 1), dtype=torch.int32).pin_memory()
        self.opts = N.ActOpts(N.PRECISION_DEFAULT, 1, self.done_pin.data_ptr())
        self.calls = self.polled = self.poll_timeouts = self.late_retries = self.stale_relaunches = 0
        self.graph_value = 1
        self.window = None
        self.obs_arg, self.q_arg = self.obs_pin.data_ptr(), self.q_pin.data_ptr()
        self.push = os.environ.get("RLPPO_ACT_PUSH", "1") != "0"
        if self.push:
            r256 = lambda x: (x + 255) // 256 * 256
            self.padded = raw is None
            obs_bytes, q_bytes = r256(cap * (a.ld_in if self.padded else d) * 4), r256(int(self.q_pin.numel()) * 4)
            mask_bytes = r256(cap * self.mask_words * 4)
            win = ctypes.c_void_p()
            with torch.cuda.device(dev):
                rc_win = L.rlppo_host_window_alloc(256 + obs_bytes + q_bytes + mask_bytes, ctypes.byref(win))
            if rc_win == 0:
                self.window = win.value
                self.ctl_arg, self.obs_arg, self.q_arg = win.value, win.value + 256, win.value + 256 + obs_bytes
                self.mask_arg = win.value + 256 + obs_bytes + q_bytes
                self._push, self._stage, self._stage_rows = L.rlppo_host_push, L.rlppo_host_stage_call, L.rlppo_host_stage_rows
                self._flush = L.rlppo_host_window_flush
                if self.padded:
                    self.rows = _WindowRows(self.obs_arg, cap, a.ld_in)
            else:
                self.push = False
        self.padded = self.push and raw is None
        if masked:
            valid = torch.full((cap, self.mask_words), -1, dtype=torch.int32)
            if self.push:
                N.check(self._push(self.mask_arg, valid.data_ptr(), 4 * valid.numel(), None, 0))
                self._flush(self.window)
            else:
                self.mask_pin = valid.pin_memory()
                self.mask_arg = self.mask_pin.data_ptr()
            if raw is not None:
                self.opts.action_mask, self.opts.mask_words = self.mask_arg, self.mask_words
            else:
                self.mask_rows = _WindowRows(self.mask_arg, cap, self.mask_words)
        self.late = bool(self.push and raw is not None and cap <= 256)
        if self.late:
            self.opts.noise_ctl = self.ctl_arg
            self.late = L.rlppo_discrete_step_one_launch(a.dims_c, a.n_layers, cap, ctypes.byref(self.opts)) == 1
            if not self.late:
                self.opts.noise_ctl = None
        if self.late:
            self.noise_seq = 0
        self.q_per_row = int(self.q_pin.numel()) // cap

        self._raw, self._pol = raw, pol
        body = self.body
        chain_masked = self.masked and raw is None
        side = torch.cuda.Stream(dev)
        side.wait_stream(torch.cuda.current_stream(dev))
        with torch.cuda.stream(side):
            body()
        side.synchronize()
        self.graph = torch.cuda.CUDAGraph()
        with torch.cuda.graph(self.graph, capture_error_mode="thread_local"):
            body()
        self._count = None
        if chain_masked:
            N.check(L.rlppo_dbg_count(6, -2))
            self._count = L.rlppo_dbg_count
        self.obs_np, self.q_np = self.obs_pin.numpy(), self.q_pin.view(-1).numpy()
        self.act_np, self.logp_np = self.act_pin.numpy(), self.logp_pin.numpy()
        self.done_np = self.done_pin.numpy()
        self.mask_np = self.mask_pin.numpy() if self.mask_pin is not None else None
        self._done_ptr = ctypes.c_void_p(self.done_pin.data_ptr())
        self._wait = L.rlppo_host_wait_words

    def __del__(self):
        win, self.window = getattr(self, "window", None), None
        if win:
            try:
                torch.cuda.synchronize(self.dev)
                with torch.cuda.device(self.dev):
                    N.lib().rlppo_host_window_free(ctypes.c_void_p(win))
            except Exception:
                pass

    def read_control_words(self):
        out = np.zeros(32, dtype=np.uint32)
        torch.cuda.synchronize(self.dev)
        ctypes.memmove(out.ctypes.data, self.ctl_arg, 128)
        return out

    def body(self):
        pol, a, cap = self._pol, self._pol.arena, self.cap
        if self._raw is not None:
            self._raw(self, cap, self.opts)
            return
        if not self.padded:
            N.check(N.lib().rlppo_pad_rows(stream_ptr(), ptr(self.obs_arg), 0, cap, a.d_in, a.d_in, ptr(self.rows), a.ld_in, 0, 0.0, 1.0))
        pol._act_launch(self.rows, cap, self.q_arg, self.act_pin, self.logp_pin, self.ws, self.opts, self.mask_rows)

    def run(self, obs, q, n, draw=None, verify=None, mask_words=None):
        m = n * self.q_per_row
        if self.masked:
            if mask_words is None or mask_words.shape != (n, self.mask_words) or mask_words.dtype != np.int32:
                raise ValueError("action mask: expected int32 words [%d, %d]" % (n, self.mask_words))
            if self.push:
                if not mask_words.flags.c_contiguous:
                    mask_words = np.ascontiguousarray(mask_words)
                rc = self._push(self.mask_arg, mask_words.ctypes.data, mask_words.nbytes, None, 0)
                if rc:
                    N.check(rc)
            else:
                self.mask_np[:n] = mask_words
        if self.push:
            if not obs.flags.c_contiguous:
                obs = np.ascontiguousarray(obs)
            if self.late:
                self.noise_seq = self.noise_seq % 0x7FFFFFFF + 1
                rc = self._stage(self.ctl_arg, self.noise_seq, n, self.obs_arg, obs.ctypes.data, obs.nbytes)
            else:
                if q is None:
                    q = draw()
                q = q if q.is_contiguous() else q.contiguous()
                if q.numel() != m or q.dtype != torch.float32:
                    raise ValueError("noise: expected %d float32 numbers" % m)
                rc = self._push(self.q_arg, q.data_ptr(), 4 * m, None, 0)
                if self.padded:
                    d4 = 4 * obs.shape[1]
                    rc = rc or self._stage_rows(None, 0, 0, self.obs_arg, 4 * self.rows.shape[1], obs.ctypes.data, d4, d4, n)
                else:
                    rc = rc or self._stage(None, 0, 0, self.obs_arg, obs.ctypes.data, obs.nbytes)
            if rc:
                N.check(rc)
        else:
            self.obs_np[:n] = obs
            if q is None:
                q = draw()
            self.q_np[:m] = q.reshape(-1).numpy()
        if self.push:
            self._flush(self.window)
        self.calls += 1
        if self._count is not None:
            self._count(6, 1)
        value, count = self._launch(n)
        if self.late:
            try:
                if q is None:
                    q = draw()
                q = q if q.is_contiguous() else q.contiguous()
                if q.numel() != m or q.dtype != torch.float32:
                    raise ValueError("noise: expected %d float32 numbers" % m)
                N.check(self._push(self.q_arg, q.data_ptr(), 4 * m, self.ctl_arg + 8, self.noise_seq))
            except BaseException:
                self._push(None, None, 0, self.ctl_arg + 8, self.noise_seq)
                self._wait(self._done_ptr, count, value, 100000)
                raise
        rc = None
        if verify is not None:
            ok, redo = verify()
            if not ok:
                rc = self._finish(value, count)
                redo()
                self.stale_relaunches += 1
                value, count = self._launch(n)
                rc = None
        if (self._finish(value, count) if rc is None else rc) == 2:
            self.late_retries += 1
            value, count = self._launch(n)
            if self._finish(value, count) != 0:
                raise RuntimeError("rollout step: the kernel gave up on noise that is there (rlppo_act_opts.noise_ctl): sequence %d, "
                                   "completion words %s" % (self.noise_seq, self.done_np.astype(np.uint32).tolist()))
        return torch.from_numpy(self.act_np[:n].copy()), torch.from_numpy(self.logp_np[:n].copy())

    def _launch(self, n):
        self.done_np[:] = 0
        self.graph.replay()
        return self.graph_value, self.n_done

    def _finish(self, value, count):
        rc = self._wait(self._done_ptr, count, value, 2000)
        if rc == 0:
            self.polled += 1
        elif rc == 1:
            self.poll_timeouts += 1
            torch.cuda.current_stream(self.dev).synchronize()
            rc = self._wait(self._done_ptr, count, value, 0) if self.late else 0
        return rc


def _bucket(n):
    if n <= 128:
        return (n + 15) // 16 * 16
    c = 256
    while c < n:
        c *= 2
    return c


class ArenaModule(nn.Module):

    noise_mode = "host"
    mask_layout = None

    def _finish(self, device):
        self.device = device
        dev = require_gpu(device)
        self.model = self.model.to(dev)
        self.arena = NetArena(linears_of(self.model), dev)
        self.act_graphs = True
        self.act_graph_max = 1024
        self._graphs = {}
        self._graph_epoch = -1

    def _graph_act(self, obs, noise, standardize, action_mask=None):
        if not self.act_graphs or standardize is not None or self.noise_mode != "host":
            return None
        if action_mask is not None and (isinstance(action_mask, AM.Packed) or (isinstance(action_mask, torch.Tensor) and action_mask.is_cuda)):
# ... 88 lines not shown
```

Measured before the change: 63.62 million samples/s.

## Fuse critic last hidden layer, value head, value loss and head backward into one kernel

Replaces the earlier fold of the one-output value head into the hidden GEMM epilogue with a dedicated critic-tail kernel. In one launch it computes the last hidden layer, the value output, the value-loss gradient, and the ReLU-masked dx for the preceding layer, followed by one gemv for the head weight gradient. This removes the separate value-loss and head-backward launches, the zeroing of the value buffer, and the side-stream fork/join for the critic head in the paired pass. In exchange it adds a large specialized kernel limited to widths of 128 or 256. The critic tail now runs serially on the main stream instead of overlapping with the policy head. It also disables Python GC while the CUDA graph is captured.

Result: no change. 63.75 million samples/s (median of 5 runs) (+0.2%).

```diff
diff --git a/rlgym_ppo_amd/csrc/api.hip b/rlgym_ppo_amd/csrc/api.hip
--- a/rlgym_ppo_amd/csrc/api.hip
+++ b/rlgym_ppo_amd/csrc/api.hip
@@ -84,7 +84,41 @@
     o->total = off;
 }
 
-static int g_fold_vhead = 1;
+static int g_fuse_tail = 1;
+static std::atomic<long long> g_cnt_tail{0};
+struct CriticTail {
+    const float *tgt, *adv;
+    LossCfg cfg;
+    double *stats;
+    float *h;
+    float *dx;
+    float *dv;
+    float *grad;
+    float *part;
+    size_t part_floats;
+};
+static bool tail_ok(const NetLayout &net) {
+    const int hl = net.n_layers - 1;
+    return g_fuse_tail && hl >= 1 && gemv_head_ok(net.L[hl].out, net.L[hl].pin) && (net.L[hl - 1].pout == 128 || net.L[hl - 1].pout == 256);
+}
+static int critic_tail(hipStream_t st, const NetLayout &net, const float *packed, const float *x, int64_t ldx, int64_t n, const CriticTail &c) {
+    const int hl = net.n_layers - 1;
+    const LayerLayout &L = net.L[hl - 1], &Lh = net.L[hl];
+    NtTail t;
+    t.w = packed + Lh.off_w;
+    t.b = packed + Lh.off_b;
+    t.tgt = c.tgt;
+    t.adv = c.adv;
+    t.h = c.h;
+    t.dx = c.dx;
+    t.dv = c.dv;
+    t.stats = c.stats;
+    t.cfg = c.cfg;
+    int rc = launch_gemm_nt_tail(st, x, ldx, packed + L.off_w, L.pin, packed + L.off_b, n, L.pout, L.pin, t);
+    if (rc) return rc;
+    ++g_cnt_tail;
+    return launch_gemv_dw(st, c.dv, 1, c.h, L.pout, c.grad + Lh.off_flat_w, c.grad + Lh.off_flat_b, Lh.in, Lh.pin, n, c.part, c.part_floats);
+}
 
 struct RowSource {
     const float *x;
@@ -95,7 +129,7 @@
 
 static int forward(hipStream_t st, const NetLayout &net, const float *packed, const RowSource &in, int64_t n, int out_tanh,
                    float *const *acts, int bf16_operands = 0, unsigned long long *const *bits = nullptr, bool *have_bits = nullptr,
-                   bool *head_folded = nullptr, const unsigned short *x3 = nullptr, bool head_prezeroed = false) {
+                   const CriticTail *tail = nullptr, bool *tail_fused = nullptr, const unsigned short *x3 = nullptr) {
     X3Layout xl;
     if (x3) x3_layout(net, &xl);
     if (have_bits)
@@ -103,16 +137,21 @@
     const float *x = in.x;
     int64_t ldx = in.ld;
     const int hl = net.n_layers - 1;
-    bool fold = head_folded && g_fold_vhead && hl >= 1 && !out_tanh && !bf16_operands && bits && bits[hl - 1] &&
-                gemv_head_ok(net.L[hl].out, net.L[hl].pin) && net.L[hl - 1].pout / 128 <= 2;
-    if (x3 && hl >= 1 && xl.fwd[hl - 1] >= 0) fold = false;
-    if (head_folded) *head_folded = false;
+    const bool fuse = tail && !x3 && !bf16_operands && !out_tanh && bits && hl >= 1 && bits[hl - 1] && tail_ok(net) && !(hl == 1 && in.rowtab);
+    if (tail_fused) *tail_fused = false;
     for (int l = 0; l < net.n_layers; ++l) {
         const LayerLayout &L = net.L[l];
         const bool last = l == net.n_layers - 1;
         const int epi = last ? (out_tanh ? EPI_BIAS_TANH : EPI_BIAS) : EPI_BIAS_RELU;
         int rc;
-        if (last && head_folded && *head_folded) break;
+        if (fuse && l == hl - 1) {
+            rc = critic_tail(st, net, packed, x, ldx, n, *tail);
+            if (rc == 0) {
+                *tail_fused = true;
+                break;
+            }
+            if (rc != -1) return rc;
+        }
         if (last && !out_tanh && gemv_head_ok(L.out, L.pin))
             rc = launch_gemv_fwd(st, x, ldx, packed + L.off_w, packed + L.off_b, acts[l], L.pout, n, L.pin, L.pout);
         else {
@@ -121,18 +160,9 @@
                 rc = launch_gemm_nt_split(st, x, ldx, x3 + xl.fwd[l], packed + L.off_b, acts[l], L.pout, n, L.pout, L.pin, 0, bits[l]);
                 if (rc == 0) have_bits[l] = true;
             } else if (!last && bits && bits[l] && !bf16_operands) {
-                NtDot dots[2];
-                const bool fold_here = fold && l == hl - 1;
-                if (fold_here) {
-                    if (!head_prezeroed) RLPPO_HIP(hipMemsetAsync(acts[hl], 0, (size_t)n * sizeof(float), st));
-                    dots[0].w = packed + net.L[hl].off_w;
-                    dots[0].b = packed + net.L[hl].off_b;
-                    dots[0].out = acts[hl];
-                }
                 rc = launch_gemm_nt_bits(st, x, ldx, packed + L.off_w, L.pin, packed + L.off_b, acts[l], L.pout, n, L.pout, L.pin,
-                                         EPI_BIAS_RELU, bits[l], l == 0 ? in.rowtab : nullptr, in.src_rows, nullptr, fold_here ? dots : nullptr);
+                                         EPI_BIAS_RELU, bits[l], l == 0 ? in.rowtab : nullptr, in.src_rows);
                 if (rc == 0) have_bits[l] = true;
-                if (fold_here) *head_folded = rc == 0;
             }
             if (l == 0 && in.rowtab && rc != 0) {
                 if (rc == -1) set_error("forward: the gathered first layer needs the bitmask form");
@@ -808,20 +838,19 @@
 
 static int backward(hipStream_t st, const NetLayout &net, const float *packed, const RowSource &in, int64_t mb, float *const *acts,
                     float *const *dx, float *grad, float *tn_ws, unsigned long long *const *bits, const bool *have_bits,
-                    bool head_folded = false, const unsigned short *x3 = nullptr, DwList *defer = nullptr) {
+                    bool tail_fused = false, const unsigned short *x3 = nullptr, DwList *defer = nullptr) {
     const int last = net.n_layers - 1;
     int rc = 0;
     X3Layout xl;
     if (x3) x3_layout(net, &xl);
-    for (int l = last; l >= 0; --l) {
+    for (int l = tail_fused ? last - 1 : last; l >= 0; --l) {
         const LayerLayout &L = net.L[l];
         const float *dY = l == last ? acts[last] : dx[l];
-        const int64_t ld_hy = head_folded ? 1 : L.pout;
         const RowSource X = l > 0 ? RowSource{acts[l - 1], net.L[l - 1].pout} : in;
         const bool gemv = l == last && l > 0 && gemv_head_ok(L.out, L.pin);
         const size_t floats = tn_layer_floats(net, l, mb, 0);
         if (gemv)
-            rc = launch_gemv_dw(st, dY, ld_hy, X.x, X.ld, grad + L.off_flat_w, grad + L.off_flat_b, L.in, L.pin, mb, tn_ws, floats);
+            rc = launch_gemv_dw(st, dY, L.pout, X.x, X.ld, grad + L.off_flat_w, grad + L.off_flat_b, L.in, L.pin, mb, tn_ws, floats);
         else if (defer)
             defer->add(L, dY, X, grad);
         else
@@ -831,8 +860,8 @@
         if (l == 0) break;
         rc = -1;
         if (gemv) {
-            if (have_bits[l - 1]) rc = launch_gemv_dx_bits(st, dY, ld_hy, packed + L.off_w, bits[l - 1], dx[l - 1], L.pin, L.pin, mb);
-            if (rc == -1) rc = launch_gemv_dx(st, dY, ld_hy, packed + L.off_w, acts[l - 1], L.pin, dx[l - 1], L.pin, L.pin, mb);
+            if (have_bits[l - 1]) rc = launch_gemv_dx_bits(st, dY, L.pout, packed + L.off_w, bits[l - 1], dx[l - 1], L.pin, L.pin, mb);
+            if (rc == -1) rc = launch_gemv_dx(st, dY, L.pout, packed + L.off_w, acts[l - 1], L.pin, dx[l - 1], L.pin, L.pin, mb);
         } else {
             if (have_bits[l - 1] && x3 && xl.dx[l] >= 0)
                 rc = launch_gemm_nt_split(st, dY, L.pout, x3 + xl.dx[l], nullptr, dx[l - 1], L.pin, mb, L.pin, L.pout, 1, bits[l - 1]);
@@ -967,20 +996,18 @@
                           out_tanh ? EPI_BIAS_TANH : EPI_BIAS);
 }
 static int head_backward(hipStream_t st, const NetLayout &net, const float *packed, const float *dY, const float *X, int64_t mb,
-                         float *dx_prev, float *grad, float *tn_ws, const unsigned long long *bits_prev, int64_t ld_dy = 0,
-                         DwList *defer = nullptr) {
+                         float *dx_prev, float *grad, float *tn_ws, const unsigned long long *bits_prev, DwList *defer = nullptr) {
     const int last = net.n_layers - 1;
     const LayerLayout &L = net.L[last];
     const int64_t ldx = net.L[last - 1].pout;
     const bool gemv = gemv_head_ok(L.out, L.pin);
     const size_t floats = tn_layer_floats(net, last, mb, 0);
-    if (!ld_dy) ld_dy = L.pout;
     int rc = 0;
-    if (gemv) rc = launch_gemv_dw(st, dY, ld_dy, X, ldx, grad + L.off_flat_w, grad + L.off_flat_b, L.in, L.pin, mb, tn_ws, floats);
+    if (gemv) rc = launch_gemv_dw(st, dY, L.pout, X, ldx, grad + L.off_flat_w, grad + L.off_flat_b, L.in, L.pin, mb, tn_ws, floats);
     else if (defer) defer->add(L, dY, RowSource{X, ldx}, grad);
     else rc = launch_gemm_tn(st, dY, L.pout, L.pout, X, ldx, L.pin, grad + L.off_flat_w, grad + L.off_flat_b, L.out, L.in, mb, tn_ws, floats);
     if (rc) return rc;
-    if (gemv) return launch_gemv_dx_bits(st, dY, ld_dy, packed + L.off_w, bits_prev, dx_prev, L.pin, L.pin, mb);
+    if (gemv) return launch_gemv_dx_bits(st, dY, L.pout, packed + L.off_w, bits_prev, dx_prev, L.pin, L.pin, mb);
     rc = launch_gemm_nt_bits(st, dY, L.pout, packed + L.off_wt, L.pout, nullptr, dx_prev, L.pin, mb, L.pin, L.pout, EPI_MASK,
                              const_cast<unsigned long long *>(bits_prev));
     if (rc == -1) {
@@ -1064,7 +1091,6 @@
     const rlppo_minibatch_args &a = *p.a;
     const WsPlan &w = p.w;
     const int width = p.pol.L[0].pin;
-    float *const vout = w.val.act[p.val.n_layers - 1];
     if (p.prec == 1) {
         auto lean0 = [](const NetLayout &n) {
             return n.n_layers > 1 && nt_b16_ok(n.L[0].pout, n.L[0].pin, true) && tn_b16_ok(n.L[0].pout, n.L[0].pin);
@@ -1076,12 +1102,17 @@
         GatherMeta gm;
         gm.actions = a.actions; gm.old_logp = a.old_logp; gm.adv = a.advantages; gm.targets = a.targets;
         gm.g_old = w.g_old; gm.g_adv = w.g_adv; gm.g_tgt = w.g_tgt; gm.g_act = w.g_act;
-        gm.zero_n = vout;
         gm.act_dim = a.act_dim;
         return launch_gather_rows(p.st, a.states, a.ld_states, a.idx, w.states, width, p.mb, p.ring_base, p.ring_cap, &gm);
     }
     return launch_gather_meta(p.st, a.idx, a.actions, a.act_dim, a.old_logp, a.advantages, a.targets, w.g_act, w.g_old, w.g_adv, w.g_tgt,
-                              p.mb, p.ring_base, p.ring_cap, p.rows.rowtab ? w.rowtab : nullptr, vout);
+                              p.mb, p.ring_base, p.ring_cap, p.rows.rowtab ? w.rowtab : nullptr);
+}
+
+static CriticTail pass_tail(const Pass &p) {
+    const int H = p.val.n_layers - 1;
+    return CriticTail{p.w.g_tgt, p.w.g_adv, p.cfg, p.a->stats, H >= 1 ? p.w.val.act[H - 1] : nullptr, H >= 1 ? p.w.val.dx[H - 1] : nullptr,
+                      p.w.val.act[H], p.a->val_grad, p.w.val.tn, tn_layer_floats(p.val, H, p.mb, 0)};
 }
 
 static int paired_pass(const Pass &p, SlotBank &bk, int slot) {
@@ -1093,9 +1124,8 @@
     const int H = pol.n_layers - 1;
     int rc;
     const LayerLayout &Lvh = val.L[H];
-    const bool fold_v = g_fold_vhead && gemv_head_ok(Lvh.out, Lvh.pin) && val.L[H - 1].pout / 128 <= 2;
+    bool fuse_v = tail_ok(val) && !(H == 1 && p.rows.rowtab);
     float *vout = w.val.act[H], *pout = w.pol.act[H];
-    const int64_t ldv = fold_v ? 1 : Lvh.pout;
     const float *xp = p.rows.x, *xv = xp;
     int64_t ldx = p.rows.ld;
     for (int l = 0; l < H; ++l) {
@@ -1106,16 +1136,14 @@
         alt.bias = p.val_w + Lv.off_b;
         alt.C = w.val.act[l];
         alt.bits = w.val.bits[l];
-        NtDot dots[2];
-        const bool fold_here = fold_v && l == H - 1;
-        if (fold_here) {
-            dots[1].w = p.val_w + Lvh.off_w;
-            dots[1].out = vout;
-            dots[1].b = p.val_w + Lvh.off_b;
+        bool alone = false;
+        if (fuse_v && l == H - 1) {
+            rc = critic_tail(st, val, p.val_w, xv, ldx, mb, pass_tail(p));
+            if (rc != 0 && rc != -1) return rc;
+            alone = fuse_v = rc == 0;
         }
         rc = launch_gemm_nt_bits(st, xp, ldx, p.pol_w + Lp.off_w, Lp.pin, p.pol_w + Lp.off_b, w.pol.act[l], Lp.pout, mb, Lp.pout, Lp.pin,
-                                 EPI_BIAS_RELU, w.pol.bits[l], l == 0 ? p.rows.rowtab : nullptr, p.rows.src_rows, &alt,
-                                 fold_here ? dots : nullptr);
+                                 EPI_BIAS_RELU, w.pol.bits[l], l == 0 ? p.rows.rowtab : nullptr, p.rows.src_rows, alone ? nullptr : &alt);
         if (rc) {
             if (rc == -1) set_error("paired pass: a hidden layer does not have the bitmask form");
             return rc == -1 ? RLPPO_ERR_ARG : rc;
@@ -1124,36 +1152,43 @@
         xv = w.val.act[l];
         ldx = Lp.pout;
     }
-    if (hs != st) {
-        rc = order_after(hs, st, bk.ev_fork[slot]);
-        if (rc) return rc;
-    }
-    if (!fold_v) {
+    if (fuse_v) {
+        rc = head_forward(st, pol, p.pol_w, xp, ldx, mb, a.head == RLPPO_HEAD_GAUSSIAN, pout);
+        if (rc) return rc;
+        rc = policy_loss(st, p);
+        if (rc) return rc;
+        rc = head_backward(st, pol, p.pol_w, pout, xp, mb, w.pol.dx[H - 1], a.pol_grad, w.pol.tn, w.pol.bits[H - 1], p.defer);
+        if (rc) return rc;
+    } else {
+        if (hs != st) {
+            rc = order_after(hs, st, bk.ev_fork[slot]);
+            if (rc) return rc;
+        }
         rc = head_forward(hs, val, p.val_w, xv, ldx, mb, 0, vout);
         if (rc) return rc;
-    }
-    rc = launch_value_loss(hs, vout, ldv, w.g_tgt, w.g_adv, mb, p.cfg, a.stats);
-    if (rc) return rc;
-    const bool ordered = g_head_order && hs != st;
-    if (!ordered) {
-        rc = head_backward(hs, val, p.val_w, vout, xv, mb, w.val.dx[H - 1], a.val_grad, w.val.tn, w.val.bits[H - 1], ldv, p.defer);
-        if (rc) return rc;
-    }
-    rc = head_forward(st, pol, p.pol_w, xp, ldx, mb, a.head == RLPPO_HEAD_GAUSSIAN, pout);
-    if (rc) return rc;
-    rc = policy_loss(st, p);
-    if (rc) return rc;
-    if (ordered) {
-        rc = order_after(hs, st, bk.ev_mid[slot]);
-        if (rc) return rc;
-        rc = head_backward(hs, val, p.val_w, vout, xv, mb, w.val.dx[H - 1], a.val_grad, w.val.tn, w.val.bits[H - 1], ldv, p.defer);
-        if (rc) return rc;
-    }
-    rc = head_backward(st, pol, p.pol_w, pout, xp, mb, w.pol.dx[H - 1], a.pol_grad, w.pol.tn, w.pol.bits[H - 1], 0, p.defer);
-    if (rc) return rc;
-    if (hs != st) {
-        rc = order_after(st, hs, bk.ev_join[slot]);
-        if (rc) return rc;
+        rc = launch_value_loss(hs, vout, Lvh.pout, w.g_tgt, w.g_adv, mb, p.cfg, a.stats);
+        if (rc) return rc;
+        const bool ordered = g_head_order && hs != st;
+        if (!ordered) {
+            rc = head_backward(hs, val, p.val_w, vout, xv, mb, w.val.dx[H - 1], a.val_grad, w.val.tn, w.val.bits[H - 1], p.defer);
+            if (rc) return rc;
+        }
+        rc = head_forward(st, pol, p.pol_w, xp, ldx, mb, a.head == RLPPO_HEAD_GAUSSIAN, pout);
+        if (rc) return rc;
+        rc = policy_loss(st, p);
+        if (rc) return rc;
+        if (ordered) {
+            rc = order_after(hs, st, bk.ev_mid[slot]);
+            if (rc) return rc;
+            rc = head_backward(hs, val, p.val_w, vout, xv, mb, w.val.dx[H - 1], a.val_grad, w.val.tn, w.val.bits[H - 1], p.defer);
+            if (rc) return rc;
+        }
+        rc = head_backward(st, pol, p.pol_w, pout, xp, mb, w.pol.dx[H - 1], a.pol_grad, w.pol.tn, w.pol.bits[H - 1], p.defer);
+        if (rc) return rc;
+        if (hs != st) {
+            rc = order_after(st, hs, bk.ev_join[slot]);
+            if (rc) return rc;
+        }
     }
     for (int l = H - 1; l >= 0; --l) {
         const LayerLayout &Lp = pol.L[l], &Lv = val.L[l];
@@ -1197,7 +1232,7 @@
     const unsigned short *pol_x3 = p.prec == 2 ? pol_wb16 : nullptr, *val_x3 = p.prec == 2 ? val_wb16 : nullptr;
     bool phave[RLPPO_MAX_LAYERS] = {}, vhave[RLPPO_MAX_LAYERS] = {};
     bool pf32[RLPPO_MAX_LAYERS] = {}, vf32[RLPPO_MAX_LAYERS] = {};
-    bool v_folded = false;
+    bool v_fused = false;
     int rc;
     if (b16) {
         rc = forward_b16(p.side, val, p.val_w, val_wb16, p.rows.x, w.states_b, p.rows.ld, mb, 0, w.val.act, w.val.actb, w.val.bits, vhave,
@@ -1206,14 +1241,16 @@
         rc = forward_b16(p.st, pol, p.pol_w, pol_wb16, p.rows.x, w.states_b, p.rows.ld, mb, a.head == RLPPO_HEAD_GAUSSIAN, w.pol.act,
                          w.pol.actb, w.pol.bits, phave, pf32);
     } else {
-        rc = forward(p.side, val, p.val_w, p.rows, mb, 0, w.val.act, 0, w.val.bits, vhave, &v_folded, val_x3, true);
-        if (rc) return rc;
-        rc = forward(p.st, pol, p.pol_w, p.rows, mb, a.head == RLPPO_HEAD_GAUSSIAN, w.pol.act, 0, w.pol.bits, phave, nullptr, pol_x3);
-    }
-    if (rc) return rc;
-    const int64_t ldv = v_folded ? 1 : val.L[val.n_layers - 1].pout;
-    rc = launch_value_loss(p.side, w.val.act[val.n_layers - 1], ldv, w.g_tgt, w.g_adv, mb, p.cfg, a.stats);
-    if (rc) return rc;
+        const CriticTail tail = pass_tail(p);
+        rc = forward(p.side, val, p.val_w, p.rows, mb, 0, w.val.act, 0, w.val.bits, vhave, &tail, &v_fused, val_x3);
+        if (rc) return rc;
+        rc = forward(p.st, pol, p.pol_w, p.rows, mb, a.head == RLPPO_HEAD_GAUSSIAN, w.pol.act, 0, w.pol.bits, phave, nullptr, nullptr, pol_x3);
+    }
+    if (rc) return rc;
+    if (!v_fused) {
+        rc = launch_value_loss(p.side, w.val.act[val.n_layers - 1], val.L[val.n_layers - 1].pout, w.g_tgt, w.g_adv, mb, p.cfg, a.stats);
+        if (rc) return rc;
+    }
     rc = policy_loss(p.st, p);
     if (rc) return rc;
     if (b16) {
@@ -1223,7 +1260,7 @@
         return backward_b16(p.st, pol, p.pol_w, pol_wb16, p.rows.x, w.states_b, p.rows.ld, mb, w.pol.act, w.pol.actb, w.pol.dx, w.pol.dxb,
                             a.pol_grad, w.pol.tn, tn_ws_floats(pol, mb, p.prec), w.pol.bits, phave, pf32);
     }
-    rc = backward(p.side, val, p.val_w, p.rows, mb, w.val.act, w.val.dx, a.val_grad, w.val.tn, w.val.bits, vhave, v_folded, val_x3, p.defer);
+    rc = backward(p.side, val, p.val_w, p.rows, mb, w.val.act, w.val.dx, a.val_grad, w.val.tn, w.val.bits, vhave, v_fused, val_x3, p.defer);
     if (rc) return rc;
     return backward(p.st, pol, p.pol_w, p.rows, mb, w.pol.act, w.pol.dx, a.pol_grad, w.pol.tn, w.pol.bits, phave, false, pol_x3, p.defer);
 }
@@ -1524,7 +1561,7 @@
         case 27: g_fused_act = value; return 0;
         case 29: g_paired = value; return 0;
         case 31: g_head_order = value; return 0;
-        case 32: g_fold_vhead = value; return 0;
+        case 32: g_fuse_tail = value; return 0;
         case 33: set_pair_interleave(value); return 0;
         case 37: g_group_dw = value; return 0;
         case 38: set_tn_group_budget(value); return 0;
@@ -1551,6 +1588,7 @@
         case 4: return g_cnt_gather_fused_pass;
         case 5: return g_cnt_group_dw;
         case 6: return g_cnt_md_nvec;
+        case 7: return g_cnt_tail;
         default: return -1;
     }
 }
diff --git a/rlgym_ppo_amd/csrc/common.hpp b/rlgym_ppo_amd/csrc/common.hpp
--- a/rlgym_ppo_amd/csrc/common.hpp
+++ b/rlgym_ppo_amd/csrc/common.hpp
@@ -93,17 +93,13 @@
     unsigned long long *bits = nullptr;
     int interleave = 0;
 };
-struct NtDot {
-    const float *w = nullptr, *b = nullptr;
-    float *out = nullptr;
-};
 struct TnPair {
     const float *dY = nullptr, *X = nullptr;
     float *dW = nullptr, *db = nullptr, *ws = nullptr;
 };
 int launch_gemm_nt_bits(hipStream_t st, const float *A, int64_t lda, const float *B, int64_t ldb, const float *bias, float *C,
                         int64_t ldc, int64_t M, int N, int K, int epi, unsigned long long *bits, const unsigned *rowtab = nullptr,
-                        int64_t src_rows = 0, const NtAlt *alt = nullptr, const NtDot *dot = nullptr );
+                        int64_t src_rows = 0, const NtAlt *alt = nullptr);
 bool nt_gather_ok(int64_t lda, int64_t src_rows, int N, int K);
 int launch_gemm_nt_bf16(hipStream_t st, const float *A, int64_t lda, const float *B, int64_t ldb, const float *bias, float *C,
                         int64_t ldc, int64_t M, int N, int nb, int K, int epi);
@@ -194,6 +190,30 @@
                                 unsigned *done_words = nullptr, unsigned done_value = 0);
 int launch_value_loss(hipStream_t st, float *vout, int64_t ldv, const float *targets, const float *adv, int64_t mb, const LossCfg &cfg,
                       double *stats);
+__device__ __forceinline__ float value_grad(float v, float target, float adv, const LossCfg &c, float *sq) {
+    if (c.vclip > 0.f) {
+        const float v_old = target - adv;
+        const float dv = v - v_old;
+        const float d = (v_old + fminf(fmaxf(dv, -c.vclip), c.vclip)) - target;
+        *sq = d * d;
+        return fabsf(dv) <= c.vclip ? c.mb_ratio * (2.f * d * c.inv_mb) : 0.f;
+    }
+    const float d = v - target;
+    *sq = d * d;
+    return c.mb_ratio * (2.f * d * c.inv_mb);
+}
+struct NtTail {
+    const float *w = nullptr, *b = nullptr;
+    const float *tgt = nullptr, *adv = nullptr;
+    float *h = nullptr;
+    float *dx = nullptr;
+    float *dv = nullptr;
+    double *stats = nullptr;
+    LossCfg cfg;
+};
+constexpr int NT_TAIL_ROWS = 64;
+int launch_gemm_nt_tail(hipStream_t st, const float *A, int64_t lda, const float *B, int64_t ldb, const float *bias, int64_t M, int N,
+                        int K, const NtTail &t);
 int64_t kl_slots_doubles(int64_t mb);
 constexpr int64_t DISCRETE_LOSS_MAX_LD = 64 * 32;
 int launch_discrete_loss(hipStream_t, float *, int64_t, int, const float *, const float *, const float *, int64_t, const LossCfg &, double *,
@@ -267,14 +287,14 @@
                          long long ocount, int state_f64);
 struct GatherMeta {
     const float *actions = nullptr, *old_logp = nullptr, *adv = nullptr, *targets = nullptr;
-    float *g_act = nullptr, *g_old = nullptr, *g_adv = nullptr, *g_tgt = nullptr, *zero_n = nullptr;
+    float *g_act = nullptr, *g_old = nullptr, *g_adv = nullptr, *g_tgt = nullptr;
     int act_dim = 0;
 };
 int launch_gather_rows(hipStream_t st, const float *src, int64_t ld_src, const int64_t *idx, float *dst, int width, int64_t n,
                        int64_t ring_base = 0, int64_t ring_cap = INT64_MAX, const GatherMeta *meta = nullptr);
 int launch_gather_meta(hipStream_t st, const int64_t *idx, const float *actions, int act_dim, const float *old_logp,
                        const float *adv, const float *targets, float *g_act, float *g_old, float *g_adv, float *g_tgt, int64_t n,
-                       int64_t ring_base, int64_t ring_cap, unsigned *rowtab = nullptr, float *zero_n = nullptr);
+                       int64_t ring_base, int64_t ring_cap, unsigned *rowtab = nullptr);
 int launch_i64_to_f32(hipStream_t st, const int64_t *src, float *dst, int64_t n);
 int launch_learn_report(hipStream_t st, const rlppo_report_args &r);
 int launch_signal_words(hipStream_t st, unsigned *words, int count, unsigned value);
diff --git a/rlgym_ppo_amd/csrc/gemm.hip b/rlgym_ppo_amd/csrc/gemm.hip
--- a/rlgym_ppo_amd/csrc/gemm.hip
+++ b/rlgym_ppo_amd/csrc/gemm.hip
@@ -11,8 +11,7 @@
                                                                               unsigned ldc_b, int64_t M, int K,
                                                                               unsigned long long *__restrict__ bits = nullptr,
                                                                               const unsigned *__restrict__ rowtab = nullptr,
-                                                                              unsigned src_rows = 0, NtAlt alt = NtAlt{},
-                                                                              NtDot dot = NtDot{}, NtDot dot_alt = NtDot{}) {
+                                                                              unsigned src_rows = 0, NtAlt alt = NtAlt{}) {
     constexpr int BN = NB * 16;
     constexpr int CPR = BKT / 4;
     constexpr int RPW = 64 / CPR;
@@ -43,7 +42,6 @@
         bias = alt.bias;
         C = alt.C;
         bits = alt.bits;
-        dot = dot_alt;
     }
     const int64_t m0 = (int64_t)row_tile * SBM;
     const int n0 = col_tile * BN;
@@ -142,33 +140,191 @@
 #pragma unroll
                 for (int e = 0; e < 4; ++e) acc[i][j][e] = relu1(acc[i][j][e]);
         *bit_word = relu_bits<NB>(acc);
-        if (dot.w) {
-            const __amdgpu_buffer_rsrc_t w_rs = make_rsrc(dot.w + n0, BN * 4);
-            float s0 = 0.f, s1 = 0.f;
-#pragma unroll
-            for (int j = 0; j < NB; ++j) {
-                const f32x4 wv = ldb(w_rs, (unsigned)(q * 16), j * 64);
-#pragma unroll
-                for (int e = 0; e < 4; ++e) {
-                    s0 += acc[0][j][e] * wv[e];
-                    s1 += acc[1][j][e] * wv[e];
-                }
-            }
-            s0 += __shfl_xor(s0, 16);
-            s1 += __shfl_xor(s1, 16);
-            s0 += __shfl_xor(s0, 32);
-            s1 += __shfl_xor(s1, 32);
-            if (q == 0) {
-                const float b0 = col_tile == 0 ? dot.b[0] : 0.f;
-                const int r0 = wave * 32 + r16;
-                if (r0 < rows_here) atomicAdd(dot.out + m0 + r0, s0 + b0);
-                if (r0 + 16 < rows_here) atomicAdd(dot.out + m0 + r0 + 16, s1 + b0);
-            }
-        }
         nt_epilogue<NB, EPI_NONE>(acc, nullptr, 0, C, ldc_b, m0, n0, rows_here, wave, r16, q, park);
     } else {
         nt_epilogue<NB, EPI>(acc, mask_src, ldm_b, C, ldc_b, m0, n0, rows_here, wave, r16, q, park);
     }
+}
+
+namespace {
+template <int CTRL>
+__device__ __forceinline__ float nt_dpp(float v) {
+    return __builtin_bit_cast(float, __builtin_amdgcn_update_dpp(0, __builtin_bit_cast(int, v), CTRL, 0xF, 0xF, true));
+}
+__device__ __forceinline__ float nt_row16_sum(float v) {
+    v += nt_dpp<0xB1>(v);
+    v += nt_dpp<0x4E>(v);
+    v += nt_dpp<0x141>(v);
+    v += nt_dpp<0x140>(v);
+    return v;
+}
+}
+
+template <int NB>
+__global__ __launch_bounds__(256, 4) void gemm_nt_tail_kernel(const float *__restrict__ A, unsigned lda_b, const float *__restrict__ B,
+                                                              unsigned ldb_b, const float *__restrict__ bias, int64_t M, int K, NtTail t) {
+    constexpr int BN = NB * 16, TBM = NT_TAIL_ROWS, BKT = 16;
+    constexpr int RPW = 16, RPP = 64;
+    constexpr int B_IT = BN / RPP;
+    static_assert(NB == 8 || NB == 16, "the tail tile is 128 or 256 columns wide");
+    constexpr int STAGE_F = 2 * (TBM + BN) * BKT;
+    constexpr int PARK_F = 4 * 2048;
+    constexpr int TAIL_F = PARK_F + 4;
+    __shared__ __attribute__((aligned(16))) float lds[STAGE_F > TAIL_F ? STAGE_F : TAIL_F];
+    float *As = lds;
+    float *Bs = lds + 2 * TBM * BKT;
+
+    const int tid = threadIdx.x;
+    const int lane = tid & 63, wave = tid >> 6;
+    const int wave_u = __builtin_amdgcn_readfirstlane(wave);
+    const int r16 = lane & 15, q = lane >> 4;
+    const int64_t m0 = (int64_t)blockIdx.x * TBM;
+    const int rows_here = (int)((M - m0) < TBM ? (M - m0) : TBM);
+    const int row_l = wave * 16 + r16;
+    const bool row_live = row_l < rows_here;
+
+    const __amdgpu_buffer_rsrc_t a_rs = make_rsrc(reinterpret_cast<const char *>(A) + m0 * lda_b, (unsigned)(rows_here - 1) * lda_b + (unsigned)K * 4);
+    const __amdgpu_buffer_rsrc_t b_rs = make_rsrc(B, (unsigned)(BN - 1) * ldb_b + (unsigned)K * 4);
+    const int row_p = wave * RPW + lane / 4, pch = lane % 4;
+    const int lch = pch ^ ((0 - (row_p >> 2)) & 3);
+    const unsigned a_off = (unsigned)row_p * lda_b + lch * 16;
+    const unsigned b_off = (unsigned)row_p * ldb_b + lch * 16;
+    const unsigned b_step = (unsigned)RPP * ldb_b;
+
+    f32x4 acc[NB];
+    {
+        const __amdgpu_buffer_rsrc_t bias_rs = make_rsrc(bias, BN * 4);
+#pragma unroll
+        for (int j = 0; j < NB; ++j) acc[j] = ldb(bias_rs, (unsigned)(q * 16), j * 64);
+    }
+
+    auto issue_tile = [&](int buf, unsigned kb) {
+        float *Ad = As + buf * TBM * BKT + wave_u * RPW * BKT;
+        float *Bd = Bs + buf * BN * BKT + wave_u * RPW * BKT;
+        __builtin_amdgcn_raw_ptr_buffer_load_lds(a_rs, Ad, 16, a_off, kb, 0, 0);
+#pragma unroll
+        for (int i = 0; i < B_IT; ++i) __builtin_amdgcn_raw_ptr_buffer_load_lds(b_rs, Bd + i * RPP * BKT, 16, b_off, kb + i * b_step, 0, 0);
+    };
+
+    const int nk = K / BKT;
+    issue_tile(0, 0);
+    asm volatile("s_waitcnt vmcnt(0)" ::: "memory");
+    __syncthreads();
+    for (int kt = 0; kt < nk; ++kt) {
+        const int cur = kt & 1;
+        if ((kt + 1) < nk) issue_tile(cur ^ 1, (unsigned)(kt + 1) * (BKT * 4));
+        const float *Ac = As + cur * TBM * BKT + (wave * 16) * BKT;
+        const float *Bc = Bs + cur * BN * BKT;
+        const f32x4 fa = *reinterpret_cast<const f32x4 *>(&Ac[dswz<BKT>(r16, q)]);
+#pragma unroll
+        for (int g = 0; g < NB / 8; ++g) {
+            f32x4 fb[8];
+#pragma unroll
+            for (int j = 0; j < 8; ++j) fb[j] = *reinterpret_cast<const f32x4 *>(&Bc[dswz<BKT>((g * 8 + j) * 16 + r16, q)]);
+#pragma unroll
+            for (int s = 0; s < 4; ++s)
+#pragma unroll
+                for (int j = 0; j < 8; ++j) acc[g * 8 + j] = MFMA16(fb[j][s], fa[s], acc[g * 8 + j]);
+        }
+        __builtin_amdgcn_sched_barrier(0);
+        asm volatile("s_waitcnt vmcnt(0)" ::: "memory");
+        __syncthreads();
+    }
+
+    float *const wsum = lds + PARK_F;
+    const __amdgpu_buffer_rsrc_t tg_rs = make_rsrc(t.tgt + m0, (unsigned)rows_here * 4);
+    const float target = __builtin_bit_cast(float, __builtin_amdgcn_raw_buffer_load_b32(tg_rs, (unsigned)row_l * 4, 0, 0));
+    float adv = 0.f;
+    if (t.cfg.vclip > 0.f) {
+        const __amdgpu_buffer_rsrc_t ad_rs = make_rsrc(t.adv + m0, (unsigned)rows_here * 4);
+        adv = __builtin_bit_cast(float, __builtin_amdgcn_raw_buffer_load_b32(ad_rs, (unsigned)row_l * 4, 0, 0));
+    }
+    const __amdgpu_buffer_rsrc_t w_rs = make_rsrc(t.w, BN * 4);
+    float sp[NB / 8];
+#pragma unroll
+    for (int g = 0; g < NB / 8; ++g) {
+        float s = 0.f;
+#pragma unroll
+        for (int j = 8 * g; j < 8 * g + 8; ++j) {
+            const f32x4 wv = ldb(w_rs, (unsigned)(q * 16), j * 64);
+#pragma unroll
+            for (int e = 0; e < 4; ++e) {
+                acc[j][e] = relu1(acc[j][e]);
+                s += acc[j][e] * wv[e];
+            }
+            if ((j & 3) == 3) __builtin_amdgcn_sched_barrier(0);
+        }
+        s += __shfl_xor(s, 16);
+        s += __shfl_xor(s, 32);
+        sp[g] = s;
+    }
+    float v = sp[0] + t.b[0];
+    if (NB == 16) v += sp[NB / 8 - 1];
+    float sq;
+    float dv = value_grad(v, target, adv, t.cfg, &sq);
+    float loss = sq * t.cfg.inv_mb;
+    if (!row_live) dv = loss = 0.f;
+    if (row_live && q == 0) t.dv[m0 + row_l] = dv;
+    {
+        const float lsum = nt_row16_sum(loss);
+        if (lane == 0) wsum[wave] = lsum;
+    }
+    __syncthreads();
+    if (tid == 0 && !(t.cfg.stop_word && *t.cfg.stop_word))
+        atomicAdd(t.stats + RLPPO_STAT_VLOSS, (double)wsum[0] + (double)wsum[1] + (double)wsum[2] + (double)wsum[3]);
+    __builtin_amdgcn_sched_barrier(0);
+    char *const park = reinterpret_cast<char *>(lds) + wave_u * 8192;
+    const unsigned ldc_b = (unsigned)BN * 4;
+    const int rr = lane >> 5, c32 = lane & 31;
+    auto store_tile = [&](float *C) {
+        const __amdgpu_buffer_rsrc_t c_rs = make_rsrc(reinterpret_cast<char *>(C) + m0 * ldc_b, (unsigned)rows_here * ldc_b);
+#pragma unroll
+        for (int h = 0; h < NB / 8; ++h) {
+            asm volatile("s_waitcnt lgkmcnt(0)" ::: "memory");
+#pragma unroll
+            for (int j = 0; j < 8; ++j) *reinterpret_cast<f32x4 *>(park + r16 * 512 + (((j * 4 + q) ^ r16) * 16)) = acc[h * 8 + j];
+            f32x4 o[8];
+#pragma unroll
+            for (int u = 0; u < 8; ++u) {
+                const int r = 2 * u + rr;
+                o[u] = *reinterpret_cast<const f32x4 *>(park + r * 512 + ((c32 ^ r) * 16));
+            }
+            const unsigned c_off = (unsigned)(wave * 16 + rr) * ldc_b + h * 512 + c32 * 16;
+#pragma unroll
+            for (int u = 0; u < 8; ++u) stb(c_rs, c_off, 2 * u * ldc_b, o[u]);
+        }
+    };
+    store_tile(t.h);
+    const float *w_again = t.w;
+    asm volatile("" : "+s"(w_again));
+    const __amdgpu_buffer_rsrc_t w2_rs = make_rsrc(w_again, BN * 4);
+    f32x4 wn = ldb(w2_rs, (unsigned)(q * 16), 0);
+#pragma unroll
+    for (int j = 0; j < NB; ++j) {
+        const f32x4 wv = wn;
+        if (j + 1 < NB) wn = ldb(w2_rs, (unsigned)(q * 16), (j + 1) * 64);
+#pragma unroll
+        for (int e = 0; e < 4; ++e) acc[j][e] = acc[j][e] > 0.f ? dv * wv[e] : 0.f;
+        asm volatile("" : "+v"(acc[j]));
+        __builtin_amdgcn_sched_barrier(0);
+    }
+    asm volatile("s_waitcnt vmcnt(0)" ::: "memory");
+    store_tile(t.dx);
+}
+
+int launch_gemm_nt_tail(hipStream_t st, const float *A, int64_t lda, const float *B, int64_t ldb, const float *bias, int64_t M, int N,
+                        int K, const NtTail &t) {
+    if (M <= 0) return 0;
+    if ((N != 128 && N != 256) || K <= 0 || K % 16 != 0 || lda % 4 != 0 || ldb % 4 != 0 || lda < K || ldb < K) return -1;
+    const int64_t lim = (int64_t)1 << 31;
+    if ((NT_TAIL_ROWS + 1) * lda * 4 >= lim || (int64_t)(N + 1) * ldb * 4 >= lim || cdiv(M, NT_TAIL_ROWS) >= lim) return -1;
+    RLPPO_CHECK_ARG(A && B && bias && t.w && t.b && t.tgt && t.h && t.dx && t.dv && t.stats && (!(t.cfg.vclip > 0.f) || t.adv), "gemm_nt (critic tail): null operand");
+    const dim3 grid((unsigned)cdiv(M, NT_TAIL_ROWS));
+    const unsigned la = (unsigned)(lda * 4), lb = (unsigned)(ldb * 4);
+    if (N == 256) hipLaunchKernelGGL((gemm_nt_tail_kernel<16>), grid, dim3(256), 0, st, A, la, B, lb, bias, M, K, t);
+    else hipLaunchKernelGGL((gemm_nt_tail_kernel<8>), grid, dim3(256), 0, st, A, la, B, lb, bias, M, K, t);
+    RLPPO_LAUNCH_CHECK();
+    return 0;
 }
 
 __device__ __forceinline__ bf16x8 to_bf16x8(const float *lo, const float *hi) {
@@ -424,7 +580,7 @@
 }
 int launch_gemm_nt_bits(hipStream_t st, const float *A, int64_t lda, const float *B, int64_t ldb, const float *bias, float *C,
                         int64_t ldc, int64_t M, int N, int K, int epi, unsigned long long *bits, const unsigned *rowtab,
-                        int64_t src_rows, const NtAlt *alt, const NtDot *dot) {
+                        int64_t src_rows, const NtAlt *alt) {
     if (!bits || N % 128 != 0 || K % 16 != 0 || M <= 0) return -1;
     if (epi != EPI_BIAS_RELU && epi != EPI_MASK) return -1;
     const int64_t lim = (int64_t)1 << 31;
@@ -437,17 +593,14 @@
         grid.z = 1;
         second.interleave = 1;
     }
-    const NtDot d0 = dot ? dot[0] : NtDot{}, d1 = dot && alt ? dot[1] : NtDot{};
-    RLPPO_CHECK_ARG(!dot || (epi == EPI_BIAS_RELU && N / 128 <= 2 && (!d0.w || (d0.out && d0.b)) && (!d1.w || (d1.out && d1.b))),
-                    "gemm_nt: the folded one-output head needs the ReLU forward form and at most two column tiles");
     const unsigned la = (unsigned)(lda * 4), lb = (unsigned)(ldb * 4), lc = (unsigned)(ldc * 4);
     if (rowtab) {
         RLPPO_CHECK_ARG(epi == EPI_BIAS_RELU && nt_gather_ok(lda, src_rows, N, K), "gemm_nt (gathered rows): unsupported shape");
         hipLaunchKernelGGL((gemm_nt_dma_kernel<8, EPI_BIAS_RELU, 16, true, true>), grid, dim3(256), 0, st, A, la, B, lb, bias, nullptr,
-                           0u, C, lc, M, K, bits, rowtab, (unsigned)src_rows, second, d0, d1);
+                           0u, C, lc, M, K, bits, rowtab, (unsigned)src_rows, second);
     } else if (epi == EPI_BIAS_RELU)
         hipLaunchKernelGGL((gemm_nt_dma_kernel<8, EPI_BIAS_RELU, 16, true>), grid, dim3(256), 0, st, A, la, B, lb, bias, nullptr,
-                           0u, C, lc, M, K, bits, nullptr, 0u, second, d0, d1);
+                           0u, C, lc, M, K, bits, nullptr, 0u, second);
     else
         hipLaunchKernelGGL((gemm_nt_dma_kernel<8, EPI_MASK, 16, true>), grid, dim3(256), 0, st, A, la, B, lb, nullptr, nullptr, 0u,
                            C, lc, M, K, bits, nullptr, 0u, second);
diff --git a/rlgym_ppo_amd/csrc/heads.hip b/rlgym_ppo_amd/csrc/heads.hip
--- a/rlgym_ppo_amd/csrc/heads.hip
+++ b/rlgym_ppo_amd/csrc/heads.hip
@@ -360,17 +360,9 @@
 }
 
 __device__ __forceinline__ float value_row(float *vout_row, float target, float adv, const LossCfg &c) {
-    const float v = vout_row[0];
-    if (c.vclip > 0.f) {
-        const float v_old = target - adv;
-        const float dv = v - v_old;
-        const float d = (v_old + fminf(fmaxf(dv, -c.vclip), c.vclip)) - target;
-        vout_row[0] = fabsf(dv) <= c.vclip ? c.mb_ratio * (2.f * d * c.inv_mb) : 0.f;
-        return d * d;
-    }
-    const float d = v - target;
-    vout_row[0] = c.mb_ratio * (2.f * d * c.inv_mb);
-    return d * d;
+    float sq;
+    vout_row[0] = value_grad(vout_row[0], target, adv, c, &sq);
+    return sq;
 }
 
 template <class L, bool MASKED>
diff --git a/rlgym_ppo_amd/csrc/optim.hip b/rlgym_ppo_amd/csrc/optim.hip
--- a/rlgym_ppo_amd/csrc/optim.hip
+++ b/rlgym_ppo_amd/csrc/optim.hip
@@ -196,7 +196,6 @@
         meta.g_adv[row] = meta.adv[srow];
         meta.g_tgt[row] = meta.targets[srow];
         for (int k = 0; k < meta.act_dim; ++k) meta.g_act[row * meta.act_dim + k] = meta.actions[srow * meta.act_dim + k];
-        if (meta.zero_n) meta.zero_n[row] = 0.f;
     }
 }
 
@@ -239,13 +238,11 @@
                                                           const float *__restrict__ adv, const float *__restrict__ targets,
                                                           float *__restrict__ g_act, float *__restrict__ g_old,
                                                           float *__restrict__ g_adv, float *__restrict__ g_tgt, int64_t n,
-                                                          int64_t ring_base, int64_t ring_cap, unsigned *__restrict__ rowtab,
-                                                          float *__restrict__ zero_n) {
+                                                          int64_t ring_base, int64_t ring_cap, unsigned *__restrict__ rowtab) {
     const int64_t r = (int64_t)blockIdx.x * 256 + threadIdx.x;
     if (r >= n) return;
     const int64_t src = ring_row(idx[r], ring_base, ring_cap);
     if (rowtab) rowtab[r] = (unsigned)src;
-    if (zero_n) zero_n[r] = 0.f;
     g_old[r] = old_logp[src];
     g_adv[r] = adv[src];
     g_tgt[r] = targets[src];
@@ -254,10 +251,10 @@
 
 int launch_gather_meta(hipStream_t st, const int64_t *idx, const float *actions, int act_dim, const float *old_logp,
                        const float *adv, const float *targets, float *g_act, float *g_old, float *g_adv, float *g_tgt, int64_t n,
-                       int64_t ring_base, int64_t ring_cap, unsigned *rowtab, float *zero_n) {
+                       int64_t ring_base, int64_t ring_cap, unsigned *rowtab) {
     if (n <= 0) return 0;
     hipLaunchKernelGGL(gather_meta_kernel, dim3((unsigned)cdiv(n, 256)), dim3(256), 0, st, idx, actions, act_dim, old_logp, adv,
-                       targets, g_act, g_old, g_adv, g_tgt, n, ring_base, ring_cap, rowtab, zero_n);
+                       targets, g_act, g_old, g_adv, g_tgt, n, ring_base, ring_cap, rowtab);
     RLPPO_LAUNCH_CHECK();
     return 0;
 }
diff --git a/rlgym_ppo_amd/ppo/_mlp.py b/rlgym_ppo_amd/ppo/_mlp.py
--- a/rlgym_ppo_amd/ppo/_mlp.py
+++ b/rlgym_ppo_amd/ppo/_mlp.py
@@ -1,4 +1,5 @@
 import ctypes
+import gc
 import math
 import os
 
@@ -116,8 +117,14 @@
             body()
         side.synchronize()
         self.graph = torch.cuda.CUDAGraph()
-        with torch.cuda.graph(self.graph, capture_error_mode="thread_local"):
-            body()
+        gc_on = gc.isenabled()
+        gc.disable()
+        try:
+            with torch.cuda.graph(self.graph, capture_error_mode="thread_local"):
+                body()
+        finally:
+            if gc_on:
+                gc.enable()
         self._count = None
         if chain_masked:
             N.check(L.rlppo_dbg_count(6, -2))
```
